# atneit/SCA-LDPC

Hardware: AMD Instinct MI355X
Metric: edge_message_updates_per_s (higher is better)
Workload: dtype f32; 1 GPU; hqc128 H=[Hin|I] N=17669 W=50 R=4000 E=204000, batch 4096/GPU, 50 fixed iters, min_sum; batch_per_gpu=4096, iters=50, tile_group=0

## Files before the change

### include/scaldpc.h

```cpp
#ifndef SCALDPC_H
#define SCALDPC_H

#include <stdint.h>

#ifdef __cplusplus
extern "C" {
#endif

#define SCALDPC_VERSION 104

#define SCALDPC_OK 0
#define SCALDPC_EINVAL 1
#define SCALDPC_EHIP 2
#define SCALDPC_ENOMEM 3
#define SCALDPC_EPMF 4
#define SCALDPC_ENOCONF 5
#define SCALDPC_EDEGREE 6

#define SCALDPC_BP_PRODUCT_SUM 0
#define SCALDPC_BP_MIN_SUM 1

#define SCALDPC_IN_SYNDROME 0
#define SCALDPC_IN_RECEIVED 1

#define SCALDPC_F_EARLY_EXIT 1u
#define SCALDPC_F_DEVICE_IO 2u
#define SCALDPC_F_ASYNC 4u

const char *scaldpc_last_error(void);
int scaldpc_version(void);
int scaldpc_device_count(int *count);
int scaldpc_set_device(int device);
int scaldpc_trim(void);
int scaldpc_debug_live_blocks(int64_t *out);
int scaldpc_debug_fail_alloc(int32_t countdown);
int scaldpc_measure_rmw_stream(int64_t bytes, int32_t rows_per_wave, int32_t reps, double *gbps);

typedef struct scaldpc_bp scaldpc_bp;

int scaldpc_bp_create(int32_t m, int32_t n, int64_t nnz, const int32_t *row_ptr,
                      const int32_t *col_idx, scaldpc_bp **out);
int scaldpc_bp_set_channel_probs(scaldpc_bp *h, const double *probs);
int scaldpc_bp_append_rows(scaldpc_bp *h, int32_t nrows, const int32_t *row_ptr, const int32_t *col_idx, int32_t new_n);
int scaldpc_bp_set_channel_probs_tail(scaldpc_bp *h, int32_t first, int32_t count, const double *probs);
int scaldpc_bp_decode_batch(scaldpc_bp *h, const uint8_t *in, int32_t input_kind, int32_t batch,
                            int32_t max_iter, int32_t method, float alpha, uint32_t flags,
                            void *stream, uint8_t *out_bits, float *out_llr, int32_t *out_iters,
                            uint8_t *out_conv);
int scaldpc_bp_decode_batch_soft(scaldpc_bp *h, const uint8_t *in, int32_t input_kind, int32_t batch,
                                 const float *probs, int32_t prob_cols,
                                 int32_t max_iter, int32_t method, float alpha, uint32_t flags, void *stream,
                                 uint8_t *out_bits, float *out_llr, int32_t *out_iters, uint8_t *out_conv);
int scaldpc_bp_decode_batch_f64(scaldpc_bp *h, const uint8_t *in, int32_t input_kind, int32_t batch,
                                const double *probs, int32_t prob_cols, int32_t max_iter, uint32_t flags, void *stream,
                                uint8_t *out_bits, double *out_llr, int32_t *out_iters, uint8_t *out_conv);
int scaldpc_bp_time_kernels(scaldpc_bp *h, int32_t iters, int32_t method, float alpha, void *stream,
                            float *ms, int32_t *launches);
int scaldpc_bp_set_tile_group(scaldpc_bp *h, int32_t tiles);
int scaldpc_bp_last_compacted(scaldpc_bp *h, int64_t *count);
int scaldpc_bp_last_stats(scaldpc_bp *h, int64_t *out);
#define SCALDPC_SCHEDULE_WORDS 24
int scaldpc_bp_last_schedule(scaldpc_bp *h, int64_t *out);
int scaldpc_bp_last_settle(scaldpc_bp *h, int32_t *frozen_at, int32_t cap, int64_t *info);
int scaldpc_bp_configure(scaldpc_bp *h, const char *key, const char *value);
int scaldpc_bp_device_of(scaldpc_bp *h, int32_t *out);
void scaldpc_bp_destroy(scaldpc_bp *h);

int scaldpc_mc_fer_run(scaldpc_bp *h, int64_t first_trial, int32_t batch, uint64_t seed, int32_t max_iter,
                       int32_t method, float alpha, uint32_t flags, void *stream, uint8_t *out_success,
                       int32_t *out_iters, uint8_t *out_error);
int scaldpc_mc_hqc_run(scaldpc_bp *h, int32_t omega, double eps, int64_t first_trial, int32_t batch, uint64_t seed,
                       int32_t max_iter, int32_t method, float alpha, uint32_t flags, void *stream,
                       uint8_t *out_success, int32_t *out_iters, uint8_t *out_msg, int32_t *out_y);

int scaldpc_mc_hqc_run_soft(scaldpc_bp *h, int32_t omega, const double *weights, const uint8_t *flips, const float *probs,
                            const int32_t *costs, int32_t K, int64_t first_trial, int32_t batch, uint64_t seed,
                            int32_t max_iter, int32_t method, float alpha, uint32_t flags, void *stream,
                            uint8_t *out_success, int32_t *out_iters, uint8_t *out_msg, int32_t *out_y, uint8_t *out_outcome,
                            int32_t *out_flips, int32_t *out_cost);

int scaldpc_mc_hqc_run_stats(scaldpc_bp *h, int32_t omega, const double *weights, const uint8_t *flips, const float *probs,
                             const int32_t *costs, int32_t K, int64_t first_trial, int32_t batch, uint64_t seed,
                             int32_t max_iter, int32_t method, float alpha, uint32_t flags, void *stream,
                             uint8_t *out_success, int32_t *out_iters, uint8_t *out_msg, int32_t *out_y, uint8_t *out_outcome,
                             int32_t *out_flips, int32_t *out_cost, int32_t *out_stats, uint8_t *out_bits);

int scaldpc_mc_fer_run_f64(scaldpc_bp *h, int64_t first_trial, int32_t batch, uint64_t seed, int32_t max_iter,
                           uint32_t flags, void *stream, uint8_t *out_success, int32_t *out_iters, uint8_t *out_error);
int scaldpc_mc_hqc_run_f64(scaldpc_bp *h, int32_t omega, double eps, int64_t first_trial, int32_t batch, uint64_t seed,
                           int32_t max_iter, uint32_t flags, void *stream, uint8_t *out_success, int32_t *out_iters,
                           uint8_t *out_msg, int32_t *out_y);
int scaldpc_mc_hqc_run_stats_f64(scaldpc_bp *h, int32_t omega, const double *weights, const uint8_t *flips,
                                 const double *probs, const int32_t *costs, int32_t K, int64_t first_trial,
                                 int32_t batch, uint64_t seed, int32_t max_iter, uint32_t flags, void *stream,
                                 uint8_t *out_success, int32_t *out_iters, uint8_t *out_msg, int32_t *out_y,
                                 uint8_t *out_outcome, int32_t *out_flips, int32_t *out_cost,
                                 int32_t *out_stats , uint8_t *out_bits);

int scaldpc_mc_fer_run_at(scaldpc_bp *h, const int64_t *trial_ids, int32_t batch, uint64_t seed, int32_t max_iter,
                          int32_t method, float alpha, uint32_t flags, void *stream, uint8_t *out_success,
                          int32_t *out_iters, uint8_t *out_error);
int scaldpc_mc_hqc_run_stats_at(scaldpc_bp *h, int32_t omega, const double *weights, const uint8_t *flips, const float *probs,
                                const int32_t *costs, int32_t K, const int64_t *trial_ids, int32_t batch, uint64_t seed,
                                int32_t max_iter, int32_t method, float alpha, uint32_t flags, void *stream,
                                uint8_t *out_success, int32_t *out_iters, uint8_t *out_msg, int32_t *out_y,
                                uint8_t *out_outcome, int32_t *out_flips, int32_t *out_cost,
                                int32_t *out_stats , uint8_t *out_bits);
int scaldpc_mc_fer_run_at_f64(scaldpc_bp *h, const int64_t *trial_ids, int32_t batch, uint64_t seed, int32_t max_iter,
                              uint32_t flags, void *stream, uint8_t *out_success, int32_t *out_iters, uint8_t *out_error);
int scaldpc_mc_hqc_run_stats_at_f64(scaldpc_bp *h, int32_t omega, const double *weights, const uint8_t *flips,
                                    const double *probs, const int32_t *costs, int32_t K, const int64_t *trial_ids,
                                    int32_t batch, uint64_t seed, int32_t max_iter, uint32_t flags, void *stream,
                                    uint8_t *out_success, int32_t *out_iters, uint8_t *out_msg, int32_t *out_y,
                                    uint8_t *out_outcome, int32_t *out_flips, int32_t *out_cost,
                                    int32_t *out_stats , uint8_t *out_bits);

typedef struct scaldpc_qary scaldpc_qary;

int scaldpc_qary_create(int32_t R, int32_t N, int32_t B, const int8_t *H, int32_t iterations,
                        scaldpc_qary **out);
int scaldpc_qary_min_sum_batch(scaldpc_qary *h, const float *pmf, int32_t batch, uint32_t flags,
                               void *stream, int8_t *out);
void scaldpc_qary_destroy(scaldpc_qary *h);
int scaldpc_qary_into_llr(const float *pmf, int64_t rows, int32_t Q, uint32_t flags, void *stream, float *llr);
int scaldpc_qary_configure(scaldpc_qary *h, const char *key, const char *value);
int scaldpc_qary_last_timing(scaldpc_qary *h, float *ms, int32_t *info);

int scaldpc_qary_special_create(int32_t R, int32_t N, int32_t B, int32_t BSUM, const int8_t *H,
                                int32_t iterations, scaldpc_qary **out);
int scaldpc_qary_special_min_sum_batch(scaldpc_qary *h, const float *pmf_b, const float *pmf_sum,
                                       int32_t batch, uint32_t flags, void *stream, int8_t *out);

int scaldpc_qary_min_sum_batch_soft(scaldpc_qary *h, const float *pmf, int32_t batch, uint32_t flags, void *stream,
                                    int8_t *out, float *out_cost, float *out_margin, int32_t *out_unmet);
int scaldpc_qary_special_min_sum_batch_soft(scaldpc_qary *h, const float *pmf_b, const float *pmf_sum, int32_t batch,
                                            uint32_t flags, void *stream, int8_t *out,
                                            float *out_cost_b, float *out_cost_sum, float *out_margin, int32_t *out_unmet);

int scaldpc_mc_qary_run(scaldpc_qary *h, const float *levels_b, const double *weights_b, int32_t k_b,
                        const float *levels_s, const double *weights_s, int32_t k_s,
                        int64_t first_trial, int32_t batch, uint64_t seed, uint32_t flags, void *stream,
                        uint8_t *out_success, int32_t *out_errs, int32_t *out_wrong, uint8_t *out_levels,
                        int8_t *out_symbols);

int scaldpc_mc_qary_run_secret(scaldpc_qary *h, const double *prior_b,
                               const float *levels_b, const double *weights_b, int32_t k_b,
                               const float *levels_s, const double *weights_s, int32_t k_s,
                               int64_t first_trial, int32_t batch, uint64_t seed, uint32_t flags, void *stream,
                               uint8_t *out_success, int32_t *out_wrong, int32_t *out_channel_wrong,
                               int8_t *out_secret, uint8_t *out_levels, int8_t *out_symbols);

int scaldpc_mc_qary_run_at(scaldpc_qary *h, const float *levels_b, const double *weights_b, int32_t k_b,
                           const float *levels_s, const double *weights_s, int32_t k_s,
                           const int64_t *trial_ids, int32_t batch, uint64_t seed, uint32_t flags, void *stream,
                           uint8_t *out_success, int32_t *out_errs, int32_t *out_wrong, uint8_t *out_levels,
                           int8_t *out_symbols);
int scaldpc_mc_qary_run_secret_at(scaldpc_qary *h, const double *prior_b,
                                  const float *levels_b, const double *weights_b, int32_t k_b,
                                  const float *levels_s, const double *weights_s, int32_t k_s,
                                  const int64_t *trial_ids, int32_t batch, uint64_t seed, uint32_t flags, void *stream,
                                  uint8_t *out_success, int32_t *out_wrong, int32_t *out_channel_wrong,
                                  int8_t *out_secret, uint8_t *out_levels, int8_t *out_symbols);

#ifdef __cplusplus
}
#endif
#endif
```

### sca-ldpc_amd/_lib.py

```python
from __future__ import annotations

import ctypes as C
import os
import subprocess
import sys

_HERE = os.path.dirname(os.path.abspath(__file__))
SO_PATH = os.environ.get("SCALDPC_SO") or os.path.join(_HERE, "libscaldpc.so")
CSRC = os.path.join(_HERE, "csrc")

OK, EINVAL, EHIP, ENOMEM, EPMF, ENOCONF, EDEGREE = range(7)
BP_PRODUCT_SUM, BP_MIN_SUM = 0, 1
IN_SYNDROME, IN_RECEIVED = 0, 1
F_EARLY_EXIT, F_DEVICE_IO, F_ASYNC = 1, 2, 4

_lib = None


class ScaldpcError(RuntimeError):
    pass


def build(verbose=False):
    out = None if verbose else subprocess.DEVNULL
    subprocess.check_call(["make", "-C", CSRC, "../libscaldpc.so"], stdout=out)
    return SO_PATH


def _declare(lib):
    p = C.POINTER
    vp = C.c_void_p
    lib.scaldpc_last_error.restype = C.c_char_p
    lib.scaldpc_last_error.argtypes = []
    lib.scaldpc_version.restype = C.c_int
    lib.scaldpc_device_count.argtypes = [p(C.c_int)]
    lib.scaldpc_set_device.argtypes = [C.c_int]
    lib.scaldpc_trim.argtypes = []
    lib.scaldpc_trim.restype = C.c_int
    lib.scaldpc_debug_live_blocks.argtypes = [p(C.c_int64)]
    lib.scaldpc_debug_live_blocks.restype = C.c_int
    lib.scaldpc_debug_fail_alloc.argtypes = [C.c_int32]
    lib.scaldpc_debug_fail_alloc.restype = C.c_int
    lib.scaldpc_measure_rmw_stream.argtypes = [C.c_int64, C.c_int32, C.c_int32, p(C.c_double)]
    lib.scaldpc_measure_rmw_stream.restype = C.c_int
    lib.scaldpc_bp_create.argtypes = [C.c_int32, C.c_int32, C.c_int64, vp, vp, p(vp)]
    lib.scaldpc_bp_set_channel_probs.argtypes = [vp, vp]
    lib.scaldpc_bp_decode_batch.argtypes = [
        vp, vp, C.c_int32, C.c_int32, C.c_int32, C.c_int32, C.c_float, C.c_uint32, vp, vp, vp, vp, vp,
    ]
    lib.scaldpc_bp_decode_batch_soft.argtypes = [
        vp, vp, C.c_int32, C.c_int32, vp, C.c_int32, C.c_int32, C.c_int32, C.c_float, C.c_uint32, vp, vp, vp, vp, vp,
    ]
    lib.scaldpc_bp_decode_batch_soft.restype = C.c_int
    lib.scaldpc_bp_decode_batch_f64.argtypes = [
        vp, vp, C.c_int32, C.c_int32, vp, C.c_int32, C.c_int32, C.c_uint32, vp, vp, vp, vp, vp,
    ]
    lib.scaldpc_bp_decode_batch_f64.restype = C.c_int
    lib.scaldpc_bp_time_kernels.argtypes = [vp, C.c_int32, C.c_int32, C.c_float, vp, p(C.c_float), p(C.c_int32)]
    lib.scaldpc_bp_set_tile_group.argtypes = [vp, C.c_int32]
    lib.scaldpc_bp_last_compacted.argtypes = [vp, p(C.c_int64)]
    lib.scaldpc_bp_last_compacted.restype = C.c_int
    lib.scaldpc_bp_last_stats.argtypes = [vp, p(C.c_int64)]
    lib.scaldpc_bp_last_stats.restype = C.c_int
    lib.scaldpc_bp_last_schedule.argtypes = [vp, p(C.c_int64)]
    lib.scaldpc_bp_last_schedule.restype = C.c_int
    if hasattr(lib, "scaldpc_bp_last_settle"):
        lib.scaldpc_bp_last_settle.argtypes = [vp, p(C.c_int32), C.c_int32, p(C.c_int64)]
        lib.scaldpc_bp_last_settle.restype = C.c_int
    lib.scaldpc_bp_append_rows.argtypes = [vp, C.c_int32, vp, vp, C.c_int32]
    lib.scaldpc_bp_append_rows.restype = C.c_int
    lib.scaldpc_bp_set_channel_probs_tail.argtypes = [vp, C.c_int32, C.c_int32, vp]
    lib.scaldpc_bp_set_channel_probs_tail.restype = C.c_int
    lib.scaldpc_bp_configure.argtypes = [vp, C.c_char_p, C.c_char_p]
    lib.scaldpc_bp_configure.restype = C.c_int
    lib.scaldpc_bp_device_of.argtypes = [vp, p(C.c_int32)]
    lib.scaldpc_bp_device_of.restype = C.c_int
    lib.scaldpc_bp_destroy.argtypes = [vp]
    lib.scaldpc_bp_destroy.restype = None
    lib.scaldpc_mc_fer_run.argtypes = [
        vp, C.c_int64, C.c_int32, C.c_uint64, C.c_int32, C.c_int32, C.c_float, C.c_uint32, vp, vp, vp, vp,
    ]
    lib.scaldpc_mc_hqc_run.argtypes = [
        vp, C.c_int32, C.c_double, C.c_int64, C.c_int32, C.c_uint64, C.c_int32, C.c_int32, C.c_float, C.c_uint32,
        vp, vp, vp, vp, vp,
    ]
    lib.scaldpc_mc_hqc_run_soft.argtypes = [
        vp, C.c_int32, vp, vp, vp, vp, C.c_int32, C.c_int64, C.c_int32, C.c_uint64, C.c_int32, C.c_int32, C.c_float, C.c_uint32,
        vp, vp, vp, vp, vp, vp, vp, vp,
    ]
    lib.scaldpc_mc_hqc_run_stats.argtypes = lib.scaldpc_mc_hqc_run_soft.argtypes + [vp, vp]
    lib.scaldpc_mc_fer_run_f64.argtypes = [vp, C.c_int64, C.c_int32, C.c_uint64, C.c_int32, C.c_uint32, vp, vp, vp, vp]
    lib.scaldpc_mc_hqc_run_f64.argtypes = [
        vp, C.c_int32, C.c_double, C.c_int64, C.c_int32, C.c_uint64, C.c_int32, C.c_uint32, vp, vp, vp, vp, vp,
    ]
    lib.scaldpc_mc_hqc_run_stats_f64.argtypes = [
        vp, C.c_int32, vp, vp, vp, vp, C.c_int32, C.c_int64, C.c_int32, C.c_uint64, C.c_int32, C.c_uint32,
        vp, vp, vp, vp, vp, vp, vp, vp, vp, vp,
    ]
    for name in ("scaldpc_mc_fer_run_f64", "scaldpc_mc_hqc_run_f64", "scaldpc_mc_hqc_run_stats_f64"):
        getattr(lib, name).restype = C.c_int
    for name, sibling, at in (("scaldpc_mc_fer_run_at", "scaldpc_mc_fer_run", 1),
                              ("scaldpc_mc_hqc_run_stats_at", "scaldpc_mc_hqc_run_stats", 7),
                              ("scaldpc_mc_fer_run_at_f64", "scaldpc_mc_fer_run_f64", 1),
                              ("scaldpc_mc_hqc_run_stats_at_f64", "scaldpc_mc_hqc_run_stats_f64", 7)):
        a = list(getattr(lib, sibling).argtypes)
        assert a[at] is C.c_int64
        a[at] = vp
        getattr(lib, name).argtypes = a
        getattr(lib, name).restype = C.c_int
    for name in (
        "scaldpc_device_count", "scaldpc_set_device", "scaldpc_bp_create", "scaldpc_bp_set_channel_probs",
        "scaldpc_bp_decode_batch", "scaldpc_bp_time_kernels", "scaldpc_bp_set_tile_group", "scaldpc_mc_fer_run",
        "scaldpc_mc_hqc_run", "scaldpc_mc_hqc_run_soft", "scaldpc_mc_hqc_run_stats",
    ):
        getattr(lib, name).restype = C.c_int
    lib.scaldpc_qary_create.argtypes = [C.c_int32, C.c_int32, C.c_int32, vp, C.c_int32, p(vp)]
    lib.scaldpc_qary_min_sum_batch.argtypes = [vp, vp, C.c_int32, C.c_uint32, vp, vp]
    lib.scaldpc_qary_configure.argtypes = [vp, C.c_char_p, C.c_char_p]
    lib.scaldpc_qary_configure.restype = C.c_int
    lib.scaldpc_qary_last_timing.argtypes = [vp, p(C.c_float), p(C.c_int32)]
    lib.scaldpc_qary_last_timing.restype = C.c_int
    lib.scaldpc_qary_into_llr.argtypes = [vp, C.c_int64, C.c_int32, C.c_uint32, vp, vp]
    lib.scaldpc_qary_into_llr.restype = C.c_int
    lib.scaldpc_qary_destroy.argtypes = [vp]
    lib.scaldpc_qary_destroy.restype = None
    lib.scaldpc_qary_special_create.argtypes = [C.c_int32, C.c_int32, C.c_int32, C.c_int32, vp, C.c_int32, p(vp)]
    lib.scaldpc_qary_special_min_sum_batch.argtypes = [vp, vp, vp, C.c_int32, C.c_uint32, vp, vp]
    lib.scaldpc_qary_min_sum_batch_soft.argtypes = [vp, vp, C.c_int32, C.c_uint32, vp, vp, vp, vp, vp]
    lib.scaldpc_qary_special_min_sum_batch_soft.argtypes = [vp, vp, vp, C.c_int32, C.c_uint32, vp, vp, vp, vp, vp, vp]
    lib.scaldpc_mc_qary_run.argtypes = [
        vp, vp, vp, C.c_int32, vp, vp, C.c_int32, C.c_int64, C.c_int32, C.c_uint64, C.c_uint32, vp, vp, vp, vp, vp, vp,
    ]
    lib.scaldpc_mc_qary_run_secret.argtypes = [
        vp, vp, vp, vp, C.c_int32, vp, vp, C.c_int32, C.c_int64, C.c_int32, C.c_uint64, C.c_uint32, vp, vp, vp, vp, vp, vp, vp,
    ]
    lib.scaldpc_mc_qary_run_at.argtypes = [
        vp, vp, vp, C.c_int32, vp, vp, C.c_int32, vp, C.c_int32, C.c_uint64, C.c_uint32, vp, vp, vp, vp, vp, vp,
    ]
    lib.scaldpc_mc_qary_run_secret_at.argtypes = [
        vp, vp, vp, vp, C.c_int32, vp, vp, C.c_int32, vp, C.c_int32, C.c_uint64, C.c_uint32, vp, vp, vp, vp, vp, vp, vp,
    ]
    lib.scaldpc_mc_qary_run_at.restype = lib.scaldpc_mc_qary_run_secret_at.restype = C.c_int
    for name in (
        "scaldpc_qary_create", "scaldpc_qary_min_sum_batch", "scaldpc_qary_special_create",
        "scaldpc_qary_special_min_sum_batch", "scaldpc_qary_min_sum_batch_soft", "scaldpc_qary_special_min_sum_batch_soft",
        "scaldpc_mc_qary_run", "scaldpc_mc_qary_run_secret",
    ):
        getattr(lib, name).restype = C.c_int


def load():
    global _lib
    if _lib is not None:
        return _lib
    if not os.path.exists(SO_PATH):
        raise ScaldpcError(
            f"{SO_PATH} is missing: build it with `make -C {CSRC}` (or __graft_entry__.build()). "
            "sca-ldpc_amd has no CPU fallback."
        )
    if "torch" not in sys.modules and os.environ.get("SCALDPC_NO_TORCH") != "1":
        try:
            import torch
        except Exception:
            pass
    lib = C.CDLL(SO_PATH, mode=C.RTLD_GLOBAL)
    _declare(lib)
    _lib = lib
    return lib


def check(rc):
    if rc == OK:
        return
    msg = load().scaldpc_last_error().decode(errors="replace")
    if rc == EINVAL:
        raise ValueError(msg)
    if rc == ENOMEM:
        raise MemoryError(msg)
    raise ScaldpcError(f"[{rc}] {msg}")


def trim():
    check(load().scaldpc_trim())


def live_blocks():
    out = (C.c_int64 * 6)()
    check(load().scaldpc_debug_live_blocks(out))
    keys = ("device_blocks", "device_bytes", "pinned_blocks", "pinned_bytes", "idle_blocks", "idle_bytes")
    return dict(zip(keys, (int(v) for v in out)))


def measure_rmw_stream(nbytes, rows_per_wave=51, reps=50):
    out = C.c_double(0.0)
    check(load().scaldpc_measure_rmw_stream(int(nbytes), int(rows_per_wave), int(reps), C.byref(out)))
    return float(out.value)


def trial_ids(ids):
    import numpy as np

    a = np.asarray(ids)
    if a.ndim != 1:
        raise ValueError(f"trial_ids must be one-dimensional, got shape {a.shape}")
    if a.size == 0:
        raise ValueError("trial_ids is empty")
    if a.dtype == object and all(isinstance(x, (int, np.integer)) and not isinstance(x, (bool, np.bool_)) for x in a):
        pass
    elif a.dtype.kind not in "iu":
        raise ValueError(f"trial_ids must be of integer dtype, got {a.dtype} (trial indices are not rounded)")
    for bad, why in ((a < 0, "is negative"), (a > 2**63 - 1, "does not fit int64")):
        if bad.any():
            i = int(np.argmax(bad))
            raise ValueError(f"trial_ids[{i}] = {a[i]} {why}")
    return np.ascontiguousarray(a, dtype=np.int64)


def ptr(a):
    if a is None:
        return None
    if isinstance(a, int):
# ... 3 lines not shown
```

### sca-ldpc_amd/bp.py

```python
from __future__ import annotations

import ctypes as C
import os

import numpy as np

from . import _lib
from .graph import TannerGraph

_PS = {"prod_sum", "product_sum", "ps", "0", "prod sum", "prod_sum_log", "product_sum_log", "ps_log", "2", "psl"}
_MS = {"min_sum", "minimum_sum", "ms", "1", "minimum sum", "min sum", "min_sum_log", "minimum_sum_log", "ms_log", "3",
       "minimum sum_log", "msl"}


def _method_id(bp_method):
    key = str(bp_method).lower()
    if key in _PS:
        return _lib.BP_PRODUCT_SUM
    if key in _MS:
        return _lib.BP_MIN_SUM
    raise ValueError(
        f"BP method '{bp_method}' is invalid. Please choose from the following methods: "
        "'product_sum', 'minimum_sum', 'product_sum_log' or 'minimum_sum_log'"
    )
# ... 172 lines not shown
            if cp.ndim != 2 or cp.shape[0] != batch:
                raise ValueError(f"channel_probs must be a 2-D array [batch = {batch}, k], got shape {cp.shape}")
            if not 1 <= cp.shape[1] <= self.n:
                raise ValueError(f"channel_probs covers {cp.shape[1]} columns: expected 1 to n = {self.n}")
        if f64:
            _lib.check(
                self._lib.scaldpc_bp_decode_batch_f64(
                    self._h, _lib.ptr(x), kind, batch, _lib.ptr(cp), 0 if cp is None else cp.shape[1],
                    self.max_iter if max_iter is None else int(max_iter), flags, None,
                    _lib.ptr(bits), _lib.ptr(llr), _lib.ptr(iters), _lib.ptr(conv),
                )
            )
            return {"bits": bits, "llr": llr, "iters": iters, "converged": conv}
        if cp is not None:
            _lib.check(
                self._lib.scaldpc_bp_decode_batch_soft(
                    self._h, _lib.ptr(x), kind, batch, _lib.ptr(cp), cp.shape[1],
                    self.max_iter if max_iter is None else int(max_iter), self._method, self.ms_scaling_factor, flags, None,
                    _lib.ptr(bits), _lib.ptr(llr), _lib.ptr(iters), _lib.ptr(conv),
                )
            )
            return {"bits": bits, "llr": llr, "iters": iters, "converged": conv}
        _lib.check(
            self._lib.scaldpc_bp_decode_batch(
                self._h, _lib.ptr(x), kind, batch, self.max_iter if max_iter is None else int(max_iter),
                self._method, self.ms_scaling_factor, flags, None, _lib.ptr(bits), _lib.ptr(llr),
                _lib.ptr(iters), _lib.ptr(conv),
            )
        )
        return {"bits": bits, "llr": llr, "iters": iters, "converged": conv}

    def decode_batch_device(self, d_in, kind, batch, d_out_bits, max_iter=None, early_exit=False, stream=0,
                            d_out_llr=0, d_out_iters=0, d_out_conv=0, asynchronous=False, d_channel_probs=0, prob_cols=0,
                            precision=None):
        flags = _lib.F_DEVICE_IO | (_lib.F_EARLY_EXIT if early_exit else 0) | (_lib.F_ASYNC if asynchronous else 0)
        if (self.precision if precision is None else _precision(precision, self._method)) == "float64":
            _lib.check(
                self._lib.scaldpc_bp_decode_batch_f64(
                    self._h, C.c_void_p(d_in), kind, batch, C.c_void_p(d_channel_probs or None), int(prob_cols),
                    self.max_iter if max_iter is None else int(max_iter), flags, C.c_void_p(stream or None),
                    C.c_void_p(d_out_bits), C.c_void_p(d_out_llr or None), C.c_void_p(d_out_iters or None),
                    C.c_void_p(d_out_conv or None),
                )
            )
            return
        if d_channel_probs or prob_cols:
            _lib.check(
                self._lib.scaldpc_bp_decode_batch_soft(
                    self._h, C.c_void_p(d_in), kind, batch, C.c_void_p(d_channel_probs or None), int(prob_cols),
                    self.max_iter if max_iter is None else int(max_iter), self._method, self.ms_scaling_factor, flags,
                    C.c_void_p(stream or None), C.c_void_p(d_out_bits), C.c_void_p(d_out_llr or None),
                    C.c_void_p(d_out_iters or None), C.c_void_p(d_out_conv or None),
                )
            )
            return
        _lib.check(
            self._lib.scaldpc_bp_decode_batch(
                self._h, C.c_void_p(d_in), kind, batch, self.max_iter if max_iter is None else int(max_iter),
                self._method, self.ms_scaling_factor, flags, C.c_void_p(stream or None), C.c_void_p(d_out_bits),
                C.c_void_p(d_out_llr or None), C.c_void_p(d_out_iters or None), C.c_void_p(d_out_conv or None),
            )
        )

    def time_kernels(self, iters, stream=0):
        ms = (C.c_float * 2)()
        ln = (C.c_int32 * 6)()
        _lib.check(
            self._lib.scaldpc_bp_time_kernels(
                self._h, iters, self._method, self.ms_scaling_factor, C.c_void_p(stream or None), ms, ln
            )
        )
        return {"ms_check": ms[0], "ms_var": ms[1], "launches_check": ln[0], "launches_var": ln[1], "codewords": ln[2],
                "lanes": ln[3], "codewords_var": ln[4], "record_form": bool(ln[5] & 1),
                "var_writes_out": bool(ln[5] & 2), "var_slim": bool(ln[5] & 4)}

    def mc_fer_run(self, runs, seed, first_trial=0, max_iter=None, early_exit=True, want_errors=False, precision="float32"):
        return _mc_fer(self, int(first_trial), int(runs), "", seed, max_iter, early_exit, want_errors, precision)

    def mc_fer_run_at(self, trial_ids, seed, max_iter=None, early_exit=True, want_errors=False, precision="float32"):
        ids = _lib.trial_ids(trial_ids)
        return _mc_fer(self, _lib.ptr(ids), len(ids), "_at", seed, max_iter, early_exit, want_errors, precision)

    def mc_hqc_run(self, runs, omega, eps, seed, first_trial=0, max_iter=None, early_exit=True, want_inputs=False,
                   want_stats=False, want_bits=False, precision="float32"):
        f64 = _precision(precision, self._method) == "float64"
        if want_stats or want_bits:
            eps = float(eps)
            table = dict(weights=np.array([[eps, 1.0 - eps]] * 2), flips=np.array([1, 0], dtype=np.uint8),
                         probs=np.array([eps, eps]), costs=None)
            r = self.mc_hqc_run_soft(runs, omega, table, seed, first_trial=first_trial, max_iter=max_iter, early_exit=early_exit,
                                     want_inputs=want_inputs, want_stats=want_stats, want_bits=want_bits, precision=precision)
            return {k: r[k] for k in ("success", "iters", "msg", "y", "stats", "bits")}
        succ = np.empty(runs, dtype=np.uint8)
        iters = np.empty(runs, dtype=np.int32)
        msg = np.empty((runs, self.n), dtype=np.uint8) if want_inputs else None
        y = np.empty((runs, omega), dtype=np.int32) if want_inputs else None
        args = (
            self._h, int(omega), float(eps), int(first_trial), int(runs), int(seed),
            self.max_iter if max_iter is None else int(max_iter),
            *(() if f64 else (self._method, self.ms_scaling_factor)),
            _lib.F_EARLY_EXIT if early_exit else 0, None, _lib.ptr(succ), _lib.ptr(iters), _lib.ptr(msg), _lib.ptr(y),
        )
        _lib.check(getattr(self._lib, "scaldpc_mc_hqc_run" + ("_f64" if f64 else ""))(*args))
        return {"success": succ, "iters": iters, "msg": msg, "y": y}

    def mc_hqc_run_at(self, trial_ids, omega, eps, seed, max_iter=None, early_exit=True, want_inputs=False, want_stats=False,
                      want_bits=False, precision="float32"):
        ids = _lib.trial_ids(trial_ids)
        _precision(precision, self._method)
        eps = float(eps)
        table = dict(weights=np.array([[eps, 1.0 - eps]] * 2), flips=np.array([1, 0], dtype=np.uint8),
                     probs=np.array([eps, eps]), costs=None)
        r = self.mc_hqc_run_soft_at(ids, omega, table, seed, max_iter=max_iter, early_exit=early_exit, want_inputs=want_inputs,
                                    want_stats=want_stats, want_bits=want_bits, precision=precision)
        return {k: r[k] for k in ("success", "iters", "msg", "y") + (("stats", "bits") if want_stats or want_bits else ())}

    def mc_hqc_run_soft_at(self, trial_ids, omega, table, seed, max_iter=None, early_exit=True, want_inputs=False,
                           want_stats=False, want_bits=False, precision="float32"):
        ids = _lib.trial_ids(trial_ids)
        return _mc_hqc_soft(self, _lib.ptr(ids), len(ids), True, omega, table, seed, max_iter, early_exit, want_inputs, want_stats,
                                 want_bits, precision)

    def mc_hqc_run_soft(self, runs, omega, table, seed, first_trial=0, max_iter=None, early_exit=True, want_inputs=False,
                        want_stats=False, want_bits=False, precision="float32"):
        return _mc_hqc_soft(self, int(first_trial), int(runs), False, omega, table, seed, max_iter, early_exit, want_inputs,
                                 want_stats, want_bits, precision)

    def last_compacted(self):
        c = C.c_int64()
        _lib.check(self._lib.scaldpc_bp_last_compacted(self._h, C.byref(c)))
        return int(c.value)

    def last_stats(self):
        out = (C.c_int64 * 4)()
        _lib.check(self._lib.scaldpc_bp_last_stats(self._h, out))
        return {"compacted": int(out[0]), "row_parallel": int(out[1]), "levels": int(out[2])}

    def last_schedule(self):
        out = (C.c_int64 * 24)()
        _lib.check(self._lib.scaldpc_bp_last_schedule(self._h, out))
        w = [int(x) for x in out]
        return {"groups": w[0:4], "handed_down": w[4:7], "polls": w[7], "unseen": w[8], "continued": w[9],
                "left_open": w[10], "fixed_chained": w[11], "clears": w[12], "open_at_clear": w[13], "ring_rows": w[14],
                "row_parallel_polls": w[15], "ring_takes": w[16]}

    def last_settle(self):
        info = (C.c_int64 * 4)()
        _lib.check(self._lib.scaldpc_bp_last_settle(self._h, None, 0, info))
        tiles = int(info[0])
        at = (C.c_int32 * max(tiles, 1))()
        _lib.check(self._lib.scaldpc_bp_last_settle(self._h, at, tiles, info))
        return {"frozen_at": [int(x) for x in at[:tiles]], "launches_saved": int(info[1]), "tiles_rerun": int(info[2]),
                "horizon": int(info[3])}

    def last_row_parallel(self):
        return self.last_stats()["row_parallel"]

    def configure(self, **knobs):
        for k, v in knobs.items():
            _lib.check(self._lib.scaldpc_bp_configure(self._h, k.encode(), str(v).encode()))

    def device_of(self):
        out = (C.c_int32 * 4)()
        _lib.check(self._lib.scaldpc_bp_device_of(self._h, out))
        return {"device": out[0], "graph": out[1], "messages": out[2], "state": out[3]}

    def set_tile_group(self, tiles):
        _lib.check(self._lib.scaldpc_bp_set_tile_group(self._h, int(tiles)))

    def close(self):
        if getattr(self, "_h", None):
            self._lib.scaldpc_bp_destroy(self._h)
            self._h = None

    def __enter__(self):
        return self

    def __exit__(self, *exc):
        self.close()
        return False

    def __del__(self):
        try:
            self.close()
        except Exception:
            pass


def _mc_fer(dec, trials, runs, at, seed, max_iter, early_exit, want_errors, precision):
    f64 = _precision(precision, dec._method) == "float64"
    succ = np.empty(runs, dtype=np.uint8)
    iters = np.empty(runs, dtype=np.int32)
    err = np.empty((runs, dec.n), dtype=np.uint8) if want_errors else None
    args = (
        dec._h, trials, runs, int(seed), dec.max_iter if max_iter is None else int(max_iter),
        *(() if f64 else (dec._method, dec.ms_scaling_factor)),
        _lib.F_EARLY_EXIT if early_exit else 0, None, _lib.ptr(succ), _lib.ptr(iters), _lib.ptr(err),
    )
    _lib.check(getattr(dec._lib, f"scaldpc_mc_fer_run{at}" + ("_f64" if f64 else ""))(*args))
    return {"success": succ, "iters": iters, "errors": err}


def _mc_hqc_soft(dec, trials, runs, listed, omega, table, seed, max_iter, early_exit, want_inputs, want_stats, want_bits,
                 precision):
    f64 = _precision(precision, dec._method) == "float64"
    w = np.ascontiguousarray(table["weights"], dtype=np.float64)
    if w.ndim != 2 or w.shape[0] != 2:
        raise ValueError(f"table['weights'] must be [2, K], got shape {w.shape}")
    K = w.shape[1]
    fl = np.asarray(table["flips"])
    pr = np.ascontiguousarray(table["probs"], dtype=np.float64 if f64 else np.float32)
    costs = table.get("costs")
    if fl.shape != (K,) or pr.shape != (K,) or (costs is not None and np.shape(costs) != (K,)):
        raise ValueError(f"table: flips, probs and costs must hold one entry per outcome (K = {K})")
    cs = None if costs is None else np.asarray(costs)
    for name, a, t in (("flips", fl, np.uint8), ("costs", cs, np.int32)):
        if a is not None and not np.array_equal(a.astype(t), a):
            raise ValueError(f"table['{name}'] = {a.tolist()} does not fit {np.dtype(t).name}")
    fl = np.ascontiguousarray(fl, dtype=np.uint8)
    cs = None if cs is None else np.ascontiguousarray(cs, dtype=np.int32)
    succ = np.empty(runs, dtype=np.uint8)
    iters = np.empty(runs, dtype=np.int32)
    flips = np.empty(runs, dtype=np.int32)
    cost = np.empty(runs, dtype=np.int32) if costs is not None else None
    msg = np.empty((runs, dec.n), dtype=np.uint8) if want_inputs else None
    y = np.empty((runs, omega), dtype=np.int32) if want_inputs else None
    outcome = np.empty((runs, dec.m), dtype=np.uint8) if want_inputs else None
    args = (
        dec._h, int(omega), _lib.ptr(w), _lib.ptr(fl), _lib.ptr(pr), _lib.ptr(cs), K,
        trials, runs, int(seed), dec.max_iter if max_iter is None else int(max_iter),
        *(() if f64 else (dec._method, dec.ms_scaling_factor)),
        _lib.F_EARLY_EXIT if early_exit else 0, None, _lib.ptr(succ), _lib.ptr(iters),
        _lib.ptr(msg), _lib.ptr(y), _lib.ptr(outcome), _lib.ptr(flips), _lib.ptr(cost),
    )
    res = {"success": succ, "iters": iters, "flips": flips, "cost": cost, "msg": msg, "y": y, "outcome": outcome}
    want = want_stats or want_bits
    with_stats = want or listed or f64
    entry = "scaldpc_mc_hqc_run_" + ("stats" if with_stats else "soft") + ("_at" if listed else "") + ("_f64" if f64 else "")
    stats = np.empty((runs, len(HQC_STATS_COLUMNS)), dtype=np.int32) if want else None
    bits = np.empty((runs, dec.n), dtype=np.uint8) if want_bits else None
    _lib.check(getattr(dec._lib, entry)(*args, *((_lib.ptr(stats), _lib.ptr(bits)) if with_stats else ())))
    return dict(res, stats=stats, bits=bits) if want else res


bp_decoder = BpDecoder
```

### sca-ldpc_amd/csrc/scaldpc_bp.hip

```cpp
#include "scaldpc_common.h"
#include "scaldpc_bp_sched.h"
#include "scaldpc_mc_law.h"
#include "scaldpc_trials.h"

#include <algorithm>
#include <cfloat>
#include <chrono>
#include <cmath>
#include <cstdlib>
#include <cstring>
#include <mutex>
#include <unordered_map>
#include <vector>

typedef unsigned long long u64;

using namespace scaldpc;

#include "scaldpc_bp_kernels.h"
#include "scaldpc_bp_ref64.h"

namespace scaldpc {
int launch_mc_hqc_outcome64(const McHqcLaw64 &law, unsigned long long *synd, double *plane, int R, int batch, int T, long first,
                            unsigned k0, unsigned k1, int *acc_flips, int *acc_cost, uint8_t *out_outcome, hipStream_t s);
int launch_gather_prior64(const double *src, int cols, const int *ids, double *dst, int T2, hipStream_t s);
int launch_mc_bernoulli_at(bool xor_into, unsigned long long *planes, int len, int batch, int T, const long long *ids, unsigned stream,
                           unsigned k0, unsigned k1, const unsigned long long *thr, unsigned long long thr0, hipStream_t s);
int launch_mc_hqc_secret_at(unsigned long long *planes, int n, int N, int omega, int batch, int T, const long long *ids, unsigned k0,
                            unsigned k1, int *out_y, hipStream_t s);
int launch_mc_hqc_outcome_at(const McHqcLaw &law, unsigned long long *synd, float *plane, int R, int batch, int T, const long long *ids,
                             unsigned k0, unsigned k1, int *acc_flips, int *acc_cost, uint8_t *out_outcome, hipStream_t s);
int launch_mc_hqc_outcome64_at(const McHqcLaw64 &law, unsigned long long *synd, double *plane, int R, int batch, int T,
                               const long long *ids, unsigned k0, unsigned k1, int *acc_flips, int *acc_cost, uint8_t *out_outcome,
                               hipStream_t s);
}

namespace {

struct Buckets {
    int nb;
    int maxd[MAXB];
    int off[MAXB];
    int cnt[MAXB];
    int blk[MAXB + 1];
};

struct HostBuckets {
    Buckets bk;
    pvec<int> list;
    bool has_generic = false;
};

}

struct Knobs {
    enum Path { AUTO = 0, STREAM = 1, EDGE = 2, LDS = 3 };
    int path = AUTO;
    int split = 2;
    double group_mb = 215.0;
    int el_max = -1;
    int compact_after = -1;
    int fuse_test = 1;
    int first_fused = 1;
    int minsum_rec = 1;
    int settle = -1;
    int settle_horizon = 0;
};

struct HandleStreams {
    int device = 0;
    hipStream_t own_stream = nullptr;
    hipStream_t aux_stream[4] = {};
    hipEvent_t ev_join[4] = {}, ev_phase[4] = {};
    HandleStreams() = default;
    HandleStreams(const HandleStreams &) = delete;
    HandleStreams &operator=(const HandleStreams &) = delete;
    ~HandleStreams()
    {
        if (own_stream) stream_release(own_stream, device);
        for (int k = 0; k < 4; k++) {
            if (aux_stream[k]) stream_release(aux_stream[k], device);
            if (ev_join[k]) (void)hipEventDestroy(ev_join[k]);
            if (ev_phase[k]) (void)hipEventDestroy(ev_phase[k]);
        }
    }
};

struct scaldpc_bp : HandleStreams {
    Knobs kn;
    int m = 0, n = 0;
    long E = 0;
    int max_row_deg = 0, max_col_deg = 0, min_row_deg = 0;
    int *d_row_ptr = nullptr, *d_col_idx = nullptr, *d_col_ptr = nullptr, *d_csc_edge = nullptr;
    int *d_var_list = nullptr, *d_row_list = nullptr;
    int *d_var_meta = nullptr, *d_csc_list = nullptr;
    Buckets var_bk{}, row_bk{};
    bool need_scratch = false;
    float *d_prior = nullptr;
    bool have_prior = false;
    int prior_n = 0;
    int cap_tiles = 0, cap_group = 0, tile_group = 0;
    Buf<float> d_msg, d_scratch, d_post;
    Buf<u64> d_synd, d_recv, d_hard, d_done, d_conv, d_unsat;
    Buf<int> d_iters, d_remaining;
    Buf<float> d_pprior, d_probs_in;
    Buf<u64> d_soft_bad;
    int cap_remaining = 0;
    RemRing rem;
    SchedCounters sched;
    Buf<uint8_t> d_in, d_out_bits, d_out_conv;
    Buf<float> d_out_llr;
    Buf<int> d_out_iters;
    PinnedBuf<int> h_remaining;
    PinnedBuf<uint8_t> h_io;
    Buf<uint8_t> d_out_all;
    pvec<double> h_probs;
    Buf<u64> d_thr, d_mc, d_diff;
    Buf<int> d_ylist;
    Buf<uint8_t> d_succ;
    bool thr_valid = false;
    Buf<int> d_mc_acc;
    Buf<int> d_mc_stats;
    Buf<uint8_t> d_mc_outcome;
    Buf<long long> d_trial_ids;
    struct Level {
        int cap_tiles = 0;
        Buf<u64> synd, hard, done, conv, unsat;
        Buf<int> iters, ids, slot_of;
        Buf<float> post, pprior;
        Buf<double> pratio64;
    };
    static constexpr int MAX_LEVELS = SCHED_MAX_LEVELS;
    Level lv[MAX_LEVELS + 1];
    long stat_levels = 0;
    long stat_deferred = 0;
    Buf<float> d_emsg;
    Buf<int> d_el_unsat;
    int *d_el_slots = nullptr, *d_el_slot_col = nullptr;
    int el_waves = 0;
    int el_cap_bins = 0;
    bool el_ok = false;
    pvec<int> h_el_slots, h_el_col;
    pvec<int> seg_slot;
    pvec<unsigned char> seg_cap;
    int el_open_used = 0;
    bool incremental = false, full_stale = false;
    pvec<int> hg_col_idx;
    Buf<int> d_csr_rp, d_csr_ci;
    Buf<float> d_prior_buf;
    int ws_m = 0, ws_n = 0;
    pvec<int> el_dirty_slot, el_dirty_col;
    Buf<int> d_pairs;
    PinnedBuf<int> h_pairs;
    Buf<int> d_graph;
    Buf<int> d_tile_tab;
    Buf<int2> d_first_tab;
    Buf<float> d_rec;
    Buf<u64> d_mask;
    int cap_rec_group = 0;
    int *d_csc_row = nullptr, *d_var_rows = nullptr, *d_csr_pos = nullptr;
    bool var_reversed = false;
    bool first_valid = false;
    int first_method = -1;
    float first_alpha = 0.0f;
    Buf<int> d_el_tab;
    pvec<int> hg_row_ptr, hg_cdeg, hg_col_ptr, hg_csc_edge;
    HostBuckets hg_var, hg_row;
    int stat_el = 0;
    int identity_from = -1;
    bool async_used = false;
    bool broken = false;
    Buf<double> d_ratio, d_x64, d_c64, d_post64, d_pratio, d_probs_in64, d_out_llr64;
    Buf<int> d_rem64;
    PinnedBuf<int> h_rem64;
    bool ratio_valid = false;
    Buf<unsigned> d_settle;
    PinnedBuf<unsigned> h_settle;
    int settle_next = 0;
    int settle_key_iter = 0, settle_key_soft = 0;
    float settle_key_alpha = -1.0f;
    std::vector<int> settle_frozen_at;
    long settle_saved = 0, settle_rerun = 0;
    int settle_K = 0;
    int last_group = 0;
    bool last_early = false;
    std::mutex mu;
};

namespace {

bool set_knob(Knobs &k, const char *key, const char *val)
{
    if (!key || !val) return false;
    if (!strcmp(key, "path")) {
        if (!strcmp(val, "auto") || !*val) k.path = Knobs::AUTO;
        else if (!strcmp(val, "stream")) k.path = Knobs::STREAM;
        else if (!strcmp(val, "edge")) k.path = Knobs::EDGE;
        else if (!strcmp(val, "lds")) k.path = Knobs::LDS;
        else return false;
        return true;
    }
    char *end = nullptr;
    const double x = strtod(val, &end);
    if (end == val) return false;
    if (!strcmp(key, "split")) k.split = (int)x;
    else if (!strcmp(key, "group_mb")) k.group_mb = x;
    else if (!strcmp(key, "el_max")) k.el_max = (int)x;
    else if (!strcmp(key, "compact_after")) k.compact_after = (int)x;
    else if (!strcmp(key, "first_fused")) k.first_fused = (int)x != 0;
    else if (!strcmp(key, "minsum_rec")) k.minsum_rec = x == 2.0 ? 2 : (int)x != 0;
    else if (!strcmp(key, "fuse_test")) k.fuse_test = (int)x != 0;
    else if (!strcmp(key, "settle") && x >= -1 && x <= 2) k.settle = (int)x;
    else if (!strcmp(key, "settle_horizon") && x >= 0) k.settle_horizon = (int)x;
    else return false;
    return true;
}

void knobs_from_env(Knobs &k)
{
    static const char *const names[][2] = {{"SCALDPC_PATH", "path"}, {"SCALDPC_SPLIT", "split"},
                                           {"SCALDPC_GROUP_MB", "group_mb"}, {"SCALDPC_EL_MAX", "el_max"},
                                           {"SCALDPC_COMPACT_AFTER", "compact_after"}, {"SCALDPC_FIRST_FUSED", "first_fused"},
                                           {"SCALDPC_FUSE_TEST", "fuse_test"}, {"SCALDPC_MINSUM_REC", "minsum_rec"},
                                           {"SCALDPC_SETTLE", "settle"}, {"SCALDPC_SETTLE_HORIZON", "settle_horizon"}};
    for (auto &nm : names)
        if (const char *e = getenv(nm[0])) (void)set_knob(k, nm[1], e);
}

void build_buckets(const pvec<int> &deg, const int *bounds, int nb, bool keep_isolated, HostBuckets &out)
{
    const int n = (int)deg.size();
    int maxdeg = 0;
    for (int d : deg) maxdeg = std::max(maxdeg, d);
    pvec<int> start(maxdeg + 2, 0);
    for (int d : deg) start[d + 1]++;
    for (int d = 0; d <= maxdeg; d++) start[d + 1] += start[d];
    pvec<int> order(n), cursor(start.begin(), start.end() - 1);
    for (int i = 0; i < n; i++) order[cursor[deg[i]]++] = i;
    out.list.clear();
    out.list.reserve(n);
    out.has_generic = false;
    Buckets &bk = out.bk;
    memset(&bk, 0, sizeof bk);
    int lo = keep_isolated ? 0 : 1;
    for (int b = 0; b <= nb && lo <= maxdeg; b++) {
        const int hi = b < nb ? std::min(bounds[b], maxdeg) : maxdeg;
        if (hi < lo) continue;
        const int first = start[lo], last = start[hi + 1];
        if (last > first) {
            const int i = bk.nb++;
            bk.maxd[i] = b < nb ? bounds[b] : 0;
            if (b == nb) out.has_generic = true;
            bk.off[i] = (int)out.list.size();
            bk.cnt[i] = last - first;
            bk.blk[i + 1] = bk.blk[i] + (bk.cnt[i] + 3) / 4;
            out.list.insert(out.list.end(), order.begin() + first, order.begin() + last);
        }
        lo = hi + 1;
    }
}

template <typename T, bool P>
int grow(Buf<T, P> &b, size_t need)
{
    return b.ensure(need, need + need / 8);
}

int auto_group(const scaldpc_bp *h, int T, int plane_cols = 0)
{
    const double budget = h->kn.group_mb * 1e6;
    const double per_tile = ((double)h->E + plane_cols) * TW * sizeof(float);
    const int g = per_tile > 0 ? (int)(budget / per_tile) : T;
    return std::max(1, std::min(g, T));
}

int parity_blocks(int m) { return (m + 4 * ROWS_PER_WAVE - 1) / (4 * ROWS_PER_WAVE); }
int parity_waves(const scaldpc_bp *h) { return 4 * parity_blocks(h->m); }

int ensure_workspace(scaldpc_bp *h, int T, int G, bool want_post, int max_iter, int prob_cols = 0)
{
    if (prob_cols) SC_TRY(grow(h->d_pprior, (size_t)T * prob_cols * TW));
    if (T > h->cap_tiles || h->m > h->ws_m || h->n > h->ws_n) {
        h->d_synd.reset(); h->d_recv.reset(); h->d_hard.reset(); h->d_done.reset();
        h->d_conv.reset(); h->d_unsat.reset(); h->d_iters.reset(); h->d_post.reset();
        T = std::max(T, h->cap_tiles);
        h->cap_tiles = 0;
        const int wm = h->incremental ? h->m + h->m / 2 + 64 : h->m, wn = h->incremental ? h->n + h->n / 2 + 64 : h->n;
        const size_t pw = (size_t)4 * parity_blocks(wm);
        SC_TRY(h->d_synd.ensure((size_t)T * wm));
        SC_TRY(h->d_recv.ensure((size_t)T * wn));
        SC_TRY(h->d_hard.ensure((size_t)T * wn));
        SC_TRY(h->d_done.ensure((size_t)T));
        SC_TRY(h->d_conv.ensure((size_t)T));
        SC_TRY(h->d_unsat.ensure((size_t)T * pw));
        SC_TRY(h->d_iters.ensure((size_t)T * TW));
        h->cap_tiles = T;
        h->ws_m = wm;
        h->ws_n = wn;
    }
    if (want_post) SC_TRY(h->d_post.ensure((size_t)h->cap_tiles * h->ws_n * TW));
    const int want_rows = ring_rows_wanted(T, G);
    if (max_iter + 2 > h->cap_remaining || want_rows > h->rem.rows) {
        h->d_remaining.reset();
        h->h_remaining.reset();
        h->cap_remaining = 0;
        h->rem.rows = 0;
        const int len = max_iter + 2;
        SC_TRY(h->d_remaining.ensure((size_t)want_rows * (size_t)len));
        SC_TRY(h->h_remaining.ensure((size_t)len));
        h->cap_remaining = len;
        h->rem.rows = want_rows;
    }
    h->rem.slot = h->rem.rows;
    h->sched.w[SCHED_RING_ROWS] = h->rem.rows;
    return 0;
}

int next_remaining_row(scaldpc_bp *h, hipStream_t s, int **row, bool lanes_open)
{
    bool clears = false;
    const int slot = ring_take(h->rem, &clears);
    h->sched.note_take(clears, lanes_open);
    if (clears) SC_HIP(hipMemsetAsync(h->d_remaining, 0, sizeof(int) * (size_t)h->rem.rows * h->cap_remaining, s));
    *row = h->d_remaining + (size_t)slot * h->cap_remaining;
    return 0;
}

int *stage_buffer(size_t ints)
{
    struct Staging {
        int *p = nullptr;
        size_t cap = 0;
        ~Staging() { free(p); }
    };
    static thread_local Staging stage;
    if (ints > stage.cap || stage.cap > ((size_t)64 << 20)) {
        free(stage.p);
        stage.cap = 0;
        stage.p = (int *)malloc(std::max<size_t>(ints, 1) * sizeof(int));
        if (!stage.p) return nullptr;
        stage.cap = ints;
    }
    return stage.p;
}

int upload_table(Buf<int> &dst, const int *host, size_t ints)
{
    SC_TRY(dst.ensure(ints));
    SC_HIP(hipMemcpy(dst, host, ints * sizeof(int), hipMemcpyHostToDevice));
    return 0;
}

int ensure_tile_tables(scaldpc_bp *h)
{
    if (h->d_tile_tab) return 0;
    const HostBuckets &hv = h->hg_var, &hr = h->hg_row;
    const int *row_ptr = h->hg_row_ptr.data(), *cdeg = h->hg_cdeg.data(), *col_ptr = h->hg_col_ptr.data(),
              *csc_edge = h->hg_csc_edge.data();
    size_t total = 0;
    auto reserve = [&](size_t cnt) {
        const size_t off = total;
        total += (cnt + 63) / 64 * 64;
        return off;
    };
    const size_t o_var_meta = reserve((size_t)4 * VAR_REC * hv.bk.blk[hv.bk.nb] + 4), o_csc_list = reserve((size_t)h->E + 1 + 64);
    const size_t o_row_list = reserve((size_t)16 * hr.bk.blk[hr.bk.nb] + 4);
    const size_t o_csc_row = reserve((size_t)h->E + 1 + 64);
    const size_t o_csr_pos = reserve((size_t)h->E + 64);
    const size_t o_var_rows = reserve((size_t)4 * VAR_INLINE * hv.bk.blk[hv.bk.nb] + 4);
    int *host = stage_buffer(total);
    if (!host) return fail(SCALDPC_ENOMEM, "out of host memory");
    pvec<int> const_last((size_t)h->m);
    rec_mark_const_last(h->m, h->n, row_ptr, col_ptr, csc_edge, const_last.data());
    for (int b = 0; b < hr.bk.nb; b++) {
        const int blocks = hr.bk.blk[b + 1] - hr.bk.blk[b];
        for (int sl = 0; sl < blocks * 4; sl++) {
            int *md = host + o_row_list + 4 * ((size_t)hr.bk.blk[b] * 4 + sl);
// ... 428 lines not shown
        with_first_prior(h, first, tv, [&](auto fst, auto P, auto prior) {
            hipLaunchKernelGGL((k_el_check<M, fst, decltype(P)>), dim3((h->m + 3) / 4, nb), dim3(256), 0, s, h->d_row_ptr,
                               h->d_col_idx, prior, h->d_emsg, tv.synd, tv.done, skip_done, h->m, h->E, alpha, hard_g, unsat_prev);
        });
    });
    LAUNCH_CHECK();
    return 0;
}
int launch_el_var(scaldpc_bp *h, const TileState &tv, int nb, int skip_done, int write_out, hipStream_t s, const int *unsat_prev,
                  int it_prev, int *remaining_prev)
{
    const unsigned gx = (unsigned)(((h->el_waves + 3) / 4 + 7) / 8 * 8);
    with_prior(h, tv.pprior, tv.first_col, [&](auto P, auto prior) {
        hipLaunchKernelGGL((k_el_var<decltype(P)>), dim3(gx, nb), dim3(256), 0, s, (const int2 *)h->d_el_slots, h->d_el_slot_col,
                           h->el_waves, prior, h->d_emsg, tv.post, tv.hard, tv.done, skip_done, h->E, write_out, unsat_prev, it_prev,
                           remaining_prev ? tv.conv : nullptr, remaining_prev ? tv.iters : nullptr, remaining_prev);
    });
    LAUNCH_CHECK();
    return 0;
}

int launch_syndrome(const scaldpc_bp *h, const u64 *x, u64 *synd, int T, hipStream_t s)
{
    hipLaunchKernelGGL(k_parity<false>, dim3(parity_blocks(h->m), T), dim3(256), 0, s, h->d_row_ptr, h->d_col_idx, x, h->m, h->n,
                       synd, (u64 *)nullptr, (const u64 *)nullptr);
    LAUNCH_CHECK();
    return 0;
}

size_t small_lds_bytes(const scaldpc_bp *h) { return (size_t)2 * h->E * sizeof(float) + (size_t)2 * h->n + h->m + 64; }
size_t small_lds(const scaldpc_bp *h)
{
    const size_t lds = small_lds_bytes(h);
    const bool fits = h->E > 0 && lds <= 60 * 1024;
    return fits && h->kn.path != Knobs::STREAM && h->kn.path != Knobs::EDGE ? lds : 0;
}

template <bool PLANES>
int launch_small(scaldpc_bp *h, size_t lds, int method, int batch, const void *in, int input_kind, int max_iter, float alpha,
                 bool early, void *bits, float *llr, int *iters, void *conv, hipStream_t s, const float *pprior = nullptr,
                 int first_col = 0)
{
    with_method(method, [&](auto M) {
        auto launch = [&](auto P, auto prior) {
            hipLaunchKernelGGL((k_bp_small<M, PLANES, decltype(P)>), dim3(batch), dim3(256), lds, s, h->d_row_ptr, h->d_col_idx,
                               h->d_col_ptr, h->d_csc_edge, prior, h->m, h->n, (int)h->E, in, input_kind, max_iter, alpha,
                               early ? 1 : 0, bits, llr, iters, conv);
        };
        with_prior(h, pprior, first_col, launch);
    });
    LAUNCH_CHECK();
    return 0;
}

float alpha_for(float alpha, int it)
{
    return alpha == 0.0f ? (float)(1.0 - std::pow(2.0, -1.0 * it)) : alpha;
}

int ensure_el_unsat(scaldpc_bp *h, int max_iter) { return h->d_el_unsat.ensure(((size_t)max_iter + 2) * TW); }

int iterate_el(scaldpc_bp *h, const DecodeCall &c, const TileState &st, int nb)
{
    const hipStream_t s = c.s;
    const bool early = c.early;
    const int max_iter = c.max_iter, skip = early ? 1 : 0;
    if (early) {
        SC_TRY(ensure_el_unsat(h, max_iter));
        if (!c.state_ready) {
            SC_HIP(hipMemsetAsync(h->d_el_unsat, 0, sizeof(int) * ((size_t)max_iter + 2) * TW, s));
            SC_HIP(hipMemsetAsync(h->d_remaining, 0, sizeof(int) * ((size_t)max_iter + 2), s));
        }
    }
    static_assert(ROW_CAP == TW, "el_ok (a row = at most one wave of edge lanes) must imply fused_init's rows <= ROW_CAP");
    for (int it = 1; it <= max_iter; it++) {
        const bool last = it == max_iter;
        int *const up = early && it > 1 ? h->d_el_unsat + (size_t)(it - 1) * TW : nullptr;
        int *const rem_prev = early ? h->d_remaining + it - 1 : nullptr;
        SC_TRY(launch_el_check(h, st, nb, c.method, alpha_for(c.alpha, it), skip, s, it == 1, early ? st.hard : nullptr, up));
        SC_TRY(launch_el_var(h, st, nb, skip, (early || last) ? 1 : 0, s, up, early ? it - 1 : 0, rem_prev));
        if (last) {
            hipLaunchKernelGGL(k_parity<true>, dim3(parity_blocks(h->m), 1), dim3(256), 0, s, h->d_row_ptr, h->d_col_idx, st.hard,
                               h->m, h->n, const_cast<u64 *>(st.synd), st.unsat, (const u64 *)st.done);
            LAUNCH_CHECK();
            hipLaunchKernelGGL(k_finalize, dim3(1), dim3(64), 0, s, it, early ? 1 : 0, st.done, st.conv, st.unsat, parity_waves(h),
                               st.iters, h->d_remaining + it);
            LAUNCH_CHECK();
            break;
        }
        const int ip = it - 1;
        if (early && el_poll_point(ip)) {
            h->sched.w[SCHED_EL_POLLS]++;
            SC_HIP(hipMemcpyAsync(h->h_remaining + ip, h->d_remaining + ip, sizeof(int), hipMemcpyDeviceToHost, s));
            SC_HIP(hipStreamSynchronize(s));
            if (h->h_remaining[ip] == 0) break;
        }
    }
    return 0;
}

constexpr int MAX_LANES = SCHED_MAX_LANES;
int fixed_lanes(const scaldpc_bp *h, int g)
{
    if (h->E == 0) return 1;
    return lanes_of(h->kn.split, g);
}
int ensure_lanes(scaldpc_bp *h, int nl)
{
    for (int k = 1; k < nl; k++)
        if (!h->aux_stream[k]) {
            int dev = 0;
            SC_TRY(stream_acquire(&h->aux_stream[k], &dev));
            SC_HIP(hipEventCreateWithFlags(&h->ev_join[k], hipEventDisableTiming));
            SC_HIP(hipEventCreateWithFlags(&h->ev_phase[k], hipEventDisableTiming));
        }
    if (nl > 1 && !h->ev_join[0]) SC_HIP(hipEventCreateWithFlags(&h->ev_join[0], hipEventDisableTiming));
    return 0;
}
struct Lanes {
    scaldpc_bp *h;
    hipStream_t s;
    int n = 1;
    bool open = false;
    Lanes(scaldpc_bp *h_, hipStream_t s_) : h(h_), s(s_) {}
    Lanes(const Lanes &) = delete;
    Lanes &operator=(const Lanes &) = delete;
    ~Lanes() { if (open) (void)join(); }
    hipStream_t operator[](int k) const { return k ? h->aux_stream[k] : s; }
    int fork(int nl)
    {
        n = nl;
        open = nl > 1;
        if (!open) return 0;
        SC_HIP(hipEventRecord(h->ev_join[0], s));
        for (int k = 1; k < n; k++) SC_HIP(hipStreamWaitEvent(h->aux_stream[k], h->ev_join[0], 0));
        return 0;
    }
    int join()
    {
        for (int k = 1; k < n; k++) {
            SC_HIP(hipEventRecord(h->ev_join[k], h->aux_stream[k]));
            SC_HIP(hipStreamWaitEvent(s, h->ev_join[k], 0));
        }
        open = false;
        return 0;
    }
};


struct SettlePlan {
    unsigned *words = nullptr;
    int first_test = 0, horizon = 0;
    unsigned *of(int tile) const { return words + (size_t)tile * SETTLE_WORDS; }
};
int iterate_tiles(scaldpc_bp *h, const DecodeCall &c, Lanes &lanes, const TileState &st, int g0, int g, int defer_after,
                  bool *deferred, PollState &ps, int chain, const SettlePlan &sl)
{
    const hipStream_t s = lanes.s;
    const bool early = c.early;
    const int max_iter = c.max_iter, method = c.method, skip = early ? 1 : 0;
    const int nl = fixed_lanes(h, g);
    SC_TRY(ensure_lanes(h, nl));
    int gs[MAX_LANES], t0[MAX_LANES];
    deal_tiles(g, nl, gs, t0);
    TileState tv[MAX_LANES];
    for (int k = 0; k < nl; k++) tv[k] = st.at(h, g0 + t0[k]);
    const int pw = parity_waves(h);
    const bool fused = fused_init(h, method);
    if (h->E && !fused) {
        with_prior(h, tv[0].pprior, st.first_col, [&](auto P, auto prior) {
            hipLaunchKernelGGL((k_init_msg<decltype(P)>), dim3((unsigned)((h->E + 3) / 4), g), dim3(256), 0, s, h->d_col_idx,
                               h->d_msg.get(), h->E, prior);
        });
        LAUNCH_CHECK();
    }
    int *rem = h->d_remaining;
    if (early) SC_TRY(next_remaining_row(h, s, &rem, lanes.open));
    if (!(chain & 1)) SC_TRY(lanes.fork(nl));
    const bool first_fuse = first_fusable(h, method) && !st.pprior;
    if (first_fuse) SC_TRY(ensure_first_table(h, method, alpha_for(c.alpha, 1), s));
    const bool ride = early && h->kn.fuse_test && check_can_test(h, method) && pw >= FT_WORDS;
    bool verdict_pending[MAX_LANES] = {};
    const bool recf = rec_form(h, method);
    bool rec_booted[MAX_LANES] = {};
    const bool tracked = sl.words && recf && !early;
    const int K = tracked ? sl.horizon : 0, last_test = K ? K : max_iter;
    bool set_phase = phase_reestablished(chain, K, max_iter);
    if (K) h->settle_saved += (long)nl * settle_launches_saved(K, max_iter);
    const bool keep_hard = tracked && st.post == nullptr;
    for (int it = 1; it <= max_iter; it++) {
        const bool last = it == max_iter;
        if (!settle_enqueued(it, K, max_iter)) continue;
        const bool no_check = (first_fuse && it == 1) || !settle_has_check(it, K, max_iter);
        const bool poll = poll_point(it, defer_after, ps);
        lanes.open = nl > 1;
        for (int k = 0; k < nl && !no_check; k++) {
            CheckPass cp;
            cp.alpha = alpha_for(c.alpha, it);
            cp.first = fused && it == 1;
            cp.tile0 = t0[k];
            if (verdict_pending[k]) {
                cp.test = fused_test(h, tv[k], rem + (it - 1), it - 1, true);
                verdict_pending[k] = false;
            }
            cp.boot = recf && !cp.first && !rec_booted[k];
            if (cp.boot) rec_booted[k] = true;
            if (tracked)
                cp.settle = Settle{sl.of(g0 + t0[k]), settle_check_done(it, sl.first_test),
                                   cp.boot ? 0 : settle_check_mark(it, sl.first_test, last_test)};
            SC_TRY(launch_check(h, tv[k], gs[k], method, skip, lanes[k], cp));
            if (set_phase && k + 1 < nl) {
                SC_HIP(hipEventRecord(h->ev_phase[k + 1], lanes[k]));
                SC_HIP(hipStreamWaitEvent(lanes[k + 1], h->ev_phase[k + 1], 0));
            }
        }
        if (!no_check) set_phase = false;
        if (!settle_has_var(it, K)) continue;
        for (int k = 0; k < nl; k++) {
            VarPass vp;
            vp.write_out = (early || last) ? 1 : 0;
            vp.tile0 = t0[k];
            vp.first_synd = first_fuse && it == 1;
            vp.rec = it > 1 && recf;
            vp.light = it > 1;
            vp.final_pass = last;
            vp.keep_hard = keep_hard && !last;
            if (tracked && !last)
                vp.settle = Settle{sl.of(g0 + t0[k]), settle_var_done(it, sl.first_test, last_test),
                                   settle_var_mark(it, sl.first_test, last_test)};
            else if (keep_hard)
                vp.settle = Settle{sl.of(g0 + t0[k]), last_test, 0};
            SC_TRY(launch_var(h, tv[k], gs[k], skip, lanes[k], vp));
            if (ride && !last && !poll) {
                verdict_pending[k] = true;
            } else if (early || last) {
                const dim3 grid(parity_blocks(h->m), gs[k]);
                const FusedTest pf = fused_test(h, tv[k], rem + it, it, early);
                if (pw >= FT_WORDS && h->kn.fuse_test)
                    hipLaunchKernelGGL(k_parity_fin_sharded, grid, dim3(256), 0, lanes[k], h->d_row_ptr, h->d_col_idx, h->m, tv[k].synd,
                                       pf);
                else
                    hipLaunchKernelGGL(k_parity_fin, grid, dim3(256), 0, lanes[k], h->d_row_ptr, h->d_col_idx, pf.hard, h->m, h->n,
                                       tv[k].synd, pf.unsat, pf.pw, pf.it_prev, pf.latch, pf.done, pf.conv, pf.iters, pf.remaining);
                LAUNCH_CHECK();
            }
        }
        if (!early || last || !poll) continue;
        if (it == defer_after && stops_unseen(defer_after, max_iter, ps)) {
            note_unseen(ps);
            h->sched.w[SCHED_UNSEEN]++;
            *deferred = true;
            if (chain & 2) return 0;
            return lanes.join();
        }
        SC_TRY(lanes.join());
        SC_HIP(hipMemcpyAsync(h->h_remaining + it, rem + it, sizeof(int), hipMemcpyDeviceToHost, s));
        SC_HIP(hipStreamSynchronize(s));
        set_phase = true;
        h->sched.w[SCHED_POLLS]++;
        const PollVerdict v = after_poll(ps, it, defer_after, max_iter, h->h_remaining[it], std::min(c.batch - g0 * TW, g * TW), g,
                                          el_limit(h, method));
        if (v == POLL_DONE) return 0;
        if (v == POLL_HAND_OVER) {
            *deferred = true;
            return 0;
        }
    }
    if (chain & 2) return 0;
    return lanes.join();
}

int ensure_level(scaldpc_bp *h, scaldpc_bp::Level &L, int T2)
{
    if (T2 <= L.cap_tiles) return 0;
    L.synd.reset(); L.hard.reset(); L.done.reset(); L.conv.reset(); L.unsat.reset();
    L.iters.reset(); L.ids.reset();
    L.cap_tiles = 0;
    SC_TRY(L.synd.ensure((size_t)T2 * h->m));
    SC_TRY(L.hard.ensure((size_t)T2 * h->n));
    SC_TRY(L.done.ensure((size_t)T2));
    SC_TRY(L.conv.ensure((size_t)T2));
    SC_TRY(L.unsat.ensure((size_t)T2 * parity_waves(h)));
    SC_TRY(L.iters.ensure((size_t)T2 * TW));
    SC_TRY(L.ids.ensure((size_t)T2 * TW));
    L.cap_tiles = T2;
    return 0;
}

int plan_settle(scaldpc_bp *h, const DecodeCall &c, int lvl, const TileState &st, SettlePlan *sl)
{
    const int settle = settle_mode(h->kn.settle, h->identity_from >= 0);
    if (lvl != 0 || c.early || settle <= 0 || !rec_form(h, c.method)) return 0;
    int alpha_from = 1;
    while (alpha_from < c.max_iter && alpha_for(c.alpha, alpha_from) != alpha_for(c.alpha, c.max_iter)) alpha_from++;
    sl->first_test = settle_first_test(alpha_from);
    const int soft = st.pprior ? 1 : 0;
    if (h->settle_key_iter != c.max_iter || h->settle_key_alpha != c.alpha || h->settle_key_soft != soft) {
        h->settle_next = 0;
        h->settle_key_iter = c.max_iter;
        h->settle_key_alpha = c.alpha;
        h->settle_key_soft = soft;
    }
    if (sl->first_test > c.max_iter) return 0;
    SC_TRY(h->d_settle.ensure((size_t)c.T * SETTLE_WORDS));
    SC_HIP(hipMemsetAsync(h->d_settle, 0, sizeof(unsigned) * (size_t)c.T * SETTLE_WORDS, c.s));
    sl->words = h->d_settle;
    if (settle >= 2 && !c.no_sync) {
        const int K = h->kn.settle_horizon > 0 ? h->kn.settle_horizon : h->settle_next;
        if (settle_horizon_usable(K, sl->first_test, c.max_iter)) sl->horizon = K;
    }
    return 0;
}

int collect_settle(scaldpc_bp *h, const DecodeCall &c, Lanes &lanes, const TileState &st, const SettlePlan &sl)
{
    const int T = c.T, Gl = std::min(c.G, T);
    SC_TRY(h->h_settle.ensure((size_t)T * SETTLE_WORDS));
    auto read_back = [&](int t0, int cnt, int last_test) -> int {
        SC_HIP(hipMemcpyAsync(h->h_settle + (size_t)t0 * SETTLE_WORDS, sl.of(t0), sizeof(unsigned) * (size_t)cnt * SETTLE_WORDS,
                              hipMemcpyDeviceToHost, c.s));
        SC_HIP(hipStreamSynchronize(c.s));
        for (int t = t0; t < t0 + cnt; t++) {
            unsigned latest = 0;
            for (int i = 0; i < SETTLE_SHARDS; i++) latest = std::max(latest, h->h_settle[(size_t)t * SETTLE_WORDS + i]);
            h->settle_frozen_at[t] = settle_frozen_at((int)latest, sl.first_test, last_test);
        }
        return 0;
    };
    h->settle_frozen_at.assign(T, 0);
    h->settle_K = sl.horizon;
    SC_TRY(read_back(0, T, sl.horizon ? sl.horizon : c.max_iter));
    if (sl.horizon) {
        SettlePlan again = sl;
        again.horizon = 0;
        PollState poll;
        for (int t = 0; t < T;) {
            if (h->settle_frozen_at[t]) { t++; continue; }
            int g = 1;
            while (g < Gl && t + g < T && !h->settle_frozen_at[t + g]) g++;
            SC_HIP(hipMemsetAsync(sl.of(t), 0, sizeof(unsigned) * (size_t)g * SETTLE_WORDS, c.s));
            bool d = false;
            SC_TRY(iterate_tiles(h, c, lanes, st, t, g, 0, &d, poll, 0, again));
            SC_TRY(read_back(t, g, c.max_iter));
            h->settle_rerun += g;
            t += g;
        }
    }
    int frozen = 0, max_at = 0;
    for (int t = 0; t < T; t++) {
        frozen += h->settle_frozen_at[t] > 0;
        max_at = std::max(max_at, h->settle_frozen_at[t]);
    }
    const bool learns = settle_mode(h->kn.settle, h->identity_from >= 0) >= 2;
    h->settle_next = learns ? settle_next_horizon(T, frozen, max_at, (int)h->settle_rerun, c.max_iter) : 0;
    return 0;
}

int hand_down(scaldpc_bp *h, const DecodeCall &c, int lvl, const TileState &st, const std::vector<char> &deferred_tile);

int decode_level(scaldpc_bp *h, const DecodeCall &c, int lvl, const TileState &st)
{
    const int T = c.T, Gl = std::min(c.G, T), max_iter = c.max_iter;
    const bool early = c.early;
    const int el = (T == 1 && c.batch <= el_limit(h, c.method)) ? c.batch : 0;
    if (el)
        SC_TRY(ensure_el(h, el));
    else
        SC_TRY(ensure_msg(h, Gl, c.method));
    if (lvl == 0) {
        h->last_group = el ? 0 : Gl;
        h->last_early = early;
    }
    h->stat_levels = lvl;
    if (el) {
        h->stat_el = el;
        return iterate_el(h, c, st, el);
    }

    const int defer_after = defer_after_of(early, lvl, h->kn.compact_after, max_iter);
    SC_HIP(hipMemsetAsync(st.unsat, 0, sizeof(u64) * (size_t)T * parity_waves(h), c.s));
    std::vector<char> deferred_tile(T, 0);
    bool any = false;
    PollState poll;
    const bool lanes2 = fused_init(h, c.method) && fixed_lanes(h, Gl) > 1;
    Lanes lanes(h, c.s);
    SettlePlan sl;
    SC_TRY(plan_settle(h, c, lvl, st, &sl));
    for (int g0 = 0; g0 < T; g0 += Gl) {
        const int g = std::min(Gl, T - g0);
        bool d = false;
        const bool next_full = g0 + Gl < T && std::min(Gl, T - (g0 + Gl)) == Gl;
        const int chain = chain_bits(early, lanes2, g == Gl, g0 == 0, next_full, lanes.open, defer_after, max_iter, poll, h->rem);
        h->sched.note_group(lvl, early, chain);
        SC_TRY(iterate_tiles(h, c, lanes, st, g0, g, defer_after, &d, poll, chain, sl));
        if (d) {
            any = true;
            for (int t = g0; t < g0 + g; t++) deferred_tile[t] = 1;
        }
    }
    if (sl.words && !c.no_sync) SC_TRY(collect_settle(h, c, lanes, st, sl));
    return any ? hand_down(h, c, lvl, st, deferred_tile) : 0;
}

int hand_down(scaldpc_bp *h, const DecodeCall &c, int lvl, const TileState &st, const std::vector<char> &deferred_tile)
{
    const hipStream_t s = c.s;
    const int T = c.T;
    std::vector<u64> done_h(T);
    SC_HIP(hipMemcpyAsync(done_h.data(), st.done, sizeof(u64) * T, hipMemcpyDeviceToHost, s));
    SC_HIP(hipStreamSynchronize(s));
    pvec<int> ids, slot_of((size_t)T * TW, -1);
    for (int t = 0; t < T; t++) {
        if (!deferred_tile[t]) continue;
        for (int w = 0; w < TW; w++) {
            const long b = (long)t * TW + w;
            if (b < c.batch && !((done_h[t] >> w) & 1)) {
                slot_of[b] = (int)ids.size();
                ids.push_back((int)b);
            }
        }
    }
    DecodeCall c2 = c;
    c2.batch = (int)ids.size();
    if (c2.batch == 0) return 0;
    if (lvl == 0) h->stat_deferred = c2.batch;
    h->sched.w[SCHED_HANDED + lvl] = c2.batch;
    const int T2 = c2.T = (c2.batch + TW - 1) / TW;
    ids.resize((size_t)T2 * TW, -1);
    scaldpc_bp::Level &L = h->lv[lvl + 1];
    SC_TRY(ensure_level(h, L, T2));
    SC_TRY(grow(L.slot_of, (size_t)T * TW));
    if (c.want_post) SC_TRY(grow(L.post, (size_t)T2 * h->n * TW));
    const int pcols = st.pprior ? h->n - st.first_col : 0;
    if (pcols) SC_TRY(grow(L.pprior, (size_t)T2 * pcols * TW));
    SC_HIP(hipMemcpyAsync(L.ids, ids.data(), sizeof(int) * ids.size(), hipMemcpyHostToDevice, s));
    SC_HIP(hipMemcpyAsync(L.slot_of, slot_of.data(), sizeof(int) * slot_of.size(), hipMemcpyHostToDevice, s));
    hipLaunchKernelGGL(k_gather_planes, dim3((h->m + 63) / 64, T2), dim3(256), 0, s, st.synd, h->m, L.ids, L.synd);
    LAUNCH_CHECK();
    if (pcols) {
        hipLaunchKernelGGL(k_gather_prior, dim3((pcols + 3) / 4, T2), dim3(256), 0, s, st.pprior, pcols, L.ids, L.pprior);
        LAUNCH_CHECK();
    }
    hipLaunchKernelGGL(k_init_state, dim3(T2), dim3(64), 0, s, c2.batch, c.max_iter, L.done, L.conv, L.iters);
    LAUNCH_CHECK();
    SC_HIP(hipMemsetAsync(L.hard, 0, sizeof(u64) * (size_t)T2 * h->n, s));
    SC_HIP(hipStreamSynchronize(s));
    const TileState st2{L.synd, L.hard, L.done, L.conv, L.unsat, L.iters, c.want_post ? L.post : nullptr,
                        pcols ? L.pprior.get() : nullptr, st.first_col};
    SC_TRY(decode_level(h, c2, lvl + 1, st2));
    hipLaunchKernelGGL(k_scatter_planes, dim3((h->n + 63) / 64, T), dim3(256), 0, s, st.hard, h->n, L.slot_of, L.hard);
    LAUNCH_CHECK();
    hipLaunchKernelGGL(k_scatter_state, dim3(T), dim3(64), 0, s, st.iters, st.conv, L.slot_of, L.iters, L.conv);
    LAUNCH_CHECK();
    if (c.want_post) {
        hipLaunchKernelGGL(k_scatter_post, dim3(h->n, T), dim3(64), 0, s, st.post, h->n, L.slot_of, L.post);
        LAUNCH_CHECK();
    }
    return 0;
}

int run_core(scaldpc_bp *h, const DecodeCall &c, const float *pprior = nullptr, int first_col = 0)
{
    if (!c.state_ready) {
        hipLaunchKernelGGL(k_init_state, dim3(c.T), dim3(64), 0, c.s, c.batch, c.max_iter, h->d_done, h->d_conv, h->d_iters);
        LAUNCH_CHECK();
        SC_HIP(hipMemsetAsync(h->d_hard, 0, sizeof(u64) * (size_t)c.T * h->n, c.s));
    }
    h->last_group = 0;
    h->stat_deferred = 0;
    h->stat_el = 0;
    h->stat_levels = 0;

    if (const size_t lds = small_lds(h)) {
        return launch_small<true>(h, lds, c.method, c.batch, h->d_synd, SCALDPC_IN_SYNDROME, c.max_iter, c.alpha, c.early, h->d_hard,
                                  c.want_post ? h->d_post.get() : nullptr, h->d_iters, h->d_conv, c.s, pprior, first_col);
    }
    const TileState st{h->d_synd, h->d_hard, h->d_done, h->d_conv, h->d_unsat, h->d_iters,
                       c.want_post ? h->d_post : nullptr, pprior, first_col};
    return decode_level(h, c, 0, st);
}

}

#define TMARK(name)                                                                                   \
    do {                                                                                              \
        static const bool on__ = getenv("SCALDPC_TIMING") != nullptr;                                 \
        if (on__) {                                                                                   \
            auto now__ = std::chrono::steady_clock::now();                                            \
            fprintf(stderr, "[create] %-10s %8.1f us\n", name,                                        \
                    std::chrono::duration<double, std::micro>(now__ - tmark_last()).count());         \
            tmark_last() = now__;                                                                     \
        }                                                                                             \
    } while (0)
static std::chrono::steady_clock::time_point &tmark_last()
{
    static thread_local std::chrono::steady_clock::time_point t = std::chrono::steady_clock::now();
    return t;
}

namespace {

int finish_graph(scaldpc_bp *h, const int *row_ptr, const int *col_idx, const pvec<int> &rdeg, pvec<int> &cdeg)
{
    const int m = h->m, n = h->n;
    const long nnz = h->E;
    h->max_row_deg = m ? *std::max_element(rdeg.begin(), rdeg.end()) : 0;
    h->min_row_deg = m ? *std::min_element(rdeg.begin(), rdeg.end()) : 0;
    h->max_col_deg = *std::max_element(cdeg.begin(), cdeg.end());
    static const int vb[] = {1, 2, 4, 8, 16, 32, 64};
    static const int rb[] = {2, 4, 8, 16, 32, 64};
    HostBuckets hv, hr;
    build_buckets(cdeg, vb, 7, true, hv);
    build_buckets(rdeg, rb, 6, false, hr);
    TMARK("buckets");
    h->var_bk = hv.bk;
    h->row_bk = hr.bk;
    h->need_scratch = hv.has_generic || hr.has_generic;
    h->identity_from = -1;
    if (n > m) {
        bool ident = true;
        for (int r = 0; r < m && ident; r++) {
            const int j = n - m + r;
            ident = cdeg[j] == 1 && row_ptr[r + 1] > row_ptr[r] && col_idx[row_ptr[r + 1] - 1] == j;
        }
        h->identity_from = ident ? n - m : -1;
    }
    h->el_ok = nnz > 0 && h->max_row_deg <= ROW_CAP && h->max_col_deg <= 64;
    const bool own_csr = h->incremental;
    size_t total = 0;
    auto reserve = [&](size_t cnt) {
        const size_t off = total;
        total += (cnt + 63) / 64 * 64;
        return off;
    };
    const size_t o_row_ptr = own_csr ? 0 : reserve((size_t)m + 1), o_col_idx = own_csr ? 0 : reserve((size_t)nnz);
    const size_t o_col_ptr = reserve((size_t)n + 1), o_csc_edge = reserve((size_t)nnz), o_var_list = reserve(hv.list.size());
    const size_t o_prior = own_csr ? 0 : reserve((size_t)n);
    int *const host = stage_buffer(total);
    if (!host) return fail(SCALDPC_ENOMEM, "out of host memory");
    TMARK("reserve");
    if (!own_csr) {
        std::copy(row_ptr, row_ptr + m + 1, host + o_row_ptr);
        std::copy(col_idx, col_idx + nnz, host + o_col_idx);
    }
    int *col_ptr = host + o_col_ptr, *csc_edge = host + o_csc_edge;
    {
        col_ptr[0] = 0;
        for (int j = 0; j < n; j++) col_ptr[j + 1] = col_ptr[j] + cdeg[j];
        pvec<int> cursor(col_ptr, col_ptr + n);
        for (int e = 0; e < (int)nnz; e++) csc_edge[cursor[col_idx[e]]++] = e;
    }
    std::copy(hv.list.begin(), hv.list.end(), host + o_var_list);
    TMARK("csc");
    SC_TRY(h->d_graph.ensure(total));
    if (hipMemcpy(h->d_graph, host, total * sizeof(int), hipMemcpyHostToDevice) != hipSuccess)
        return fail(SCALDPC_EHIP, "graph upload failed");
    TMARK("upload");
    if (!own_csr) h->hg_row_ptr.assign(row_ptr, row_ptr + m + 1);
    h->hg_col_ptr.assign(col_ptr, col_ptr + n + 1);
    h->hg_csc_edge.assign(csc_edge, csc_edge + nnz);
    h->hg_cdeg.swap(cdeg);
    h->hg_var = std::move(hv);
    h->hg_row = std::move(hr);
    TMARK("keep");
    if (!own_csr) {
        h->d_row_ptr = h->d_graph + o_row_ptr;
        h->d_col_idx = h->d_graph + o_col_idx;
        h->d_prior = (float *)(h->d_graph + o_prior);
    }
    h->d_col_ptr = h->d_graph + o_col_ptr;
    h->d_csc_edge = h->d_graph + o_csc_edge;
    h->d_var_list = h->d_graph + o_var_list;
    return 0;
}

int make_incremental(scaldpc_bp *h)
{
    if (h->incremental) return 0;
    const size_t rows = (size_t)h->m + 1, edges = (size_t)h->E, cols = (size_t)h->n;
    SC_TRY(h->d_csr_rp.ensure(rows + rows / 2 + 256));
    SC_TRY(h->d_csr_ci.ensure(edges + edges / 2 + 4096));
    SC_TRY(h->d_prior_buf.ensure(cols + cols / 2 + 256));
    SC_HIP(hipMemcpy(h->d_csr_rp, h->d_row_ptr, rows * sizeof(int), hipMemcpyDeviceToDevice));
    if (edges) SC_HIP(hipMemcpy(h->d_csr_ci, h->d_col_idx, edges * sizeof(int), hipMemcpyDeviceToDevice));
    SC_HIP(hipMemcpy(h->d_prior_buf, h->d_prior, cols * sizeof(float), hipMemcpyDeviceToDevice));
    h->d_row_ptr = h->d_csr_rp;
    h->d_col_idx = h->d_csr_ci;
    h->d_prior = h->d_prior_buf;
    h->hg_col_idx.resize(edges);
    for (int j = 0; j < h->n; j++)
        for (int k = h->hg_col_ptr[j]; k < h->hg_col_ptr[j + 1]; k++) h->hg_col_idx[h->hg_csc_edge[k]] = j;
    h->incremental = true;
    h->d_el_tab.reset();
    h->d_el_slots = h->d_el_slot_col = nullptr;
    return 0;
}

template <typename T>
int grow_graph(Buf<T> &b, size_t used, size_t need)
{
    return b.grow_keep(used, need, need + need / 2 + 256);
}

int refresh_full(scaldpc_bp *h)
{
    if (!h->full_stale) return 0;
    pvec<int> rdeg(h->m), cdeg(h->hg_cdeg);
    for (int r = 0; r < h->m; r++) rdeg[r] = h->hg_row_ptr[r + 1] - h->hg_row_ptr[r];
    h->d_graph.reset();
    h->d_tile_tab.reset();
    h->d_var_meta = h->d_csc_list = h->d_row_list = nullptr;
    SC_TRY(finish_graph(h, h->hg_row_ptr.data(), h->hg_col_idx.data(), rdeg, cdeg));
    h->full_stale = false;
    return 0;
}

int check_usable(const scaldpc_bp *h)
{
    if (!h->broken) return 0;
    return fail(SCALDPC_EHIP, "this decoder is unusable: an earlier scaldpc_bp_append_rows failed part-way; destroy it and build a new one");
}

int prior_llrs(const double *probs, int first, int count, pvec<float> &llr)
{
    float last_p = 0.0f, last_llr = 0.0f;
    for (int j = 0; j < count; j++) {
        if (!(probs[j] >= 0.0 && probs[j] <= 1.0))
            return fail(SCALDPC_EINVAL, "channel_probs[%d] = %g is not a probability", first + j, probs[j]);
        const float p = (float)probs[j];
        if (j == 0 || p != last_p) {
            last_p = p;
            last_llr = logf((1.0f - p) / p);
        }
        llr[j] = last_llr;
    }
    return 0;
}

void settle_report_reset(scaldpc_bp *h)
{
    h->settle_frozen_at.clear();
    h->settle_saved = h->settle_rerun = 0;
    h->settle_K = 0;
}
int begin_call(scaldpc_bp *h, int batch, int max_iter, void *stream, DecodeCall *c)
{
    if (!h->have_prior || h->prior_n < h->n)
        return fail(SCALDPC_EINVAL, "channel probabilities not set (columns [%d, %d))", h->have_prior ? h->prior_n : 0, h->n);
    h->sched.reset();
    settle_report_reset(h);
    c->batch = batch;
    c->max_iter = max_iter > 0 ? max_iter : h->n;
    c->s = stream ? (hipStream_t)stream : h->own_stream;
    c->T = (batch + TW - 1) / TW;
    if (c->T > 65535) return fail(SCALDPC_EINVAL, "batch %d too large for one call (max %d)", batch, 65535 * TW);
    c->G = (h->tile_group > 0) ? std::min(h->tile_group, c->T) : auto_group(h, c->T);
    return 0;
}

struct SyncOnError {
    hipStream_t s;
    bool ok = false;
    ~SyncOnError() { if (!ok) (void)hipStreamSynchronize(s); }
    int done() { ok = true; return 0; }
};

struct TimingEvents {
    std::vector<hipEvent_t> ev;
    TimingEvents() = default;
    TimingEvents(const TimingEvents &) = delete;
    TimingEvents &operator=(const TimingEvents &) = delete;
    ~TimingEvents() { for (hipEvent_t e : ev) if (e) (void)hipEventDestroy(e); }
    int create(size_t count)
    {
        ev.assign(count, nullptr);
        for (hipEvent_t &e : ev) SC_HIP(hipEventCreate(&e));
        return 0;
    }
    hipEvent_t &operator[](size_t i) { return ev[i]; }
};

int stage_input(scaldpc_bp *h, const uint8_t *in, size_t bytes, bool dev_io, hipStream_t s, const uint8_t **din)
{
    *din = in;
    if (dev_io) return 0;
    SC_TRY(grow(h->d_in, bytes));
    SC_HIP(hipMemcpyAsync(h->d_in, in, bytes, hipMemcpyHostToDevice, s));
    *din = h->d_in;
    return 0;
}

struct Outputs {
    uint8_t *bits = nullptr;
    float *llr = nullptr;
    int32_t *iters = nullptr;
    uint8_t *conv = nullptr;
};
int stage_outputs(scaldpc_bp *h, const Outputs &out, int batch, bool dev_io, bool with_state, Outputs *dev)
{
    *dev = out;
    if (dev_io) return 0;
    const size_t planes = (size_t)batch * h->n;
    if (out.bits) {
        SC_TRY(grow(h->d_out_bits, planes));
        dev->bits = h->d_out_bits;
    }
    if (out.llr) {
        SC_TRY(grow(h->d_out_llr, planes));
        dev->llr = h->d_out_llr;
    }
    if (with_state) {
        if ((size_t)batch > h->d_out_conv.cap()) {
            h->d_out_iters.reset();
            h->d_out_conv.reset();
            SC_TRY(h->d_out_iters.ensure((size_t)batch));
            SC_TRY(h->d_out_conv.ensure((size_t)batch));
        }
        dev->iters = out.iters ? h->d_out_iters.get() : nullptr;
        dev->conv = out.conv ? h->d_out_conv.get() : nullptr;
    }
    return 0;
}
int copy_outputs(const scaldpc_bp *h, const Outputs &out, const Outputs &dev, int batch, bool dev_io, hipStream_t s)
{
    if (dev_io) return 0;
    const size_t planes = (size_t)batch * h->n;
    if (out.bits) SC_HIP(hipMemcpyAsync(out.bits, dev.bits, planes, hipMemcpyDeviceToHost, s));
    if (out.llr) SC_HIP(hipMemcpyAsync(out.llr, dev.llr, sizeof(float) * planes, hipMemcpyDeviceToHost, s));
    if (out.iters) SC_HIP(hipMemcpyAsync(out.iters, dev.iters, sizeof(int) * (size_t)batch, hipMemcpyDeviceToHost, s));
    if (out.conv) SC_HIP(hipMemcpyAsync(out.conv, dev.conv, (size_t)batch, hipMemcpyDeviceToHost, s));
    return 0;
}

template <typename T, bool P>
int mc_stage(Buf<T, P> &block, T *out, size_t count, bool dev_io, T **dev)
{
    *dev = out;
    if (!out || dev_io) return 0;
    SC_TRY(grow(block, count));
    *dev = block.get();
    return 0;
}
template <typename T>
int mc_unstage(T *out, const T *dev, size_t count, bool dev_io, hipStream_t s)
{
    if (out && !dev_io) SC_HIP(hipMemcpyAsync(out, dev, sizeof(T) * count, hipMemcpyDeviceToHost, s));
    return 0;
}

}


extern "C" {

int scaldpc_bp_create(int32_t m, int32_t n, int64_t nnz, const int32_t *row_ptr, const int32_t *col_idx,
                      scaldpc_bp **out)
{
    if (!out) return fail(SCALDPC_EINVAL, "out is NULL");
    *out = nullptr;
    if (m <= 0 || n <= 0 || nnz < 0 || !row_ptr || (nnz && !col_idx))
        return fail(SCALDPC_EINVAL, "bad graph arguments (m=%d n=%d nnz=%lld)", m, n, (long long)nnz);
    if (nnz > 0x7fffffffLL) return fail(SCALDPC_EINVAL, "nnz too large");
    if (row_ptr[0] != 0 || row_ptr[m] != nnz) return fail(SCALDPC_EINVAL, "row_ptr does not span [0, nnz]");
    TMARK("start");
    pvec<int> rdeg(m), cdeg(n, 0);
    for (int r = 0; r < m; r++) {
        if (row_ptr[r + 1] < row_ptr[r]) return fail(SCALDPC_EINVAL, "row_ptr not monotone at row %d", r);
        rdeg[r] = row_ptr[r + 1] - row_ptr[r];
        for (int e = row_ptr[r]; e < row_ptr[r + 1]; e++) {
            if (col_idx[e] < 0 || col_idx[e] >= n) return fail(SCALDPC_EINVAL, "col_idx out of range at edge %d", e);
            if (e > row_ptr[r] && col_idx[e] <= col_idx[e - 1])
                return fail(SCALDPC_EINVAL, "col_idx not strictly ascending in row %d", r);
            cdeg[col_idx[e]]++;
        }
    }
    scaldpc_bp *h = new (std::nothrow) scaldpc_bp();
    if (!h) return fail(SCALDPC_ENOMEM, "out of host memory");
    knobs_from_env(h->kn);
    h->m = m;
    h->n = n;
    h->E = nnz;
    TMARK("validate");
    int rc = finish_graph(h, row_ptr, col_idx, rdeg, cdeg);
    if (!rc) rc = stream_acquire(&h->own_stream, &h->device);
    TMARK("stream");
    if (rc) {
        scaldpc_bp_destroy(h);
        return rc;
    }
    *out = h;
    return 0;
}

int scaldpc_bp_set_channel_probs(scaldpc_bp *h, const double *probs)
{
    if (!h || !probs) return fail(SCALDPC_EINVAL, "NULL argument");
    std::lock_guard<std::mutex> lk(h->mu);
    SC_TRY(check_usable(h));
    DeviceGuard dg(h->device);
    pvec<float> llr(h->n);
    SC_TRY(prior_llrs(probs, 0, h->n, llr));
    SC_HIP(hipMemcpy(h->d_prior, llr.data(), sizeof(float) * h->n, hipMemcpyHostToDevice));
    h->h_probs.assign(probs, probs + h->n);
    h->thr_valid = false;
    h->first_valid = false;
    h->settle_next = 0;
    h->ratio_valid = false;
    h->have_prior = true;
    h->prior_n = h->n;
    return 0;
}

int scaldpc_bp_set_channel_probs_tail(scaldpc_bp *h, int32_t first, int32_t count, const double *probs)
{
    if (!h || (count > 0 && !probs)) return fail(SCALDPC_EINVAL, "NULL argument");
    std::lock_guard<std::mutex> lk(h->mu);
    SC_TRY(check_usable(h));
    DeviceGuard dg(h->device);
    if (first < 0 || count < 0 || (long)first + count > h->n)
        return fail(SCALDPC_EINVAL, "columns [%d, %d) are outside the graph (n = %d)", first, first + count, h->n);
    if (first > h->prior_n) return fail(SCALDPC_EINVAL, "priors of columns [%d, %d) are still unset", h->prior_n, first);
    if (count == 0) return 0;
    if (h->async_used) SC_HIP(hipDeviceSynchronize());
    pvec<float> llr(count);
    SC_TRY(prior_llrs(probs, first, count, llr));
    SC_HIP(hipMemcpy(h->d_prior + first, llr.data(), sizeof(float) * count, hipMemcpyHostToDevice));
    h->h_probs.resize(h->n, 0.0);
    std::copy(probs, probs + count, h->h_probs.begin() + first);
    h->thr_valid = false;
    h->first_valid = false;
    h->settle_next = 0;
    h->ratio_valid = false;
    h->prior_n = std::max(h->prior_n, first + count);
    h->have_prior = true;
    return 0;
}

int scaldpc_bp_append_rows(scaldpc_bp *h, int32_t nrows, const int32_t *row_ptr, const int32_t *col_idx, int32_t new_n)
{
    if (!h || nrows < 0 || (nrows > 0 && !row_ptr)) return fail(SCALDPC_EINVAL, "bad arguments");
    std::lock_guard<std::mutex> lk(h->mu);
    SC_TRY(check_usable(h));
    DeviceGuard dg(h->device);
    CacheBypass guard(h->async_used);
    if (new_n < h->n) return fail(SCALDPC_EINVAL, "new_n = %d is smaller than the current block length %d", new_n, h->n);
    const long add = nrows ? row_ptr[nrows] : 0;
    if (nrows && (row_ptr[0] != 0 || add < 0 || (add && !col_idx))) return fail(SCALDPC_EINVAL, "row_ptr does not start at 0");
    if ((long)h->E + add > 0x7fffffffL) return fail(SCALDPC_EINVAL, "nnz too large");
    for (int r = 0; r < nrows; r++) {
        if (row_ptr[r + 1] < row_ptr[r]) return fail(SCALDPC_EINVAL, "row_ptr not monotone at appended row %d", r);
        for (int e = row_ptr[r]; e < row_ptr[r + 1]; e++) {
            if (col_idx[e] < 0 || col_idx[e] >= new_n) return fail(SCALDPC_EINVAL, "col_idx out of range at appended edge %d", e);
            if (e > row_ptr[r] && col_idx[e] <= col_idx[e - 1])
                return fail(SCALDPC_EINVAL, "col_idx not strictly ascending in appended row %d", r);
        }
    }
    if (nrows == 0 && new_n == h->n) return 0;
    if (h->async_used) SC_HIP(hipDeviceSynchronize());
    TMARK("app:start");
    struct Unfinished {
        scaldpc_bp *h;
        bool done = false;
        ~Unfinished() { if (!done) h->broken = true; }
    } unfinished{h};
    SC_TRY(make_incremental(h));
    hipStream_t s = h->own_stream;
    const int m0 = h->m, n0 = h->n;
    const long E0 = h->E;
    SC_TRY(grow_graph(h->d_csr_rp, (size_t)m0 + 1, (size_t)m0 + 1 + nrows));
    h->d_row_ptr = h->d_csr_rp;
    SC_TRY(grow_graph(h->d_csr_ci, (size_t)E0, (size_t)E0 + add));
    h->d_col_idx = h->d_csr_ci;
    SC_TRY(grow_graph(h->d_prior_buf, (size_t)n0, (size_t)new_n));
    h->d_prior = h->d_prior_buf;

    h->hg_row_ptr.reserve((size_t)m0 + 1 + nrows);
    for (int r = 0; r < nrows; r++) h->hg_row_ptr.push_back((int)(E0 + row_ptr[r + 1]));
    h->hg_col_idx.insert(h->hg_col_idx.end(), col_idx, col_idx + add);
    h->hg_cdeg.resize(new_n, 0);
    for (int r = 0; r < nrows; r++) h->max_row_deg = std::max(h->max_row_deg, row_ptr[r + 1] - row_ptr[r]);

    TMARK("app:mirror");
    const bool had_tables = h->d_el_tab;
    pvec<int> &dirty_slot = h->el_dirty_slot, &dirty_col = h->el_dirty_col;
    dirty_slot.clear();
    dirty_col.clear();
    bool el_alive = had_tables;
    if (had_tables) {
        h->seg_slot.resize(new_n, -1);
        h->seg_cap.resize(new_n, 0);
    }
    auto set_slot = [&](size_t i, int v) {
        h->h_el_slots[i] = v;
        dirty_slot.push_back((int)i);
    };
    auto new_segment = [&](int c, int cap, const int *edges, int d) {
        const int s0 = el_alloc_segment(h, cap), start = s0 & 63;
        for (int k = 0; k < cap; k++) {
            set_slot(2 * (size_t)(s0 + k), k < d ? edges[k] : -1);
            set_slot(2 * (size_t)(s0 + k) + 1, el_tag(start, k, cap, true));
        }
        h->h_el_col[s0] = c;
        dirty_col.push_back(s0);
        h->seg_slot[c] = s0;
        h->seg_cap[c] = (unsigned char)cap;
    };
    int edges_tmp[64];
    for (long i = 0; i < add; i++) {
        const int c = col_idx[i], e = (int)(E0 + i);
        const int d_old = h->hg_cdeg[c]++;
        h->max_col_deg = std::max(h->max_col_deg, d_old + 1);
        if (!el_alive) continue;
        if (d_old + 1 > 64) {
            el_alive = false;
            continue;
        }
        if (h->seg_slot[c] < 0) {
            edges_tmp[0] = e;
            new_segment(c, std::min(64, 1 + el_slack(h, c, 1)), edges_tmp, 1);
        } else if (d_old < h->seg_cap[c]) {
            set_slot(2 * (size_t)(h->seg_slot[c] + d_old), e);
        } else {
            const int s_old = h->seg_slot[c];
            for (int k = 0; k < d_old; k++) edges_tmp[k] = h->h_el_slots[2 * (size_t)(s_old + k)];
            edges_tmp[d_old] = e;
            for (int k = 0; k < d_old; k++) set_slot(2 * (size_t)(s_old + k), -1);
            set_slot(2 * (size_t)s_old + 1, 0);
            new_segment(c, std::min(64, d_old + 1 + std::max(el_slack(h, c, d_old + 1), (d_old + 1) / 2)), edges_tmp, d_old + 1);
        }
    }
    if (el_alive)
        for (int c = n0; c < new_n; c++)
            if (h->seg_slot[c] < 0) new_segment(c, 1, edges_tmp, 0);

    h->m = m0 + nrows;
    h->n = new_n;
    h->E = E0 + add;
    h->el_ok = h->E > 0 && h->max_row_deg <= ROW_CAP && h->max_col_deg <= 64;
    if (had_tables && (!el_alive || !h->el_ok)) {
        h->d_el_tab.reset();
        h->d_el_slots = h->d_el_slot_col = nullptr;
        el_alive = false;
    }

    TMARK("app:tables");
    const bool reupload = el_alive && h->el_waves > h->el_cap_bins;
    const size_t npairs = (el_alive && !reupload) ? dirty_slot.size() + dirty_col.size() : 0;
    const size_t stage_ints = (size_t)nrows + add + 2 * npairs;
    if (stage_ints > h->d_pairs.cap()) {
        h->h_pairs.reset();
        h->d_pairs.reset();
        const size_t want = stage_ints + stage_ints / 2 + 1024;
        SC_TRY(h->h_pairs.ensure(want));
        SC_TRY(h->d_pairs.ensure(want));
    }
    int *st = h->h_pairs;
    for (int r = 0; r < nrows; r++) st[r] = (int)(E0 + row_ptr[r + 1]);
    std::copy(col_idx, col_idx + add, st + nrows);
    if (nrows) SC_HIP(hipMemcpyAsync(h->d_row_ptr + m0 + 1, st, sizeof(int) * nrows, hipMemcpyHostToDevice, s));
    if (add) SC_HIP(hipMemcpyAsync(h->d_col_idx + E0, st + nrows, sizeof(int) * add, hipMemcpyHostToDevice, s));
    if (reupload) {
        SC_TRY(el_upload(h));
    } else if (npairs) {
        int *pp = st + nrows + add;
        const int col_base = (int)el_col_off(h);
        size_t q = 0;
        for (int i : dirty_slot) {
            pp[2 * q] = i;
            pp[2 * q + 1] = h->h_el_slots[i];
            q++;
        }
        for (int i : dirty_col) {
            pp[2 * q] = col_base + i;
            pp[2 * q + 1] = h->h_el_col[i];
            q++;
        }
        SC_HIP(hipMemcpyAsync(h->d_pairs, pp, sizeof(int) * 2 * npairs, hipMemcpyHostToDevice, s));
        hipLaunchKernelGGL(k_apply_pairs, dim3((unsigned)((npairs + 255) / 256)), dim3(256), 0, s, h->d_el_tab,
                           (const int2 *)h->d_pairs.get(), (int)npairs);
        LAUNCH_CHECK();
    }
    SC_HIP(hipStreamSynchronize(s));
    TMARK("app:device");

    h->full_stale = true;
    h->h_probs.resize(new_n, 0.0);
    h->thr_valid = false;
    h->first_valid = false;
    h->settle_next = 0;
    h->ratio_valid = false;
    h->d_x64.reset();
    h->d_c64.reset();
    h->d_post64.reset();
    h->d_thr.reset();
    h->d_msg.reset();
    h->d_scratch.reset();
    h->cap_group = 0;
    h->d_rec.reset();
    h->d_mask.reset();
    h->cap_rec_group = 0;
    for (auto &L : h->lv) {
        L.synd.reset(); L.hard.reset(); L.done.reset(); L.conv.reset(); L.unsat.reset();
        L.iters.reset(); L.ids.reset(); L.post.reset(); L.pprior.reset(); L.pratio64.reset();
        L.cap_tiles = 0;
    }
    h->last_group = 0;
    TMARK("app:tail");
    unfinished.done = true;
    return 0;
}

int scaldpc_bp_last_compacted(scaldpc_bp *h, int64_t *count)
{
    if (!h || !count) return fail(SCALDPC_EINVAL, "NULL argument");
    std::lock_guard<std::mutex> lk(h->mu);
    *count = h->stat_deferred;
    return 0;
}

int scaldpc_bp_last_stats(scaldpc_bp *h, int64_t *out)
{
    if (!h || !out) return fail(SCALDPC_EINVAL, "NULL argument");
    std::lock_guard<std::mutex> lk(h->mu);
    out[0] = h->stat_deferred;
    out[1] = h->stat_el;
    out[2] = h->stat_levels;
    out[3] = 0;
    return 0;
}

int scaldpc_bp_last_schedule(scaldpc_bp *h, int64_t *out)
{
    if (!h || !out) return fail(SCALDPC_EINVAL, "NULL argument");
    std::lock_guard<std::mutex> lk(h->mu);
    for (int i = 0; i < SCHED_WORDS; i++) out[i] = h->sched.w[i];
    for (int i = SCHED_WORDS; i < SCALDPC_SCHEDULE_WORDS; i++) out[i] = 0;
    return 0;
}

int scaldpc_bp_last_settle(scaldpc_bp *h, int32_t *frozen_at, int32_t cap, int64_t *info)
{
    if (!h || !info || cap < 0 || (cap > 0 && !frozen_at)) return fail(SCALDPC_EINVAL, "bad argument");
    std::lock_guard<std::mutex> lk(h->mu);
    const size_t T = h->settle_frozen_at.size();
    for (size_t t = 0; t < T && t < (size_t)cap; t++) frozen_at[t] = h->settle_frozen_at[t];
    info[0] = (int64_t)T;
    info[1] = h->settle_saved;
    info[2] = h->settle_rerun;
    info[3] = h->settle_K;
    return 0;
}

int scaldpc_bp_set_tile_group(scaldpc_bp *h, int32_t tiles)
{
    if (!h || tiles < 0) return fail(SCALDPC_EINVAL, "bad tile group");
    std::lock_guard<std::mutex> lk(h->mu);
    h->tile_group = tiles;
    return 0;
}

static int size_call(scaldpc_bp *h, DecodeCall &c, int prob_cols)
{
    if (prob_cols > 0 && h->tile_group <= 0) {
        int cols = prob_cols;
        if (!c.early && rec_form(h, c.method)) {
            cols = 0;
            for (int v = h->n - prob_cols; v < h->n; v++) cols += h->hg_cdeg[v] > 1;
        }
        c.G = auto_group(h, c.T, cols);
    }
    return ensure_workspace(h, c.T, c.G, c.want_post, c.max_iter, prob_cols);
}

static int decode_batch_impl(scaldpc_bp *h, const uint8_t *in, int32_t input_kind, int32_t batch, const float *probs,
                             int32_t prob_cols, int32_t max_iter_arg, int32_t method, float alpha, uint32_t flags, void *stream,
                             uint8_t *out_bits, float *out_llr, int32_t *out_iters, uint8_t *out_conv)
{
    if (!h || !in || !out_bits) return fail(SCALDPC_EINVAL, "NULL argument");
    if (batch <= 0) return fail(SCALDPC_EINVAL, "batch must be positive (got %d)", batch);
    if (input_kind != SCALDPC_IN_SYNDROME && input_kind != SCALDPC_IN_RECEIVED)
        return fail(SCALDPC_EINVAL, "unknown input kind %d", input_kind);
    if (method != SCALDPC_BP_PRODUCT_SUM && method != SCALDPC_BP_MIN_SUM)
        return fail(SCALDPC_EINVAL, "unknown bp method %d", method);
    if (!(alpha >= 0.0f)) return fail(SCALDPC_EINVAL, "ms_scaling_factor must be >= 0");
    std::lock_guard<std::mutex> lk(h->mu);
    SC_TRY(check_usable(h));
    if (prob_cols > h->n) return fail(SCALDPC_EINVAL, "prob_cols = %d exceeds the block length n = %d", prob_cols, h->n);
    DeviceGuard dg(h->device);
    DecodeCall c;
    SC_TRY(begin_call(h, batch, max_iter_arg, stream, &c));
    const bool dev_io = flags & SCALDPC_F_DEVICE_IO;
    const bool early = flags & SCALDPC_F_EARLY_EXIT;
    if ((flags & SCALDPC_F_ASYNC) && (!dev_io || early))
        return fail(SCALDPC_EINVAL, "SCALDPC_F_ASYNC needs DEVICE_IO and no EARLY_EXIT (early exit polls the device)");
    if (flags & SCALDPC_F_ASYNC) h->async_used = true;
    c.method = method;
    c.alpha = alpha;
    c.early = early;
    c.want_post = out_llr != nullptr;
    c.no_sync = (flags & SCALDPC_F_ASYNC) != 0;
    CacheBypass guard(h->async_used);
    const hipStream_t s = c.s;
    SyncOnError settle{s};
    const int T = c.T, max_iter = c.max_iter;
    const int len = input_kind == SCALDPC_IN_SYNDROME ? h->m : h->n;
    const Outputs out{out_bits, out_llr, out_iters, out_conv};
    Outputs dev;
    const bool soft = prob_cols > 0;
    const int first_col = h->n - prob_cols;
    if (soft && !dev_io)
        for (size_t i = 0, cnt = (size_t)batch * prob_cols; i < cnt; i++)
            if (!(probs[i] >= 0.0f && probs[i] <= 1.0f))
                return fail(SCALDPC_EINVAL, "channel_probs[%zu][%zu] = %g is not a probability (codeword %zu, column %zu)",
                            i / prob_cols, i % prob_cols, (double)probs[i], i / prob_cols, first_col + i % prob_cols);

    const size_t lds = small_lds(h);
    if (h->full_stale && (lds || !(T == 1 && batch <= el_limit(h, method))))
        SC_TRY(refresh_full(h));
    if (h->kn.path == Knobs::LDS && !lds)
        return fail(SCALDPC_EINVAL, "SCALDPC_PATH=lds but the graph needs %zu B of LDS", small_lds_bytes(h));
    auto soft_convert = [&]() -> int {
        const float *dp = probs;
        const size_t cnt = (size_t)batch * prob_cols;
        if (!dev_io) {
            SC_TRY(grow(h->d_probs_in, cnt));
            SC_HIP(hipMemcpyAsync(h->d_probs_in, probs, sizeof(float) * cnt, hipMemcpyHostToDevice, s));
            dp = h->d_probs_in;
        }
        SC_TRY(h->d_soft_bad.ensure(1));
        SC_HIP(hipMemsetAsync(h->d_soft_bad, 0xff, sizeof(u64), s));
        hipLaunchKernelGGL(k_soft_convert, dim3((prob_cols + 63) / 64, T), dim3(256), 0, s, dp, prob_cols, batch, h->d_pprior.get(),
                           h->d_soft_bad.get());
        LAUNCH_CHECK();
        return 0;
    };
    auto soft_verdict = [&]() -> int {
        u64 bad = ~0ull;
        SC_HIP(hipMemcpyAsync(&bad, h->d_soft_bad, sizeof(u64), hipMemcpyDeviceToHost, s));
        SC_HIP(hipStreamSynchronize(s));
        if (bad != ~0ull)
            return fail(SCALDPC_EINVAL, "channel_probs[%llu][%llu] is not a probability (codeword %llu, column %llu)", bad / prob_cols,
                        bad % prob_cols, bad / prob_cols, first_col + bad % prob_cols);
        return 0;
    };
    if (lds) {
        const uint8_t *din = in;
        SC_TRY(stage_input(h, in, (size_t)batch * len, dev_io, s, &din));
        SC_TRY(stage_outputs(h, out, batch, dev_io, true, &dev));
        if (soft) {
            SC_TRY(grow(h->d_pprior, (size_t)T * prob_cols * TW));
            SC_TRY(soft_convert());
        }
        SC_TRY(launch_small<false>(h, lds, method, batch, din, input_kind, max_iter, alpha, early, dev.bits, dev.llr, dev.iters,
                                   dev.conv, s, soft ? h->d_pprior.get() : nullptr, first_col));
        SC_TRY(copy_outputs(h, out, dev, batch, dev_io, s));
        h->stat_deferred = 0;
        if (soft && !(flags & SCALDPC_F_ASYNC)) SC_TRY(soft_verdict());
        if (!(flags & SCALDPC_F_ASYNC)) SC_HIP(hipStreamSynchronize(s));
        return settle.done();
    }
    SC_TRY(size_call(h, c, prob_cols));
    if (soft) SC_TRY(soft_convert());
    const float *const pprior = soft ? h->d_pprior.get() : nullptr;

    if (!dev_io && T == 1 && batch <= 8 && max_iter <= 1024) {
        const size_t bits_bytes = ((size_t)batch * h->n + 3) / 4 * 4;
        const size_t out_bytes = bits_bytes + (out_llr ? sizeof(float) * (size_t)batch * h->n : 0) + sizeof(int) * batch + batch;
        const size_t in_bytes = (size_t)batch * len, io_bytes = std::max(in_bytes, out_bytes);
        SC_TRY(h->h_io.ensure(io_bytes, io_bytes + io_bytes / 2));
        SC_TRY(grow(h->d_in, in_bytes));
        SC_TRY(grow(h->d_out_all, out_bytes));
        SC_TRY(ensure_el_unsat(h, max_iter));
        memcpy(h->h_io, in, in_bytes);
        SC_HIP(hipMemcpyAsync(h->d_in, h->h_io, in_bytes, hipMemcpyHostToDevice, s));
        const bool recvd = input_kind == SCALDPC_IN_RECEIVED;
        hipLaunchKernelGGL(k_small_prepare, dim3((std::max(len, h->n) + 63) / 64), dim3(256), 0, s, h->d_in, len, batch,
                           recvd ? h->d_recv : h->d_synd, h->n, h->d_hard, max_iter, h->d_done, h->d_conv, h->d_iters,
                           h->d_remaining, max_iter + 2, h->d_el_unsat, (max_iter + 2) * TW);
        LAUNCH_CHECK();
        if (recvd) SC_TRY(launch_syndrome(h, h->d_recv, h->d_synd, 1, s));
        c.state_ready = true;
        SC_TRY(run_core(h, c, pprior, first_col));
        hipLaunchKernelGGL(k_small_unpack, dim3((h->n + 255) / 256), dim3(256), 0, s, h->d_hard, recvd ? h->d_recv : (const u64 *)nullptr,
                           out_llr ? h->d_post : (const float *)nullptr, h->d_conv, h->d_iters, h->n, batch, h->d_out_all);
        LAUNCH_CHECK();
        SC_HIP(hipMemcpyAsync(h->h_io, h->d_out_all, out_bytes, hipMemcpyDeviceToHost, s));
        SC_HIP(hipStreamSynchronize(s));
        const uint8_t *o = h->h_io;
        memcpy(out_bits, o, (size_t)batch * h->n);
        o += bits_bytes;
        if (out_llr) {
            memcpy(out_llr, o, sizeof(float) * (size_t)batch * h->n);
            o += sizeof(float) * (size_t)batch * h->n;
        }
        if (out_iters) memcpy(out_iters, o, sizeof(int) * batch);
        if (out_conv) memcpy(out_conv, o + sizeof(int) * batch, batch);
        return settle.done();
    }

    const uint8_t *din = in;
    SC_TRY(stage_input(h, in, (size_t)batch * len, dev_io, s, &din));
    if (input_kind == SCALDPC_IN_SYNDROME) {
// ... 838 lines not shown
```

### sca-ldpc_amd/csrc/scaldpc_bp_kernels.h

```cpp
#pragma once
#include "scaldpc_logf.h"
#include "scaldpc_mc_law.h"
#include "scaldpc_philox.h"
#include "scaldpc_mc_draw.h"
#include "scaldpc_rec_pack.h"
#include "scaldpc_rec_trim.h"
#include <type_traits>

extern "C" __device__ int scaldpc_llvm_writelane(int src, int lane, int old) __asm("llvm.amdgcn.writelane.i32");

namespace {

__device__ __forceinline__ unsigned writelane(unsigned src, int lane, unsigned old)
{
    return (unsigned)scaldpc_llvm_writelane((int)src, lane, (int)old);
}

constexpr int TW = 64;
constexpr int MAXB = 8;
constexpr int ROW_CAP = 64;
#ifndef REC_CHUNK
#define REC_CHUNK 8
#endif

// ... 435 lines not shown
    const u64 *bt = ft.hard + (size_t)t * ft.n;
    u64 bad = 0;
    constexpr int IL = 4;
    const int rend = min(r0 + ROWS_PER_WAVE, m);
    for (int rb = r0; rb < rend; rb += IL) {
        u64 a[IL];
        int ea[IL], eb[IL];
#pragma unroll
        for (int i = 0; i < IL; i++) {
            const int r = min(rb + i, rend - 1);
            ea[i] = rfl(row_ptr[r]) + lane;
            eb[i] = rb + i < rend ? rfl(row_ptr[r + 1]) : 0;
        }
#pragma unroll
        for (int i = 0; i < IL; i++) a[i] = ea[i] < eb[i] ? bt[col_idx[ea[i]]] : 0ull;
#pragma unroll
        for (int i = 0; i < IL; i++)
            for (int e = ea[i] + 64; e < eb[i]; e += 64) a[i] ^= bt[col_idx[e]];
#pragma unroll
        for (int i = 0; i < IL; i++) {
            const int r = rb + i;
            if (r >= rend) break;
            u64 x = a[i];
#pragma unroll
            for (int off = 32; off >= 1; off >>= 1) x ^= __shfl_xor(x, off);
            bad |= x ^ synd[(size_t)t * m + r];
        }
    }
    fused_commit(ft, t, bad, dw);
}

template <class P>
__device__ __forceinline__ void init_msg_body(const int *__restrict__ col_idx, P pr, float *__restrict__ msg, long E)
{
    const int lane = threadIdx.x & 63;
    const long e = (long)blockIdx.x * 4 + (threadIdx.x >> 6);
    if (e >= E) return;
    msg[((size_t)blockIdx.y * E + e) * TW + lane] = pr(col_idx[e], blockIdx.y, lane);
}
template <class P>
__global__ __launch_bounds__(256) void k_init_msg(const int *__restrict__ col_idx, float *__restrict__ msg, long E,
                                                  typename P::Arg prior_arg)
{
    init_msg_body(col_idx, P{prior_arg}, msg, E);
}

template <bool FIRST, class P>
__device__ __forceinline__ void check_minsum_body(const int *__restrict__ row_ptr, float *msg,
                                                  const u64 *__restrict__ synd, const u64 *__restrict__ done,
                                                  int skip_done, int m, long E, float alpha,
                                                  const int *__restrict__ col_idx, P prior)
{
    const int lane = threadIdx.x & 63;
    const int r = rfl((int)blockIdx.x * 4 + (int)(threadIdx.x >> 6));
    if (r >= m) return;
    const int tl = blockIdx.y;
    if (skip_done && done[tl] == ~0ull) return;
    const int e0 = row_ptr[r];
    const int deg = row_ptr[r + 1] - e0;
    float *p = msg + ((size_t)tl * E + e0) * TW + lane;
    unsigned par = (unsigned)(synd[(size_t)tl * m + r] >> lane) & 1u;
    float m1 = FLT_MAX, m2 = FLT_MAX;
    int ix = 0;
#pragma unroll 16
    for (int k = 0; k < deg; k++) {
        const float x = FIRST ? prior(rfl(col_idx[e0 + k]), tl, lane) : p[(size_t)k * TW];
        const float a = fabsf(x);
        const unsigned n_ = x <= 0.0f;
        par ^= n_;
        const bool lt = a < m1;
        m2 = lt ? m1 : ((a < m2) ? a : m2);
        ix = lt ? k : ix;
        m1 = lt ? a : m1;
    }
    const float nalpha = -alpha;
#pragma unroll 8
    for (int k = 0; k < deg; k++) {
        const unsigned b = (unsigned)((FIRST ? prior(rfl(col_idx[e0 + k]), tl, lane) : p[(size_t)k * TW]) <= 0.0f);
        p[(size_t)k * TW] = ((k == ix) ? m2 : m1) * ((par ^ b) ? nalpha : alpha);
    }
}
template <bool FIRST, class P>
__global__ __launch_bounds__(256) void k_check_minsum(const int *__restrict__ row_ptr, float *msg,
                                                      const u64 *__restrict__ synd, const u64 *__restrict__ done,
                                                      int skip_done, int m, long E, float alpha,
                                                      const int *__restrict__ col_idx, typename P::Arg prior_arg)
{
    check_minsum_body<FIRST>(row_ptr, msg, synd, done, skip_done, m, E, alpha, col_idx, P{prior_arg});
}

template <int DEG, bool FIRST, class P>
__device__ __forceinline__ void check_minsum_row(float *p, unsigned par, float alpha, P prior, const int *__restrict__ cidx,
                                                 int tl, int lane)
{
    float x[DEG];
#pragma unroll
    for (int k = 0; k < DEG; k++) x[k] = FIRST ? prior(rfl(cidx[k]), tl, lane) : p[(size_t)k * TW];
    float m1 = FLT_MAX, m2 = FLT_MAX;
    int ix = 0;
#pragma unroll
    for (int k = 0; k < DEG; k++) {
        const float a = fabsf(x[k]);
        par ^= (unsigned)(x[k] <= 0.0f);
        const bool lt = a < m1;
        m2 = lt ? m1 : ((a < m2) ? a : m2);
        ix = lt ? k : ix;
        m1 = lt ? a : m1;
    }
    const float nalpha = -alpha;
#pragma unroll
    for (int k = 0; k < DEG; k++)
        p[(size_t)k * TW] = ((k == ix) ? m2 : m1) * ((par ^ (unsigned)(x[k] <= 0.0f)) ? nalpha : alpha);
}

template <int CAP, bool FIRST, bool PAR, class P>
__global__ __launch_bounds__(256) void k_check_minsum_x(const int *__restrict__ list, float *msg,
                                                        const u64 *__restrict__ synd, const u64 *done,
                                                        int skip_done, int m, long E, float alpha,
                                                        const int *__restrict__ col_idx, typename P::Arg prior_arg,
                                                        FusedTest ft)
{
    const P prior{prior_arg};
    const int lane = threadIdx.x & 63;
    const int tl = blockIdx.y;
    const int *md = list + (size_t)rfl((int)blockIdx.x * 4 + (int)(threadIdx.x >> 6)) * 4;
    u64 dw = 0;
    if constexpr (PAR) {
        dw = done[tl];
        if (skip_done && dw == ~0ull) return;
    } else {
        if (skip_done && done[tl] == ~0ull) return;
    }
    const int r = md[0];
    u64 bad = 0;
    if constexpr (PAR) bad = fused_row_parity(ft, tl, r, md[1], md[2], col_idx, synd, m);
    if (!PAR && r < 0) return;
    if (r >= 0) {
        const int e0 = md[1];
        const int deg = md[2];
        float *p = msg + ((size_t)tl * E + e0) * TW + lane;
        const unsigned sbit = (unsigned)(synd[(size_t)tl * m + r] >> lane) & 1u;
        for_exact_degree<CAP>(deg, [&](auto d) { check_minsum_row<d, FIRST>(p, sbit, alpha, prior, col_idx + e0, tl, lane); });
    }
    if constexpr (PAR) fused_commit(ft, tl, bad, dw);
}

constexpr unsigned REC_NO_ARG = 255;
static_assert(REC_TW == TW, "the record layout of scaldpc_rec_pack.h is laid out for the kernels' tile width");

constexpr int SETTLE_WORDS = 32, SETTLE_SHARDS = 8;
struct Settle {
    unsigned *words = nullptr;
    int done = 0, mark = 0;
};
__device__ __forceinline__ bool settle_frozen(const unsigned *__restrict__ w, int done)
{
    unsigned mx = 0;
#pragma unroll
    for (int i = 0; i < SETTLE_SHARDS; i++) mx = w[i] > mx ? w[i] : mx;
    return (int)mx < done;
}

template <int DEG, bool BOOT>
__device__ __forceinline__ void check_minsum_row_rec(const float *p, u64 synd_mask, float alpha, float *__restrict__ rec,
                                                     float *__restrict__ rec2, unsigned char *__restrict__ arg,
                                                     u64 *__restrict__ sgn, int lane, const int *__restrict__ pos,
                                                     bool const_last = false, float x_last = 0.0f,
                                                     unsigned *mark_word = nullptr, unsigned mark = 0, u64 real = 0)
{
    int mp = 0;
    if constexpr (BOOT)
        if (lane < DEG) mp = pos[lane];
    float x[DEG];
#pragma unroll
    for (int k = 0; k < DEG - 1; k++) x[k] = p[(size_t)k * TW];
    if (const_last)
        x[DEG - 1] = x_last;
    else
        x[DEG - 1] = p[(size_t)(DEG - 1) * TW];
    constexpr bool EARLY = DEG <= 32;
    bool tracked = false;
    if constexpr (!BOOT) tracked = mark_word != nullptr;
    unsigned o1 = 0, o2 = 0, oa = 0;
    if constexpr (!BOOT && EARLY)
        if (tracked) {
            o1 = __float_as_uint(rec[lane]);
            o2 = __float_as_uint(rec2[lane]);
            oa = arg[lane];
        }
    float m1 = FLT_MAX, m2 = FLT_MAX;
    const float fmax = FLT_MAX;
    u64 par = ((u64)(unsigned)rfl((int)(synd_mask >> 32)) << 32) | (unsigned)rfl((int)synd_mask);
#pragma unroll
    for (int k = 0; k < DEG; k++) {
        if (k % REC_CHUNK == 0 && k > 0) {
            asm volatile("" : "+s"(par));
#pragma unroll
            for (int j = k; j < DEG && j < k + REC_CHUNK; j++) asm volatile("" : "+v"(x[j]));
        }
        par ^= __ballot(x[k] <= 0.0f);
        float a;
        asm("v_min_f32 %0, |%1|, %2" : "=v"(a) : "v"(x[k]), "v"(fmax));
        asm("v_med3_f32 %0, %1, %2, %0" : "+v"(m2) : "v"(a), "v"(m1));
        asm("v_min_f32 %0, %0, %1" : "+v"(m1) : "v"(a));
    }
    float s1, s2;
    {
        const bool odd = __builtin_amdgcn_inverse_ballot_w64(par);
        const float r1 = m1 * alpha, r2 = m2 * alpha;
        s1 = odd ? -r1 : r1;
        s2 = odd ? -r2 : r2;
    }
    if (!tracked || EARLY) {
        rec[lane] = s1;
        rec2[lane] = s2;
    }
    constexpr int AT = DEG - 8;
    unsigned idx = REC_NO_ARG;
#pragma unroll
    for (int k = DEG - 1; k >= 0; k--) {
        asm("" : "+v"(x[k]) : "v"(idx));
        idx = (fabsf(x[k]) == m1) ? (unsigned)k : idx;
        if constexpr (!BOOT && !EARLY)
            if (k == AT && tracked) {
                int lo = lane;
                asm volatile("" : "+v"(lo) : "v"(idx));
                o1 = __float_as_uint(rec[lo]);
                o2 = __float_as_uint(rec2[lo]);
                rec[lo] = s1;
                rec2[lo] = s2;
            }
    }
    if constexpr (!BOOT) {
        if (tracked) {
            if constexpr (!EARLY) oa = arg[lane];
            arg[lane] = (unsigned char)idx;
            const bool changed = o1 != __float_as_uint(s1) || o2 != __float_as_uint(s2) || oa != idx;
            if ((__ballot(changed) & real) != 0 && lane == 0) *mark_word = mark;
        } else
            arg[lane] = (unsigned char)idx;
    } else
        arg[lane] = (unsigned char)idx;
    if constexpr (BOOT) {
        unsigned nlo = 0, nhi = 0;
#pragma unroll
        for (int k = 0; k < DEG; k++) {
            if (k % REC_CHUNK == 0) {
                asm volatile("" ::"v"(nlo), "v"(nhi));
#pragma unroll
                for (int j = k; j < DEG && j < k + REC_CHUNK; j++) asm volatile("" : "+v"(x[j]));
            }
            const u64 ng = __ballot(x[k] <= 0.0f);
            nlo = writelane((unsigned)ng, k, nlo);
            nhi = writelane((unsigned)(ng >> 32), k, nhi);
        }
        if (lane < DEG) sgn[mp] = ((u64)nhi << 32) | nlo;
    }
}

template <int CAP, bool BOOT, bool PAR = false>
__global__ __launch_bounds__(256) void k_check_minsum_rec(const int *__restrict__ list, const float *msg,
                                                          const u64 *__restrict__ synd, const u64 *done,
                                                          int skip_done, int m, long E, float alpha,
                                                          const int *__restrict__ col_idx,
                                                          float *__restrict__ rec, u64 *__restrict__ sgn,
                                                          const int *__restrict__ csr_pos,
                                                          const float *__restrict__ const_prior, FusedTest ft = FusedTest{},
                                                          Settle st = Settle{})
{
    const int lane = threadIdx.x & 63;
    const int tl = blockIdx.y;
    const int *md = list + (size_t)rfl((int)blockIdx.x * 4 + (int)(threadIdx.x >> 6)) * 4;
    u64 dw = 0;
    unsigned *mark_word = nullptr;
    if constexpr (PAR) {
        dw = done[tl];
        if (skip_done && dw == ~0ull) return;
    } else {
        if (skip_done && done[tl] == ~0ull) return;
        if (st.words) {
            unsigned *w = st.words + (size_t)tl * SETTLE_WORDS;
            if (settle_frozen(w, st.done)) return;
            if (!BOOT && st.mark) {
                mark_word = w + (blockIdx.x & (SETTLE_SHARDS - 1));
                dw = done[tl];
            }
        }
    }
    const int r = md[0];
    u64 bad = 0;
    if constexpr (PAR) bad = fused_row_parity(ft, tl, r, md[1], md[2], col_idx, synd, m);
    if (!PAR && r < 0) return;
    if (r >= 0) {
        const int e0 = md[1];
        const int deg = md[2];
        const float *p = msg + ((size_t)tl * E + e0) * TW + lane;
        float *rt = rec + (size_t)tl * rec_tile_floats(m);
        float *rc = rt + rec_row_off(r), *rc2 = rc + rec_m2_off(m);
        unsigned char *ar = (unsigned char *)(rt + rec_arg_off(m)) + (size_t)r * TW;
        u64 *sg = sgn + (size_t)tl * E;
        const int *ps = csr_pos + e0;
        const u64 sw = synd[(size_t)tl * m + r];
        const bool cl = const_prior != nullptr && (md[3] & REC_CONST_LAST) != 0;
        float xl = 0.0f;
        if (cl) xl = const_prior[rec_desc_col(md[3])];
#define MR(D)                                                                                                   \
    case D:                                                                                                     \
        if constexpr (D <= CAP)                                                                                 \
            check_minsum_row_rec<D, BOOT>(p, sw, alpha, rc, rc2, ar, sg, lane, ps, cl, xl, mark_word, (unsigned)st.mark, ~dw); \
        break;
#define MR8(D) MR(D) MR(D + 1) MR(D + 2) MR(D + 3) MR(D + 4) MR(D + 5) MR(D + 6) MR(D + 7)
        switch (deg) {
            MR(1) MR(2) MR(3) MR(4) MR(5) MR(6) MR(7)
            MR8(8) MR8(16) MR8(24) MR8(32) MR8(40) MR8(48) MR8(56)
            MR(64)
            default: break;
        }
#undef MR8
#undef MR
    }
    if constexpr (PAR) fused_commit(ft, tl, bad, dw);
}

__device__ __forceinline__ float tanh_compl(float a)
{
    return 2.0f * __builtin_amdgcn_rcpf(__builtin_amdgcn_exp2f(a * 1.44269504088896340736f) + 1.0f);
}
__device__ __forceinline__ float llr_from_compl(float U)
{
    return __builtin_amdgcn_logf(fmaf(2.0f, __builtin_amdgcn_rcpf(U), -1.0f)) * 0.69314718055994530942f;
}
__device__ __forceinline__ float compl_step(float U, float u) { return fmaf(u, 1.0f - U, U); }

template <int DEG, bool FIRST, class P>
__device__ __forceinline__ void check_tanh_row(float *p, unsigned sbit, P prior, const int *__restrict__ cidx, int tl, int lane)
{
    float uu[DEG], pre[DEG];
#pragma unroll
    for (int k = 0; k < DEG; k++) uu[k] = FIRST ? prior(rfl(cidx[k]), tl, lane) : p[(size_t)k * TW];
    unsigned acc = sbit << 31;
    float U = 0.0f;
#pragma unroll
    for (int k = 0; k < DEG; k++) {
        const unsigned xb = __float_as_uint(uu[k]);
        acc ^= xb;
        const float u = tanh_compl(fabsf(uu[k]));
        uu[k] = __uint_as_float(__float_as_uint(u) | (xb & 0x80000000u));
        pre[k] = U;
        U = compl_step(U, u);
    }
    U = 0.0f;
#pragma unroll
    for (int k = DEG - 1; k >= 0; k--) {
        const float Ut = compl_step(pre[k], U);
        const float Lm = llr_from_compl(Ut);
        const unsigned sg = (acc ^ __float_as_uint(uu[k])) & 0x80000000u;
        U = compl_step(U, fabsf(uu[k]));
        p[(size_t)k * TW] = __uint_as_float(__float_as_uint(Lm) ^ sg);
    }
}

__device__ __forceinline__ void check_tanh_row_generic(float *p, float *sc, int deg, unsigned sbit)
{
    float U = 0.0f;
    unsigned par = sbit;
    for (int k = 0; k < deg; k++) {
        const float x = p[(size_t)k * TW];
        sc[(size_t)k * TW] = U;
        par ^= (unsigned)(x < 0.0f);
        const float u = tanh_compl(fabsf(x));
        U = compl_step(U, u);
    }
    U = 0.0f;
    for (int k = deg - 1; k >= 0; k--) {
        const float x = p[(size_t)k * TW];
        const float pk = sc[(size_t)k * TW];
        const float Ut = compl_step(pk, U);
        const float Lm = llr_from_compl(Ut);
        p[(size_t)k * TW] = ((par ^ (unsigned)(x < 0.0f)) & 1u) ? -Lm : Lm;
        const float u = tanh_compl(fabsf(x));
        U = compl_step(U, u);
    }
}

template <int CAP, bool FIRST, bool PAR, class P>
__global__ __launch_bounds__(256) void k_check_tanh(const int *__restrict__ list, float *msg, float *scratch,
                                                    const u64 *__restrict__ synd, const u64 *done,
                                                    int skip_done, int m, long E, const int *__restrict__ col_idx,
                                                    typename P::Arg prior_arg, FusedTest ft)
{
    const P prior{prior_arg};
    const int lane = threadIdx.x & 63;
    const int tl = blockIdx.y;
    const int *md = list + (size_t)rfl((int)blockIdx.x * 4 + (int)(threadIdx.x >> 6)) * 4;
    u64 dw = 0;
    if constexpr (PAR) {
        dw = done[tl];
        if (skip_done && dw == ~0ull) return;
    } else {
        if (skip_done && done[tl] == ~0ull) return;
    }
    const int r = md[0];
    u64 bad = 0;
    if constexpr (PAR) bad = fused_row_parity(ft, tl, r, md[1], md[2], col_idx, synd, m);
    if (!PAR && r < 0) return;
    if (r >= 0) {
        const int e0 = md[1];
        const int deg = md[2];
        const size_t base = ((size_t)tl * E + e0) * TW + lane;
        float *p = msg + base;
        const unsigned sbit = (unsigned)(synd[(size_t)tl * m + r] >> lane) & 1u;
        if (md[3] == 0)
            check_tanh_row_generic(p, scratch + base, deg, sbit);
        else
            for_exact_degree<CAP>(deg, [&](auto d) { check_tanh_row<d, FIRST>(p, sbit, prior, col_idx + e0, tl, lane); });
    }
    if constexpr (PAR) fused_commit(ft, tl, bad, dw);
}

template <int METHOD, bool PLANES, class P>
__device__ __forceinline__ void bp_small_body(const int *__restrict__ row_ptr, const int *__restrict__ col_idx,
                                              const int *__restrict__ col_ptr, const int *__restrict__ csc_edge,
                                              P prior, int m, int n, int E,
                                              const void *__restrict__ in_, int kind, int max_iter, float alpha0,
                                              int early, void *__restrict__ out_bits_,
                                              float *__restrict__ out_llr, int *__restrict__ out_iters,
                                              void *__restrict__ out_conv_)
{
    const uint8_t *in = (const uint8_t *)in_;
    uint8_t *out_bits = (uint8_t *)out_bits_;
    uint8_t *out_conv = (uint8_t *)out_conv_;
    const u64 *in_planes = (const u64 *)in_;
    u64 *hard_planes = (u64 *)out_bits_;
    u64 *conv_planes = (u64 *)out_conv_;
    extern __shared__ float sm[];
    float *msg = sm, *scr = sm + E;
    uint8_t *hard = (uint8_t *)(scr + E);
    uint8_t *synd = hard + n;
    uint8_t *recv = synd + m;
    __shared__ int flag;
    const int b = blockIdx.x, tid = threadIdx.x, nt = blockDim.x;
    const int pt = b >> 6, pc = b & 63;

    if (PLANES) {
        for (int r = tid; r < m; r += nt) synd[r] = (uint8_t)((in_planes[(size_t)pt * m + r] >> pc) & 1);
    } else if (kind == SCALDPC_IN_SYNDROME) {
        for (int r = tid; r < m; r += nt) synd[r] = in[(size_t)b * m + r] & 1;
    } else {
        for (int v = tid; v < n; v += nt) recv[v] = in[(size_t)b * n + v] & 1;
        __syncthreads();
        for (int r = tid; r < m; r += nt) {
            uint8_t p = 0;
            for (int e = row_ptr[r]; e < row_ptr[r + 1]; e++) p ^= recv[col_idx[e]];
            synd[r] = p;
        }
    }
    for (int e = tid; e < E; e += nt) msg[e] = prior(col_idx[e], pt, pc);
    for (int v = tid; v < n; v += nt) hard[v] = 0;
    __syncthreads();

    int it_done = max_iter, conv = 0;
    for (int it = 1; it <= max_iter; it++) {
// ... 217 lines not shown
        temp += mt[o];
    }
    float suf = 0.0f;
    for (int k = d - 1; k >= 0; k--) {
        const size_t o = (size_t)ce[k] * TW;
        const float mk = mt[o];
        mt[o] = st[o] + suf;
        suf += mk;
    }
    return temp;
}

struct RecWide {
    const int *var_rows = nullptr, *csc_row = nullptr;
    const float *rec = nullptr;
    u64 *sgn = nullptr;
    int m = 0, blk0 = 0, xmap = 0;
    int last = 0;
    Settle stl = Settle{};
};
template <class P>
__device__ __forceinline__ void var_rec_wide_wave(const int *__restrict__ list, const int *__restrict__ csc_edge, const P &prior,
                                                  float *msg, float *__restrict__ post, u64 *__restrict__ hard,
                                                  const u64 *__restrict__ done, int skip_done, int n, long E, int write_out,
                                                  const RecWide &rw);

template <int CAP, class P>
__global__ __launch_bounds__(256) void k_var(const int *__restrict__ list, const int *__restrict__ csc_edge,
                                             typename P::Arg prior_arg, float *msg, float *scratch,
                                             float *__restrict__ post, u64 *__restrict__ hard,
                                             const u64 *__restrict__ done, int skip_done, int n, long E,
                                             int write_out, RecWide rw = RecWide{})
{
    const P prior{prior_arg};
    if constexpr (CAP >= 64)
        if (rw.rec) {
            var_rec_wide_wave(list, csc_edge, prior, msg, post, hard, done, skip_done, n, E, write_out, rw);
            return;
        }
    const int lane = threadIdx.x & 63;
    const int tl = blockIdx.y;
    const int *rec = list + (size_t)rfl((int)blockIdx.x * 4 + (int)(threadIdx.x >> 6)) * VAR_REC;
    const u64 dn = done[tl];
    if (skip_done && dn == ~0ull) return;
    const int v = rec[0];
    if (v < 0) return;
    const int cb = rec[1];
    const int d = rec[2];
    float *mt = msg + (size_t)tl * E * TW + lane;
    const int *ce = csc_edge + cb;
    const float pr = prior(v, tl, lane);
    float L = pr;
    {
        float *tb = msg + (size_t)tl * E * TW;
        const unsigned ul = threadIdx.x & 63u;
        const int4 *r4 = (const int4 *)rec;
        switch (rec[3]) {
            case 1: L = var_col_s<1>(tb, ul, r4, ce, d, pr); break;
            case 2: L = var_col_s<2>(tb, ul, r4, ce, d, pr); break;
            case 4: L = var_col_s<4>(tb, ul, r4, ce, d, pr); break;
            case 8: L = var_col_s<8>(tb, ul, r4, ce, d, pr); break;
            case 16: L = var_col_s<16>(tb, ul, r4, ce, d, pr); break;
            case 32:
                if constexpr (CAP >= 32) L = var_col_s<32>(tb, ul, r4, ce, d, pr);
                break;
            case 64:
                if constexpr (CAP >= 64) L = var_col_s<64>(tb, ul, r4, ce, d, pr);
                break;
            default: L = var_col_generic(mt, scratch + (size_t)tl * E * TW + lane, ce, d, pr);
        }
    }
    if (write_out) {
        const u64 hb = __ballot(L <= 0.0f);
        const size_t hi = (size_t)tl * n + v;
        if (lane == 0) hard[hi] = (hard[hi] & dn) | (hb & ~dn);
        if (post && !((dn >> lane) & 1)) post[hi * TW + lane] = L;
    }
}
template <int CAP>
__global__ __launch_bounds__(256) void k_var_first(const int *__restrict__ list, const int *__restrict__ csc_edge,
                                                   const float *__restrict__ prior, float *msg, float *__restrict__ post,
                                                   u64 *__restrict__ hard, const u64 *__restrict__ done, int skip_done, int n,
                                                   long E, int write_out, const int2 *__restrict__ first_tab,
                                                   const u64 *__restrict__ synd, int m, int nrec)
{
    const unsigned lane = threadIdx.x & 63u;
    const int tl = blockIdx.y;
    const int r0 = 2 * rfl((int)blockIdx.x * 4 + (int)(threadIdx.x >> 6));
    if (r0 >= nrec) return;
    const u64 dn = done[tl];
    if (skip_done && dn == ~0ull) return;
    float *tb = msg + (size_t)tl * E * TW;
    const u64 *st = synd + (size_t)tl * m;
    const int *rec[2] = {list + (size_t)r0 * VAR_REC, list + (size_t)(r0 + 1) * VAR_REC};
    int v[2], cb[2], d[2];
    int2 f[2];
    u64 wv[2];
    float pr[2];
#pragma unroll
    for (int j = 0; j < 2; j++) {
        v[j] = rec[j][0];
        cb[j] = rec[j][1];
        d[j] = v[j] < 0 ? 0 : rec[j][2];
        f[j] = make_int2(0, 0);
        if ((int)lane < d[j]) f[j] = first_tab[(size_t)cb[j] + lane];
    }
#pragma unroll
    for (int j = 0; j < 2; j++) {
        wv[j] = st[f[j].y];
        pr[j] = prior[v[j] < 0 ? 0 : v[j]];
    }
#pragma unroll
    for (int j = 0; j < 2; j++) {
        if (v[j] < 0) continue;
        const int4 *r4 = (const int4 *)rec[j];
        const int *ce = csc_edge + cb[j];
        float L = pr[j];
        switch (rec[j][3]) {
            case 1: L = var_col_first<1>(tb, lane, r4, ce, f[j], wv[j], d[j], pr[j]); break;
            case 2: L = var_col_first<2>(tb, lane, r4, ce, f[j], wv[j], d[j], pr[j]); break;
            case 4: L = var_col_first<4>(tb, lane, r4, ce, f[j], wv[j], d[j], pr[j]); break;
            case 8: L = var_col_first<8>(tb, lane, r4, ce, f[j], wv[j], d[j], pr[j]); break;
            case 16: L = var_col_first<16>(tb, lane, r4, ce, f[j], wv[j], d[j], pr[j]); break;
            case 32:
                if constexpr (CAP >= 32) L = var_col_first<32>(tb, lane, r4, ce, f[j], wv[j], d[j], pr[j]);
                break;
            case 64:
                if constexpr (CAP >= 64) L = var_col_first<64>(tb, lane, r4, ce, f[j], wv[j], d[j], pr[j]);
                break;
            default: break;
        }
        if (write_out) {
            const u64 hb = __ballot(L <= 0.0f);
            const size_t hi = (size_t)tl * n + v[j];
            if (lane == 0) hard[hi] = (hard[hi] & dn) | (hb & ~dn);
            if (post && !((dn >> lane) & 1)) post[hi * TW + lane] = L;
        }
    }
}

typedef __attribute__((address_space(1))) unsigned char gbyte;
__device__ __forceinline__ gbyte *sbase_b(const unsigned char *p)
{
    gbyte *g = (gbyte *)p;
    asm("" : "+s"(g));
    return g;
}

template <int D, bool LAST>
__device__ __forceinline__ float var_col_rec(float *tile_base, const float *__restrict__ rec_base, unsigned rec2_off,
                                             const unsigned char *__restrict__ arg_base, u64 *sgn_col, unsigned lane,
                                             const int *__restrict__ rc, const int4 *__restrict__ row4,
                                             const int *__restrict__ ce1, const int *__restrict__ cr1, float pr,
                                             unsigned *mark_word = nullptr, unsigned mark = 0, u64 real = 0)
{
    int eid[D], rw[D];
    {
        const int4 ra = row4[0], rb = row4[1], rc4 = row4[2], re = row4[3];
        const int rw16[16] = {ra.x, ra.y, ra.z, ra.w, rb.x, rb.y, rb.z, rb.w, rc4.x, rc4.y, rc4.z, rc4.w, re.x, re.y, re.z, re.w};
#pragma unroll
        for (int k = 0; k < D && k < VAR_INLINE; k++) rw[k] = rw16[k];
#pragma unroll
        for (int k = VAR_INLINE; k < D; k++) rw[k] = cr1[k];
    }
    u64 sg = 0;
    if ((int)lane < D) sg = sgn_col[lane];
    const int slo = (int)(unsigned)sg, shi = (int)(unsigned)(sg >> 32);
    float mm[D], pp[D];
    unsigned ab[D];
#pragma unroll
    for (int k = 0; k < D; k++) ab[k] = sbase_b(arg_base + (size_t)rec_row_of(rfl(rw[k])) * TW)[lane];
    const unsigned off1 = lane * 4u, off2 = off1 + rec2_off;
#pragma unroll
    for (int k = 0; k < D; k++) {
        const unsigned off = ab[k] == (unsigned)rec_index_of(rfl(rw[k])) ? off2 : off1;
        mm[k] = *(const gfloat *)((const gbyte *)sbase(rec_base + (size_t)rec_row_of(rfl(rw[k])) * TW) + off);
    }
#pragma unroll
    for (int k = 0; k < D; k++) {
        const u64 ng = ((u64)(unsigned)__builtin_amdgcn_readlane(shi, k) << 32) | (unsigned)__builtin_amdgcn_readlane(slo, k);
        mm[k] = __builtin_amdgcn_inverse_ballot_w64(ng) ? -mm[k] : mm[k];
    }
    if constexpr (LAST) {
        float sum = pr;
#pragma unroll
        for (int k = 0; k < D; k++) sum += mm[k];
        return sum;
    }
    {
        const int4 *rec4 = (const int4 *)rc;
        const int4 a = rec4[1], b = rec4[2], c = rec4[3], e = rec4[4];
        const int in16[16] = {a.x, a.y, a.z, a.w, b.x, b.y, b.z, b.w, c.x, c.y, c.z, c.w, e.x, e.y, e.z, e.w};
#pragma unroll
        for (int k = 0; k < D && k < VAR_INLINE; k++) eid[k] = in16[k];
    }
    float temp = pr;
#pragma unroll
    for (int k = 0; k < D; k++) {
        pp[k] = temp;
        temp += mm[k];
    }
#pragma unroll
    for (int k = VAR_INLINE; k < D; k++) eid[k] = ce1[k];
    float suf = 0.0f;
    unsigned nlo = 0, nhi = 0;
#pragma unroll
    for (int k = D - 1; k >= 0; k--) {
        gfloat *q = sbase(tile_base + (size_t)rfl(eid[k]) * TW) + lane;
        const float out = pp[k] + suf;
        __hip_atomic_store(q, out, __ATOMIC_RELAXED, __HIP_MEMORY_SCOPE_AGENT);
        const u64 nm = __ballot(out <= 0.0f);
        nlo = writelane((unsigned)nm, k, nlo);
        nhi = writelane((unsigned)(nm >> 32), k, nhi);
        suf += mm[k];
    }
    if ((int)lane < D) sgn_col[lane] = ((u64)nhi << 32) | nlo;
    if (mark_word) {
        const unsigned dlo = (nlo ^ (unsigned)slo) & (unsigned)real, dhi = (nhi ^ (unsigned)shi) & (unsigned)(real >> 32);
        if (__ballot((int)lane < D && (dlo | dhi) != 0) != 0 && lane == 0) *mark_word = mark;
    }
    return temp;
}

template <bool LAST>
__device__ __forceinline__ float var_col_rec_wide(float *tile_base, const float *__restrict__ rec_base, unsigned rec2_off,
                                                  const unsigned char *__restrict__ arg_base, u64 *sgn_col, unsigned lane,
                                                  const int *__restrict__ rc, const int4 *__restrict__ row4,
                                                  const int *__restrict__ ce1, const int *__restrict__ cr1, int d, float pr,
                                                  unsigned *mark_word = nullptr, unsigned mark = 0, u64 real = 0)
{
    constexpr int W = 64, CH = 16, SURE = 32;
    u64 sg = 0;
    if ((int)lane < d) sg = sgn_col[lane];
    const int slo = (int)(unsigned)sg, shi = (int)(unsigned)(sg >> 32);
    const unsigned off1 = lane * 4u, off2 = off1 + rec2_off;
    float mm[W];
    float sum = pr;
#pragma unroll
    for (int c = 0; c < W / CH; c++) {
        if (c * CH >= SURE && c * CH >= d) break;
        int rw[CH];
        if (c == 0) {
            const int4 ra = row4[0], rb = row4[1], rc4 = row4[2], re = row4[3];
            const int rw16[16] = {ra.x, ra.y, ra.z, ra.w, rb.x, rb.y, rb.z, rb.w, rc4.x, rc4.y, rc4.z, rc4.w, re.x, re.y, re.z, re.w};
#pragma unroll
            for (int k = 0; k < CH; k++) rw[k] = rw16[k];
        } else {
#pragma unroll
            for (int k = 0; k < CH; k++) rw[k] = cr1[c * CH + k];
        }
        unsigned ab[CH];
#pragma unroll
        for (int k = 0; k < CH; k++)
            if (c * CH + k < SURE || c * CH + k < d) ab[k] = sbase_b(arg_base + (size_t)rec_row_of(rfl(rw[k])) * TW)[lane];
#pragma unroll
        for (int k = 0; k < CH; k++)
            if (c * CH + k < SURE || c * CH + k < d) {
                const unsigned off = ab[k] == (unsigned)rec_index_of(rfl(rw[k])) ? off2 : off1;
                mm[c * CH + k] = *(const gfloat *)((const gbyte *)sbase(rec_base + (size_t)rec_row_of(rfl(rw[k])) * TW) + off);
            }
#pragma unroll
        for (int k = 0; k < CH; k++)
            if (c * CH + k < SURE || c * CH + k < d) {
                const int e = c * CH + k;
                const u64 ng = ((u64)(unsigned)__builtin_amdgcn_readlane(shi, e) << 32) | (unsigned)__builtin_amdgcn_readlane(slo, e);
                mm[e] = __builtin_amdgcn_inverse_ballot_w64(ng) ? -mm[e] : mm[e];
                if constexpr (LAST) sum += mm[e];
            }
    }
    if constexpr (LAST) return sum;
    float pp[W];
    float temp = pr;
#pragma unroll
    for (int k = 0; k < W; k++)
        if (k < SURE || k < d) {
            pp[k] = temp;
            temp += mm[k];
        }
    float suf = 0.0f;
    unsigned nlo = 0, nhi = 0;
#pragma unroll
    for (int c = W / CH - 1; c >= 0; c--) {
        if (c * CH >= SURE && c * CH >= d) continue;
        int eid[CH];
        if (c == 0) {
            const int4 *rec4 = (const int4 *)rc;
            const int4 a = rec4[1], b = rec4[2], c4 = rec4[3], e4 = rec4[4];
            const int in16[16] = {a.x, a.y, a.z, a.w, b.x, b.y, b.z, b.w, c4.x, c4.y, c4.z, c4.w, e4.x, e4.y, e4.z, e4.w};
#pragma unroll
            for (int k = 0; k < CH; k++) eid[k] = in16[k];
        } else {
#pragma unroll
            for (int k = 0; k < CH; k++) eid[k] = ce1[c * CH + k];
        }
#pragma unroll
        for (int k = CH - 1; k >= 0; k--)
            if (c * CH + k < SURE || c * CH + k < d) {
                const int e = c * CH + k;
                gfloat *q = sbase(tile_base + (size_t)rfl(eid[k]) * TW) + lane;
                const float out = pp[e] + suf;
                __hip_atomic_store(q, out, __ATOMIC_RELAXED, __HIP_MEMORY_SCOPE_AGENT);
                const u64 nm = __ballot(out <= 0.0f);
                nlo = writelane((unsigned)nm, e, nlo);
                nhi = writelane((unsigned)(nm >> 32), e, nhi);
                suf += mm[e];
            }
    }
    if ((int)lane < d) sgn_col[lane] = ((u64)nhi << 32) | nlo;
    if (mark_word) {
        const unsigned dlo = (nlo ^ (unsigned)slo) & (unsigned)real, dhi = (nhi ^ (unsigned)shi) & (unsigned)(real >> 32);
        if (__ballot((int)lane < d && (dlo | dhi) != 0) != 0 && lane == 0) *mark_word = mark;
    }
    return temp;
}

template <class P>
__device__ __forceinline__ void var_rec_wide_wave(const int *__restrict__ list, const int *__restrict__ csc_edge, const P &prior,
                                                  float *msg, float *__restrict__ post, u64 *__restrict__ hard,
                                                  const u64 *__restrict__ done, int skip_done, int n, long E, int write_out,
                                                  const RecWide &rw)
{
    const unsigned lane = threadIdx.x & 63u;
    int tl = blockIdx.y, bx = blockIdx.x;
    if (rw.xmap) {
        const unsigned G = gridDim.y, L = blockIdx.y * gridDim.x + blockIdx.x, xcd = L & 7u, slot = L >> 3;
        tl = (int)(xcd % G);
        bx = (int)(slot * (8u / G) + xcd / G);
        if (bx >= rw.xmap) return;
    }
    const int ri = rfl((bx + rw.blk0) * 4 + (int)(threadIdx.x >> 6));
    const int *rc = list + (size_t)ri * VAR_REC;
    const u64 dn = done[tl];
    if (skip_done && dn == ~0ull) return;
    const bool last = rw.last != 0;
    unsigned *mark_word = nullptr;
    bool decided = false;
    if (rw.stl.words) {
        unsigned *w = rw.stl.words + (size_t)tl * SETTLE_WORDS;
        const bool frozen = settle_frozen(w, rw.stl.done);
        if (last)
            decided = frozen;
        else {
            if (frozen) return;
            if (rw.stl.mark) mark_word = w + ((unsigned)bx & (SETTLE_SHARDS - 1));
        }
    }
    const int v = rc[0];
    if (v < 0) return;
    const int cb = rc[1];
    const int d = rc[2];
    if (d <= 32 || d > 64) return;
    if (last && decided) return;
    float *tb = msg + (size_t)tl * E * TW;
    const float *rb = rw.rec + (size_t)tl * rec_tile_floats(rw.m);
    const unsigned char *ab = (const unsigned char *)(rb + rec_arg_off(rw.m));
    u64 *st = rw.sgn + (size_t)tl * E;
    const int *ce = csc_edge + cb, *cr = rw.csc_row + cb;
    const int4 *w4 = (const int4 *)(rw.var_rows + (size_t)ri * VAR_INLINE);
    const float pr = prior(v, tl, (int)lane);
    const unsigned r2 = (unsigned)rw.m * (TW * (unsigned)sizeof(float));
    const float L = last ? var_col_rec_wide<true>(tb, rb, r2, ab, st + cb, lane, rc, w4, ce, cr, d, pr)
                         : var_col_rec_wide<false>(tb, rb, r2, ab, st + cb, lane, rc, w4, ce, cr, d, pr, mark_word,
                                                   (unsigned)rw.stl.mark, ~dn);
    if (write_out) {
        const u64 hb = __ballot(L <= 0.0f);
        const size_t hi = (size_t)tl * n + v;
        if (dn == 0) {
            if (lane == 0) hard[hi] = hb;
        } else if (lane == 0)
            hard[hi] = (hard[hi] & dn) | (hb & ~dn);
        if (post && !((dn >> lane) & 1)) post[hi * TW + lane] = L;
    }
}

template <int CAP, class P, bool LAST = false>
__global__ __launch_bounds__(256) void k_var_rec(const int *__restrict__ list, const int *__restrict__ var_rows,
                                                 const int *__restrict__ csc_edge, const int *__restrict__ csc_row,
                                                 typename P::Arg prior_arg, float *msg, const float *__restrict__ rec,
                                                 u64 *sgn, float *__restrict__ post,
                                                 u64 *__restrict__ hard, const u64 *__restrict__ done, int skip_done, int n, int m,
                                                 long E, int write_out, int blk0, int xmap, Settle stl = Settle{})
{
    const P prior{prior_arg};
    const unsigned lane = threadIdx.x & 63u;
    int tl = blockIdx.y, bx = blockIdx.x;
    if (xmap) {
        const unsigned G = gridDim.y, L = blockIdx.y * gridDim.x + blockIdx.x, xcd = L & 7u, slot = L >> 3;
        tl = (int)(xcd % G);
        bx = (int)(slot * (8u / G) + xcd / G);
        if (bx >= xmap) return;
    }
    const int ri = rfl((bx + blk0) * 4 + (int)(threadIdx.x >> 6));
    const int *rc = list + (size_t)ri * VAR_REC;
    const u64 dn = done[tl];
    if (skip_done && dn == ~0ull) return;
    unsigned *mark_word = nullptr;
    bool decided = false;
    if (stl.words) {
        unsigned *w = stl.words + (size_t)tl * SETTLE_WORDS;
        const bool frozen = settle_frozen(w, stl.done);
        if constexpr (LAST)
            decided = frozen;
        else {
            if (frozen) return;
            if (stl.mark) mark_word = w + ((unsigned)bx & (SETTLE_SHARDS - 1));
        }
    }
    const int v = rc[0];
    if (v < 0) return;
    const int cb = rc[1];
    const int d = rc[2];
    if (LAST && decided && d > 1) return;
    float *tb = msg + (size_t)tl * E * TW;
    const float *rb = rec + (size_t)tl * rec_tile_floats(m);
    const unsigned char *ab = (const unsigned char *)(rb + rec_arg_off(m));
    u64 *st = sgn + (size_t)tl * E;
    const int *ce = csc_edge + cb, *cr = csc_row + cb;
    const int4 *w4 = (const int4 *)(var_rows + (size_t)ri * VAR_INLINE);
    const float pr = prior(v, tl, (int)lane);
    float L = pr;
    const unsigned r2 = (unsigned)m * (TW * (unsigned)sizeof(float));
#define VR(D)                                                                                                \
    case D:                                                                                                  \
        if constexpr (D <= CAP)                                                                              \
            L = var_col_rec<D, LAST>(tb, rb, r2, ab, st + cb, lane, rc, w4, ce, cr, pr, mark_word, (unsigned)stl.mark, ~dn); \
        break;
#define VR8(D) VR(D) VR(D + 1) VR(D + 2) VR(D + 3) VR(D + 4) VR(D + 5) VR(D + 6) VR(D + 7)
    switch (d) {
        VR(1) VR(2) VR(3) VR(4) VR(5) VR(6) VR(7)
        VR8(8) VR8(16) VR8(24) VR(32)
        default: break;
    }
#undef VR8
#undef VR
    if (write_out) {
        const u64 hb = __ballot(L <= 0.0f);
        const size_t hi = (size_t)tl * n + v;
        if (dn == 0) {
            if (lane == 0) hard[hi] = hb;
        } else if (lane == 0)
            hard[hi] = (hard[hi] & dn) | (hb & ~dn);
        if (post && !((dn >> lane) & 1)) post[hi * TW + lane] = L;
    }
}
__device__ __forceinline__ float wave_min_f(float v)
{
#pragma unroll
    for (int off = 32; off >= 1; off >>= 1) v = fminf(v, __shfl_xor(v, off));
    return v;
}
__device__ __forceinline__ float readlane_f(float v, int l)
{
    return __int_as_float(__builtin_amdgcn_readlane(__float_as_int(v), l));
}

template <int METHOD, bool FIRST, class P>
__global__ __launch_bounds__(256) void k_el_check(const int *__restrict__ row_ptr, const int *__restrict__ col_idx,
                                                  typename P::Arg prior_arg, float *emsg,
                                                  const u64 *__restrict__ synd, const u64 *__restrict__ done,
                                                  int skip_done, int m, long E, float alpha,
                                                  const u64 *__restrict__ hard, int *__restrict__ unsat_prev)
{
    const P prior{prior_arg};
    const int lane = threadIdx.x & 63;
    int r = blockIdx.x * 4 + (threadIdx.x >> 6);
    if (r >= m) return;
    r = rfl(r);
    const int c = blockIdx.y;
    if (skip_done && ((done[0] >> c) & 1)) return;
    const int e0 = rfl(row_ptr[r]);
    const int deg = rfl(row_ptr[r + 1]) - e0;
    const bool act = lane < deg;
    const unsigned sbit = (unsigned)(synd[r] >> c) & 1u;
    if (unsat_prev) {
        const unsigned hb = act ? (unsigned)(hard[col_idx[e0 + lane]] >> c) & 1u : 0u;
        if ((((unsigned)__popcll(__ballot(hb != 0u)) & 1u) ^ sbit) && lane == 0) unsat_prev[c] = 1;
    }
    if (deg == 0) return;
    float *p = emsg + (size_t)c * E + e0 + lane;
    float x = 0.0f;
    if (act) x = FIRST ? prior(col_idx[e0 + lane], 0, c) : *p;
    if (METHOD == SCALDPC_BP_MIN_SUM) {
        const float a = act ? fminf(fabsf(x), FLT_MAX) : FLT_MAX;
        const bool ng = act && x <= 0.0f;
        const unsigned par = sbit ^ ((unsigned)__popcll(__ballot(ng)) & 1u);
        const float m1 = wave_min_f(a);
        const int ix = __ffsll((long long)__ballot(act && a == m1)) - 1;
        const float m2 = wave_min_f(lane == ix ? FLT_MAX : a);
        if (act) *p = ((lane == ix) ? m2 : m1) * ((par ^ (unsigned)ng) ? -alpha : alpha);
    } else {
        const unsigned xb = act ? __float_as_uint(x) : 0u;
        const float u = act ? tanh_compl(fabsf(x)) : 0.0f;
        const unsigned par = sbit ^ ((unsigned)__popcll(__ballot((xb >> 31) != 0u)) & 1u);
        float pre = 0.0f, suf = 0.0f;
#pragma unroll 4
        for (int t = 0; t < deg; t++) {
            const float nv = compl_step(pre, readlane_f(u, t));
            pre = (t < lane) ? nv : pre;
        }
#pragma unroll 4
        for (int t = deg - 1; t >= 0; t--) {
            const float nv = compl_step(suf, readlane_f(u, t));
            suf = (t > lane) ? nv : suf;
        }
        const float Lm = llr_from_compl(compl_step(pre, suf));
        const unsigned sg = ((par << 31) ^ xb) & 0x80000000u;
        if (act) *p = __uint_as_float(__float_as_uint(Lm) ^ sg);
    }
}
template <class P>
__device__ __forceinline__ void el_var_body(const int2 *__restrict__ slots, const int *__restrict__ slot_col,
                                            int nwaves, P prior, float *emsg,
                                            float *__restrict__ post, u64 *__restrict__ hard,
                                            u64 *done, int skip_done, long E, int write_out,
                                            const int *__restrict__ unsat_prev, int it_prev, u64 *conv,
                                            int *__restrict__ iters, int *__restrict__ remaining_prev)
{
    const int lane = threadIdx.x & 63;
    int w = blockIdx.x * 4 + (threadIdx.x >> 6);
    if (w >= nwaves) return;
    w = rfl(w);
    const int c = blockIdx.y;
    const bool frozen = (done[0] >> c) & 1;
    if (skip_done && frozen) return;
    if (unsat_prev) {
        const bool newly = !frozen && unsat_prev[c] == 0;
        if (newly) {
            if (w == 0 && lane == 0) {
                atomicOr(done, 1ull << c);
                atomicOr(conv, 1ull << c);
                iters[c] = it_prev;
            }
            return;
        }
        if (w == 0 && lane == 0 && !frozen) atomicAdd(remaining_prev, 1);
    }
    const int2 sl = slots[(size_t)w * 64 + lane];
    const int e = sl.x, start = sl.y & 63, pos = (sl.y >> 6) & 63, cap = ((sl.y >> 12) & 63) + 1;
    const bool live = (sl.y >> 18) & 1;
    const bool head = live && pos == 0;
    const u64 has = __ballot(e >= 0);
    const u64 segmask = (cap == 64 ? ~0ull : ((1ull << cap) - 1ull)) << start;
    const int deg = live ? __popcll(has & segmask) : 0;
    int dmax = deg;
#pragma unroll
    for (int off = 32; off >= 1; off >>= 1) dmax = max(dmax, __shfl_xor(dmax, off));
    dmax = rfl(dmax);
    float *mt = emsg + (size_t)c * E;
    const float mk = e >= 0 ? mt[e] : 0.0f;
    int v = 0;
    float pr = 0.0f;
    if (head) {
        v = slot_col[(size_t)w * 64 + lane];
        pr = prior(v, 0, c);
    }
    pr = __shfl(pr, start);
    float pre = pr, tot = pr, suf = 0.0f;
    for (int t = 0; t < dmax; t++) {
        const float val = __shfl(mk, (start + t) & 63);
        pre = (t < pos) ? pre + val : pre;
        tot = (t < deg) ? tot + val : tot;
    }
    for (int t = dmax - 1; t >= 0; t--) {
        const float val = __shfl(mk, (start + t) & 63);
        suf = (t > pos && t < deg) ? suf + val : suf;
    }
    if (e >= 0) mt[e] = pre + suf;
    if (write_out && head) {
        if (tot <= 0.0f)
            atomicOr(hard + v, 1ull << c);
        else
            atomicAnd(hard + v, ~(1ull << c));
        if (post) post[(size_t)v * TW + c] = tot;
    }
}
template <class P>
__global__ __launch_bounds__(256) void k_el_var(const int2 *__restrict__ slots, const int *__restrict__ slot_col,
                                                int nwaves, typename P::Arg prior_arg, float *emsg,
// ... 167 lines not shown
```

### sca-ldpc_amd/csrc/scaldpc_bp_sched.h

```cpp
#pragma once

#include <cstdint>

namespace scaldpc {

constexpr int SCHED_TW = 64;
constexpr int SCHED_MAX_LANES = 4;
constexpr int SCHED_MAX_LEVELS = 3;
constexpr int REM_SLOTS = 512;

constexpr int SPEC_PERIOD = 16;
constexpr int POLL_EVERY = 4;
struct PollState {
    int hint = 1, streak = 0, since_poll = 0;
};
inline bool poll_point(int it, int defer_after, const PollState &ps)
{
    return (it % POLL_EVERY == 0 || it == 1 || it == defer_after) && it >= ps.hint;
}
inline bool stops_unseen(int defer_after, int max_iter, const PollState &ps)
{
    return defer_after > 0 && 2 * defer_after < max_iter && ps.streak >= 2 && ps.since_poll < SPEC_PERIOD - 1 &&
           poll_point(defer_after, defer_after, ps);
}
// ... 8 lines not shown

inline int lanes_of(int split, int g)
{
    const int nl = split < g ? split : g;
    return nl < 1 ? 1 : nl > SCHED_MAX_LANES ? SCHED_MAX_LANES : nl;
}
inline void deal_tiles(int g, int nl, int *gs, int *t0)
{
    for (int k = 0, t = 0; k < nl; k++) {
        gs[k] = g / nl + (k < g % nl ? 1 : 0);
        t0[k] = t;
        t += gs[k];
    }
}

inline int defer_after_of(bool early, int lvl, int compact_after, int max_iter)
{
    int defer_after = 0;
    if (early && lvl < SCHED_MAX_LEVELS) {
        defer_after = 4;
        if (compact_after >= 0) defer_after = compact_after;
        if (max_iter <= 2 * defer_after) defer_after = 0;
    }
    return defer_after;
}

enum PollVerdict { POLL_DONE = 0, POLL_HAND_OVER = 1, POLL_GO_ON = 2 };
inline PollVerdict after_poll(PollState &ps, int it, int defer_after, int max_iter, int left, int real, int g, int el_lim)
{
    if (left == 0) return POLL_DONE;
    if (left >= real) ps.hint = ps.hint > it + 1 ? ps.hint : it + 1;
    const bool shrinks = (left + SCHED_TW - 1) / SCHED_TW < g || left <= el_lim;
    if (defer_after > 0 && it >= defer_after && 2 * it < max_iter && 2 * left <= real && shrinks) {
        ps.streak = (it == defer_after && 8 * left <= real) ? ps.streak + 1 : 0;
        ps.since_poll = 0;
        return POLL_HAND_OVER;
    }
    if (it >= defer_after) ps.streak = 0;
    return POLL_GO_ON;
}

inline int ring_rows_wanted(int T, int G)
{
    const int gg = G > 1 ? G : 1;
    const int groups = (T + gg - 1) / gg;
    const int want = 2 * groups + 8;
    return want < REM_SLOTS ? want : REM_SLOTS;
}
struct RemRing {
    int slot = 0, rows = 0;
};
inline int ring_take(RemRing &r, bool *clears)
{
    *clears = r.slot >= r.rows;
    if (*clears) r.slot = 1;
    return r.slot++;
}

inline int chain_bits(bool early, bool lanes2, bool full, bool first, bool next_full, bool lanes_open, int defer_after,
                      int max_iter, const PollState &ps, const RemRing &ring)
{
    int chain = 0;
    if (!lanes2 || !full) return 0;
    if (!early) {
        if (!first) chain |= 1;
        if (next_full) chain |= 2;
    } else if (runs_unseen(defer_after, max_iter, ps)) {
        PollState nxt = ps;
        note_unseen(nxt);
        if (lanes_open) chain |= 1;
        if (next_full && runs_unseen(defer_after, max_iter, nxt) && ring.slot + 2 < ring.rows) chain |= 2;
    }
    return chain;
}

inline bool phase_reestablished(int chain, int horizon, int max_iter)
{
    (void)chain;
    (void)horizon;
    (void)max_iter;
    return true;
}

enum SchedWord {
    SCHED_GROUPS = 0,
    SCHED_HANDED = 4,
    SCHED_POLLS = 7,
    SCHED_UNSEEN = 8,
    SCHED_CONTINUED = 9,
    SCHED_LEFT_OPEN = 10,
    SCHED_FIXED_CHAINED = 11,
    SCHED_CLEARS = 12,
    SCHED_OPEN_AT_CLEAR = 13,
    SCHED_RING_ROWS = 14,
    SCHED_EL_POLLS = 15,
    SCHED_RING_TAKES = 16,
    SCHED_WORDS = 17
};
struct SchedCounters {
    int64_t w[SCHED_WORDS] = {};
    bool ring_cleared = false;
    void reset() { *this = SchedCounters{}; }
    void note_take(bool clears, bool lanes_open)
    {
        w[SCHED_RING_TAKES]++;
        if (!clears) return;
        if (ring_cleared) w[SCHED_CLEARS]++;
        if (lanes_open) w[SCHED_OPEN_AT_CLEAR]++;
        ring_cleared = true;
    }
    void note_group(int lvl, bool early, int chain)
    {
        w[SCHED_GROUPS + lvl]++;
        if (early) {
            if (chain & 1) w[SCHED_CONTINUED]++;
            if (chain & 2) w[SCHED_LEFT_OPEN]++;
        } else if (chain & 1)
            w[SCHED_FIXED_CHAINED]++;
    }
};

constexpr int SETTLE_FIRST = 3;
inline int settle_first_test(int alpha_from)
{
    const int t = alpha_from + 1;
    return t < SETTLE_FIRST ? SETTLE_FIRST : t;
}
inline int settle_check_done(int it, int first_test) { return it - 1 >= first_test ? it - 1 : 0; }
inline int settle_check_mark(int it, int first_test, int last_test) { return it >= first_test && it <= last_test ? it : 0; }
inline int settle_var_done(int it, int first_test, int last_test) { return it >= first_test && it <= last_test ? it : 0; }
inline int settle_var_mark(int it, int first_test, int last_test) { return settle_check_mark(it + 1, first_test, last_test); }
inline int settle_frozen_at(int latest, int first_test, int last_test)
{
    if (last_test < first_test || latest >= last_test) return 0;
    return latest + 1 > first_test ? latest + 1 : first_test;
}
inline bool settle_horizon_usable(int K, int first_test, int max_iter) { return K >= first_test && K + 1 < max_iter; }
inline bool settle_enqueued(int it, int K, int max_iter) { return !(K && it > K && it < max_iter); }
inline bool settle_has_check(int it, int K, int max_iter) { return !(K && it == max_iter); }
inline bool settle_has_var(int it, int K) { return !(K && it == K); }
inline int settle_launches_saved(int K, int max_iter) { return 2 * (max_iter - K); }
inline int settle_next_horizon(int tiles, int frozen, int max_frozen_at, int rerun, int max_iter)
{
    if (tiles <= 0 || max_frozen_at <= 0) return 0;
    if (8 * rerun > tiles) return 0;
    const int K = max_frozen_at + 2;
    if (8 * frozen < 7 * tiles) return 0;
    if (2 * K >= max_iter) return 0;
    return K;
}

inline int settle_mode(int knob, bool identity_block) { return knob >= 0 ? knob : identity_block ? 2 : 0; }

struct RecVarSlices {
    int narrow0 = 0, narrow_n = 0, narrow_deg = 0, narrow_grid = 0;
    int wide0 = 0, wide_n = 0, wide_grid = 0;
    bool xmap = false;
};
inline RecVarSlices rec_var_slices(int nb, const int *maxd, const int *blk, bool var_reversed, bool light, bool write_out, int G,
                                   int max_col_deg)
{
    RecVarSlices r;
    const int nblk = blk[nb];
    const int n1 = (nb > 0 && maxd[0] == 1) ? blk[1] : 0;
    const bool slim = light && !write_out && n1 > 0 && n1 < nblk;
    r.wide_n = (nb > 0 && maxd[nb - 1] > 32) ? nblk - blk[nb - 1] : 0;
    r.narrow_deg = r.wide_n ? (nb > 1 ? maxd[nb - 2] : 0) : max_col_deg;
    r.narrow_n = (slim ? nblk - n1 : nblk) - r.wide_n;
    r.narrow0 = var_reversed ? r.wide_n : (slim ? n1 : 0);
    r.wide0 = var_reversed ? 0 : nblk - r.wide_n;
    r.xmap = G == 2 || G == 4 || G == 8;
    r.narrow_grid = r.xmap ? (r.narrow_n + 7) / 8 * 8 : r.narrow_n;
    r.wide_grid = r.xmap ? (r.wide_n + 7) / 8 * 8 : r.wide_n;
    return r;
}

inline bool el_poll_point(int ip) { return (ip >= 3 && ip <= 6) || (ip > 6 && ip <= 16 && ip % 2 == 0) || (ip > 16 && ip % 16 == 0); }

}
```

Before: 8378 billion directed edge-message updates/s.

## Skip unchanged check rows and variable columns via per-tile sparse dirty flags

Adds per-tile row and column change flags during the settle-tracking passes. A check row records which of its min/argmin outputs changed, and a variable column records whether its sign bits changed. On later passes, a check row whose neighbouring columns are all unchanged exits early, and so does a variable column whose rows did not change the relevant entries. The gating start iteration is learned from the earliest frozen iteration of the previous call. This removes redundant min-sum work once most of the graph has settled, at the cost of extra flag reads and writes and memsets. It is on by default when settle mode 2 is used with an identity block, which applies to this H=[Hin|I] workload.

```diff
diff --git a/include/scaldpc.h b/include/scaldpc.h
--- a/include/scaldpc.h
+++ b/include/scaldpc.h
@@ -62,6 +62,8 @@
 #define SCALDPC_SCHEDULE_WORDS 24
 int scaldpc_bp_last_schedule(scaldpc_bp *h, int64_t *out);
 int scaldpc_bp_last_settle(scaldpc_bp *h, int32_t *frozen_at, int32_t cap, int64_t *info);
+int scaldpc_bp_debug_sparse_flags(scaldpc_bp *h, int32_t tile, uint32_t *row_stamp, uint64_t *row_dirty, uint32_t *col_flag,
+                                  int64_t *info);
 int scaldpc_bp_configure(scaldpc_bp *h, const char *key, const char *value);
 int scaldpc_bp_device_of(scaldpc_bp *h, int32_t *out);
 void scaldpc_bp_destroy(scaldpc_bp *h);
diff --git a/profiles/settle_sparse/pass_means.py b/profiles/settle_sparse/pass_means.py
--- /dev/null
+++ b/profiles/settle_sparse/pass_means.py
@@ -0,0 +1,34 @@
+import collections
+import csv
+import re
+import sys
+
+
+def kind(name):
+    m = re.search(r"(k_\w+)(<[^>]*>)?", name)
+    if not m:
+        return name
+    k, t = m.group(1), m.group(2) or ""
+    if k == "k_var_rec":
+        return "var_last" if t.rstrip(">").endswith("true") else "var"
+    if k == "k_check_minsum_rec":
+        return "boot" if t.split(",")[1].strip() == "true" else "check"
+    return k
+
+
+rows = list(csv.DictReader(open(sys.argv[1])))
+ev = sorted((int(r["Start_Timestamp"]), int(r["End_Timestamp"]), r["Stream_Id"], kind(r["Kernel_Name"])) for r in rows)
+first = max(i for i, e in enumerate(ev) if e[3] == "k_pack_bits")
+ev = ev[first:]
+per = collections.defaultdict(list)
+count = {}
+for s, e, stream, k in ev:
+    if k == "k_var_first":
+        count[stream] = {"check": 0, "var": 0}
+    elif k in ("check", "var") and stream in count:
+        p = count[stream][k] + (3 if k == "check" else 2)
+        count[stream][k] += 1
+        per[(k, p)].append((e - s) / 1e3)
+print(sys.argv[1])
+for (k, p), v in sorted(per.items(), key=lambda kv: (kv[0][1], kv[0][0] == "var")):
+    print(f"  {k:5s} pass {p:2d}: {len(v):4d} launches, mean {sum(v) / len(v):6.2f} us, min {min(v):6.2f}, max {max(v):6.2f}")
diff --git a/sca-ldpc_amd/_lib.py b/sca-ldpc_amd/_lib.py
--- a/sca-ldpc_amd/_lib.py
+++ b/sca-ldpc_amd/_lib.py
@@ -67,6 +67,9 @@
     if hasattr(lib, "scaldpc_bp_last_settle"):
         lib.scaldpc_bp_last_settle.argtypes = [vp, p(C.c_int32), C.c_int32, p(C.c_int64)]
         lib.scaldpc_bp_last_settle.restype = C.c_int
+    if hasattr(lib, "scaldpc_bp_debug_sparse_flags"):
+        lib.scaldpc_bp_debug_sparse_flags.argtypes = [vp, C.c_int32, p(C.c_uint32), p(C.c_uint64), p(C.c_uint32), p(C.c_int64)]
+        lib.scaldpc_bp_debug_sparse_flags.restype = C.c_int
     lib.scaldpc_bp_append_rows.argtypes = [vp, C.c_int32, vp, vp, C.c_int32]
     lib.scaldpc_bp_append_rows.restype = C.c_int
     lib.scaldpc_bp_set_channel_probs_tail.argtypes = [vp, C.c_int32, C.c_int32, vp]
diff --git a/sca-ldpc_amd/bp.py b/sca-ldpc_amd/bp.py
--- a/sca-ldpc_amd/bp.py
+++ b/sca-ldpc_amd/bp.py
@@ -348,6 +348,24 @@
         _lib.check(self._lib.scaldpc_bp_last_settle(self._h, at, tiles, info))
         return {"frozen_at": [int(x) for x in at[:tiles]], "launches_saved": int(info[1]), "tiles_rerun": int(info[2]),
                 "horizon": int(info[3])}
+
+    def debug_sparse_flags(self):
+        info = (C.c_int64 * 4)()
+        _lib.check(self._lib.scaldpc_bp_debug_sparse_flags(self._h, 0, None, None, None, info))
+        tiles, m, n = (int(x) for x in info[:3])
+        out = []
+        for t in range(tiles):
+            rs, rd, cf = np.zeros(m, dtype=np.uint32), np.zeros(m, dtype=np.uint64), np.zeros(n, dtype=np.uint32)
+            _lib.check(self._lib.scaldpc_bp_debug_sparse_flags(
+                self._h, t, rs.ctypes.data_as(C.POINTER(C.c_uint32)), rd.ctypes.data_as(C.POINTER(C.c_uint64)),
+                cf.ctypes.data_as(C.POINTER(C.c_uint32)), info))
+            out.append({"row_stamp": rs, "row_dirty": rd, "col_flag": cf})
+        return out
+
+    def debug_sparse_start(self):
+        info = (C.c_int64 * 4)()
+        _lib.check(self._lib.scaldpc_bp_debug_sparse_flags(self._h, 0, None, None, None, info))
+        return int(info[3])
 
     def last_row_parallel(self):
         return self.last_stats()["row_parallel"]
diff --git a/sca-ldpc_amd/csrc/scaldpc_bp.hip b/sca-ldpc_amd/csrc/scaldpc_bp.hip
--- a/sca-ldpc_amd/csrc/scaldpc_bp.hip
+++ b/sca-ldpc_amd/csrc/scaldpc_bp.hip
@@ -65,6 +65,7 @@
     int minsum_rec = 1;
     int settle = -1;
     int settle_horizon = 0;
+    int settle_sparse = -1;
 };
 
 struct HandleStreams {
@@ -175,6 +176,10 @@
     PinnedBuf<int> h_rem64;
     bool ratio_valid = false;
     Buf<unsigned> d_settle;
+    Buf<uint4> d_rowf;
+    Buf<unsigned> d_colf;
+    int sparse_m = 0, sparse_n = 0, sparse_T = 0;
+    int sparse_start_next = 0, sparse_start = 0;
     PinnedBuf<unsigned> h_settle;
     int settle_next = 0;
     int settle_key_iter = 0, settle_key_soft = 0;
@@ -212,6 +217,7 @@
     else if (!strcmp(key, "fuse_test")) k.fuse_test = (int)x != 0;
     else if (!strcmp(key, "settle") && x >= -1 && x <= 2) k.settle = (int)x;
     else if (!strcmp(key, "settle_horizon") && x >= 0) k.settle_horizon = (int)x;
+    else if (!strcmp(key, "settle_sparse") && x >= -1 && x <= 1) k.settle_sparse = (int)x;
     else return false;
     return true;
 }
@@ -222,7 +228,8 @@
                                            {"SCALDPC_GROUP_MB", "group_mb"}, {"SCALDPC_EL_MAX", "el_max"},
                                            {"SCALDPC_COMPACT_AFTER", "compact_after"}, {"SCALDPC_FIRST_FUSED", "first_fused"},
                                            {"SCALDPC_FUSE_TEST", "fuse_test"}, {"SCALDPC_MINSUM_REC", "minsum_rec"},
-                                           {"SCALDPC_SETTLE", "settle"}, {"SCALDPC_SETTLE_HORIZON", "settle_horizon"}};
+                                           {"SCALDPC_SETTLE", "settle"}, {"SCALDPC_SETTLE_HORIZON", "settle_horizon"},
+                                           {"SCALDPC_SETTLE_SPARSE", "settle_sparse"}};
     for (auto &nm : names)
         if (const char *e = getenv(nm[0])) (void)set_knob(k, nm[1], e);
 }
@@ -957,6 +964,21 @@
     unsigned *words = nullptr;
     int first_test = 0, horizon = 0;
     unsigned *of(int tile) const { return words + (size_t)tile * SETTLE_WORDS; }
+    uint4 *rowf = nullptr;
+    unsigned *colf = nullptr;
+    int m = 0, n = 0;
+    int gate_start = 0;
+    Settle pass(int tile, int done, int mark, int gate) const
+    {
+        Settle s{of(tile), done, mark};
+        if (rowf && mark) {
+            s.rowf = rowf + (size_t)tile * m;
+            s.colf = colf + (size_t)tile * n;
+            s.ncol = n;
+            s.gate = gate;
+        }
+        return s;
+    }
 };
 int iterate_tiles(scaldpc_bp *h, const DecodeCall &c, Lanes &lanes, const TileState &st, int g0, int g, int defer_after,
                   bool *deferred, PollState &ps, int chain, const SettlePlan &sl)
@@ -988,6 +1010,7 @@
     bool verdict_pending[MAX_LANES] = {};
     const bool recf = rec_form(h, method);
     bool rec_booted[MAX_LANES] = {};
+    int boot_it[MAX_LANES] = {};
     const bool tracked = sl.words && recf && !early;
     const int K = tracked ? sl.horizon : 0, last_test = K ? K : max_iter;
     bool set_phase = phase_reestablished(chain, K, max_iter);
@@ -1010,9 +1033,11 @@
             }
             cp.boot = recf && !cp.first && !rec_booted[k];
             if (cp.boot) rec_booted[k] = true;
+            boot_it[k] = cp.boot ? it : boot_it[k];
             if (tracked)
-                cp.settle = Settle{sl.of(g0 + t0[k]), settle_check_done(it, sl.first_test),
-                                   cp.boot ? 0 : settle_check_mark(it, sl.first_test, last_test)};
+                cp.settle = sl.pass(g0 + t0[k], settle_check_done(it, sl.first_test),
+                                    cp.boot ? 0 : settle_check_mark(it, sl.first_test, last_test),
+                                    cp.boot ? 0 : settle_sparse_check_gate(it, sl.first_test, last_test, sl.gate_start));
             SC_TRY(launch_check(h, tv[k], gs[k], method, skip, lanes[k], cp));
             if (set_phase && k + 1 < nl) {
                 SC_HIP(hipEventRecord(h->ev_phase[k + 1], lanes[k]));
@@ -1031,8 +1056,9 @@
             vp.final_pass = last;
             vp.keep_hard = keep_hard && !last;
             if (tracked && !last)
-                vp.settle = Settle{sl.of(g0 + t0[k]), settle_var_done(it, sl.first_test, last_test),
-                                   settle_var_mark(it, sl.first_test, last_test)};
+                vp.settle = sl.pass(g0 + t0[k], settle_var_done(it, sl.first_test, last_test),
+                                    settle_var_mark(it, sl.first_test, last_test),
+                                    boot_it[k] == it ? 0 : settle_sparse_var_gate(it, sl.first_test, last_test, sl.gate_start));
             else if (keep_hard)
                 vp.settle = Settle{sl.of(g0 + t0[k]), last_test, 0};
             SC_TRY(launch_var(h, tv[k], gs[k], skip, lanes[k], vp));
@@ -1102,6 +1128,7 @@
     const int soft = st.pprior ? 1 : 0;
     if (h->settle_key_iter != c.max_iter || h->settle_key_alpha != c.alpha || h->settle_key_soft != soft) {
         h->settle_next = 0;
+        h->sparse_start_next = 0;
         h->settle_key_iter = c.max_iter;
         h->settle_key_alpha = c.alpha;
         h->settle_key_soft = soft;
@@ -1110,6 +1137,21 @@
     SC_TRY(h->d_settle.ensure((size_t)c.T * SETTLE_WORDS));
     SC_HIP(hipMemsetAsync(h->d_settle, 0, sizeof(unsigned) * (size_t)c.T * SETTLE_WORDS, c.s));
     sl->words = h->d_settle;
+    if (settle_sparse_mode(h->kn.settle_sparse, settle, h->identity_from >= 0)) {
+        SC_TRY(h->d_rowf.ensure((size_t)c.T * h->m));
+        SC_TRY(h->d_colf.ensure((size_t)c.T * h->n));
+        SC_HIP(hipMemsetAsync(h->d_rowf, 0, sizeof(uint4) * (size_t)c.T * h->m, c.s));
+        SC_HIP(hipMemsetAsync(h->d_colf, 0, sizeof(unsigned) * (size_t)c.T * h->n, c.s));
+        sl->rowf = h->d_rowf;
+        sl->colf = h->d_colf;
+        sl->m = h->m;
+        sl->n = h->n;
+        h->sparse_m = h->m;
+        h->sparse_n = h->n;
+        h->sparse_T = c.T;
+        sl->gate_start = h->sparse_start_next > sl->first_test ? h->sparse_start_next : sl->first_test;
+        h->sparse_start = sl->gate_start;
+    }
     if (settle >= 2 && !c.no_sync) {
         const int K = h->kn.settle_horizon > 0 ? h->kn.settle_horizon : h->settle_next;
         if (settle_horizon_usable(K, sl->first_test, c.max_iter)) sl->horizon = K;
@@ -1144,6 +1186,10 @@
             int g = 1;
             while (g < Gl && t + g < T && !h->settle_frozen_at[t + g]) g++;
             SC_HIP(hipMemsetAsync(sl.of(t), 0, sizeof(unsigned) * (size_t)g * SETTLE_WORDS, c.s));
+            if (sl.rowf) {
+                SC_HIP(hipMemsetAsync(sl.rowf + (size_t)t * sl.m, 0, sizeof(uint4) * (size_t)g * sl.m, c.s));
+                SC_HIP(hipMemsetAsync(sl.colf + (size_t)t * sl.n, 0, sizeof(unsigned) * (size_t)g * sl.n, c.s));
+            }
             bool d = false;
             SC_TRY(iterate_tiles(h, c, lanes, st, t, g, 0, &d, poll, 0, again));
             SC_TRY(read_back(t, g, c.max_iter));
@@ -1158,6 +1204,10 @@
     }
     const bool learns = settle_mode(h->kn.settle, h->identity_from >= 0) >= 2;
     h->settle_next = learns ? settle_next_horizon(T, frozen, max_at, (int)h->settle_rerun, c.max_iter) : 0;
+    int min_at = 0;
+    for (int t = 0; t < T; t++)
+        if (h->settle_frozen_at[t] > 0 && (min_at == 0 || h->settle_frozen_at[t] < min_at)) min_at = h->settle_frozen_at[t];
+    h->sparse_start_next = settle_sparse_next_start(min_at, sl.first_test);
     return 0;
 }
 
@@ -1447,6 +1497,8 @@
     h->settle_frozen_at.clear();
     h->settle_saved = h->settle_rerun = 0;
     h->settle_K = 0;
+    h->sparse_m = h->sparse_n = h->sparse_T = 0;
+    h->sparse_start = 0;
 }
 int begin_call(scaldpc_bp *h, int batch, int max_iter, void *stream, DecodeCall *c)
 {
@@ -1610,6 +1662,7 @@
     h->thr_valid = false;
     h->first_valid = false;
     h->settle_next = 0;
+    h->sparse_start_next = 0;
     h->ratio_valid = false;
     h->have_prior = true;
     h->prior_n = h->n;
@@ -1635,6 +1688,7 @@
     h->thr_valid = false;
     h->first_valid = false;
     h->settle_next = 0;
+    h->sparse_start_next = 0;
     h->ratio_valid = false;
     h->prior_n = std::max(h->prior_n, first + count);
     h->have_prior = true;
@@ -1793,6 +1847,7 @@
     h->thr_valid = false;
     h->first_valid = false;
     h->settle_next = 0;
+    h->sparse_start_next = 0;
     h->ratio_valid = false;
     h->d_x64.reset();
     h->d_c64.reset();
@@ -1853,6 +1908,28 @@
     info[1] = h->settle_saved;
     info[2] = h->settle_rerun;
     info[3] = h->settle_K;
+    return 0;
+}
+
+int scaldpc_bp_debug_sparse_flags(scaldpc_bp *h, int32_t tile, uint32_t *row_stamp, uint64_t *row_dirty, uint32_t *col_flag, int64_t *info)
+{
+    if (!h || !info || tile < 0) return fail(SCALDPC_EINVAL, "bad argument");
+    std::lock_guard<std::mutex> lk(h->mu);
+    info[0] = h->sparse_T;
+    info[1] = h->sparse_m;
+    info[2] = h->sparse_n;
+    info[3] = h->sparse_start;
+    if (!row_stamp && !row_dirty && !col_flag) return 0;
+    if (tile >= h->sparse_T || !row_stamp || !row_dirty || !col_flag) return fail(SCALDPC_EINVAL, "no sparse flags for that tile");
+    DeviceGuard dev(h->device);
+    const int m = h->sparse_m, n = h->sparse_n;
+    std::vector<uint4> rows((size_t)m);
+    if (m) SC_HIP(hipMemcpy(rows.data(), h->d_rowf + (size_t)tile * m, sizeof(uint4) * (size_t)m, hipMemcpyDeviceToHost));
+    if (n) SC_HIP(hipMemcpy(col_flag, h->d_colf + (size_t)tile * n, sizeof(unsigned) * (size_t)n, hipMemcpyDeviceToHost));
+    for (int r = 0; r < m; r++) {
+        row_stamp[r] = rows[(size_t)r].x;
+        row_dirty[r] = ((uint64_t)rows[(size_t)r].w << 32) | rows[(size_t)r].z;
+    }
     return 0;
 }
 
diff --git a/sca-ldpc_amd/csrc/scaldpc_bp_kernels.h b/sca-ldpc_amd/csrc/scaldpc_bp_kernels.h
--- a/sca-ldpc_amd/csrc/scaldpc_bp_kernels.h
+++ b/sca-ldpc_amd/csrc/scaldpc_bp_kernels.h
@@ -611,6 +611,9 @@
 struct Settle {
     unsigned *words = nullptr;
     int done = 0, mark = 0;
+    uint4 *rowf = nullptr;
+    unsigned *colf = nullptr;
+    int ncol = 0, gate = 0;
 };
 __device__ __forceinline__ bool settle_frozen(const unsigned *__restrict__ w, int done)
 {
@@ -625,7 +628,8 @@
                                                      float *__restrict__ rec2, unsigned char *__restrict__ arg,
                                                      u64 *__restrict__ sgn, int lane, const int *__restrict__ pos,
                                                      bool const_last = false, float x_last = 0.0f,
-                                                     unsigned *mark_word = nullptr, unsigned mark = 0, u64 real = 0)
+                                                     unsigned *mark_word = nullptr, unsigned mark = 0, u64 real = 0,
+                                                     uint4 *row_flag = nullptr)
 {
     int mp = 0;
     if constexpr (BOOT)
@@ -694,8 +698,28 @@
         if (tracked) {
             if constexpr (!EARLY) oa = arg[lane];
             arg[lane] = (unsigned char)idx;
-            const bool changed = o1 != __float_as_uint(s1) || o2 != __float_as_uint(s2) || oa != idx;
-            if ((__ballot(changed) & real) != 0 && lane == 0) *mark_word = mark;
+            const u64 c1 = __ballot(o1 != __float_as_uint(s1)) & real;
+            const u64 c2 = __ballot(o2 != __float_as_uint(s2) || oa != idx) & real;
+            if ((c1 | c2) != 0 && lane == 0) *mark_word = mark;
+            if (row_flag) {
+                u64 dirty = 0;
+                if (c1 != 0)
+                    dirty = ~0ull;
+                else if (c2 != 0) {
+#pragma unroll 1
+                    for (int half = 0; half < 2; half++) {
+                        const unsigned av = half ? idx : oa;
+                        u64 rem = c2;
+#pragma unroll 1
+                        while (rem != 0) {
+                            const unsigned a = (unsigned)__builtin_amdgcn_readlane((int)av, rfl(__builtin_ctzll(rem)));
+                            if (a < 64u) dirty |= 1ull << a;
+                            rem &= ~__ballot(av == a);
+                        }
+                    }
+                }
+                if (lane == 0) *row_flag = make_uint4(mark, 0u, (unsigned)dirty, (unsigned)(dirty >> 32));
+            }
         } else
             arg[lane] = (unsigned char)idx;
     } else
@@ -732,6 +756,7 @@
     const int *md = list + (size_t)rfl((int)blockIdx.x * 4 + (int)(threadIdx.x >> 6)) * 4;
     u64 dw = 0;
     unsigned *mark_word = nullptr;
+    bool sparse = false;
     if constexpr (PAR) {
         dw = done[tl];
         if (skip_done && dw == ~0ull) return;
@@ -743,6 +768,7 @@
             if (!BOOT && st.mark) {
                 mark_word = w + (blockIdx.x & (SETTLE_SHARDS - 1));
                 dw = done[tl];
+                sparse = st.rowf != nullptr;
             }
         }
     }
@@ -753,6 +779,16 @@
     if (r >= 0) {
         const int e0 = md[1];
         const int deg = md[2];
+        uint4 *rf = nullptr;
+        if constexpr (!BOOT && !PAR)
+            if (sparse) {
+                if (st.gate) {
+                    unsigned cf = 0;
+                    if (lane < deg) cf = st.colf[(size_t)tl * st.ncol + col_idx[e0 + lane]];
+                    if (__ballot(lane < deg && (cf >> 1) == (unsigned)(st.mark - 1)) == 0) return;
+                }
+                rf = st.rowf + (size_t)tl * m + r;
+            }
         const float *p = msg + ((size_t)tl * E + e0) * TW + lane;
         float *rt = rec + (size_t)tl * rec_tile_floats(m);
         float *rc = rt + rec_row_off(r), *rc2 = rc + rec_m2_off(m);
@@ -766,7 +802,7 @@
 #define MR(D)                                                                                                   \
     case D:                                                                                                     \
         if constexpr (D <= CAP)                                                                                 \
-            check_minsum_row_rec<D, BOOT>(p, sw, alpha, rc, rc2, ar, sg, lane, ps, cl, xl, mark_word, (unsigned)st.mark, ~dw); \
+            check_minsum_row_rec<D, BOOT>(p, sw, alpha, rc, rc2, ar, sg, lane, ps, cl, xl, mark_word, (unsigned)st.mark, ~dw, rf); \
         break;
 #define MR8(D) MR(D) MR(D + 1) MR(D + 2) MR(D + 3) MR(D + 4) MR(D + 5) MR(D + 6) MR(D + 7)
         switch (deg) {
@@ -1290,7 +1326,8 @@
                                              const unsigned char *__restrict__ arg_base, u64 *sgn_col, unsigned lane,
                                              const int *__restrict__ rc, const int4 *__restrict__ row4,
                                              const int *__restrict__ ce1, const int *__restrict__ cr1, float pr,
-                                             unsigned *mark_word = nullptr, unsigned mark = 0, u64 real = 0)
+                                             unsigned *mark_word = nullptr, unsigned mark = 0, u64 real = 0,
+                                             unsigned *col_flag = nullptr)
 {
     int eid[D], rw[D];
     {
@@ -1355,7 +1392,9 @@
     if ((int)lane < D) sgn_col[lane] = ((u64)nhi << 32) | nlo;
     if (mark_word) {
         const unsigned dlo = (nlo ^ (unsigned)slo) & (unsigned)real, dhi = (nhi ^ (unsigned)shi) & (unsigned)(real >> 32);
-        if (__ballot((int)lane < D && (dlo | dhi) != 0) != 0 && lane == 0) *mark_word = mark;
+        const bool sc = __ballot((int)lane < D && (dlo | dhi) != 0) != 0;
+        if (sc && lane == 0) *mark_word = mark;
+        if (col_flag && lane == 0) *col_flag = ((mark - 1u) << 1) | (sc ? 1u : 0u);
     }
     return temp;
 }
@@ -1497,6 +1536,7 @@
     const int4 *w4 = (const int4 *)(rw.var_rows + (size_t)ri * VAR_INLINE);
     const float pr = prior(v, tl, (int)lane);
     const unsigned r2 = (unsigned)rw.m * (TW * (unsigned)sizeof(float));
+    if (mark_word && rw.stl.colf && lane == 0) rw.stl.colf[(size_t)tl * rw.stl.ncol + v] = ((unsigned)rw.stl.mark - 1u) << 1;
     const float L = last ? var_col_rec_wide<true>(tb, rb, r2, ab, st + cb, lane, rc, w4, ce, cr, d, pr)
                          : var_col_rec_wide<false>(tb, rb, r2, ab, st + cb, lane, rc, w4, ce, cr, d, pr, mark_word,
                                                    (unsigned)rw.stl.mark, ~dn);
@@ -1549,11 +1589,28 @@
     const int cb = rc[1];
     const int d = rc[2];
     if (LAST && decided && d > 1) return;
+    const int *ce = csc_edge + cb, *cr = csc_row + cb;
+    unsigned *cf = nullptr;
+    if constexpr (!LAST)
+        if (mark_word && stl.colf && d > 1) {
+            cf = stl.colf + (size_t)tl * n + v;
+            if (stl.gate) {
+                const unsigned t = (unsigned)stl.mark - 1u;
+                bool hit = false;
+                if ((int)lane < d) {
+                    const int w = cr[lane];
+                    const uint4 f = stl.rowf[(size_t)tl * m + rec_row_of(w)];
+                    const unsigned ix = (unsigned)rec_index_of(w);
+                    hit = f.x == t && (((ix < 32u ? f.z : f.w) >> (ix & 31u)) & 1u) != 0;
+                }
+                const unsigned own = *cf;
+                if (__ballot(hit) == 0 && own != (((t - 1u) << 1) | 1u)) return;
+            }
+        }
     float *tb = msg + (size_t)tl * E * TW;
     const float *rb = rec + (size_t)tl * rec_tile_floats(m);
     const unsigned char *ab = (const unsigned char *)(rb + rec_arg_off(m));
     u64 *st = sgn + (size_t)tl * E;
-    const int *ce = csc_edge + cb, *cr = csc_row + cb;
     const int4 *w4 = (const int4 *)(var_rows + (size_t)ri * VAR_INLINE);
     const float pr = prior(v, tl, (int)lane);
     float L = pr;
@@ -1561,7 +1618,7 @@
 #define VR(D)                                                                                                \
     case D:                                                                                                  \
         if constexpr (D <= CAP)                                                                              \
-            L = var_col_rec<D, LAST>(tb, rb, r2, ab, st + cb, lane, rc, w4, ce, cr, pr, mark_word, (unsigned)stl.mark, ~dn); \
+            L = var_col_rec<D, LAST>(tb, rb, r2, ab, st + cb, lane, rc, w4, ce, cr, pr, mark_word, (unsigned)stl.mark, ~dn, cf); \
         break;
 #define VR8(D) VR(D) VR(D + 1) VR(D + 2) VR(D + 3) VR(D + 4) VR(D + 5) VR(D + 6) VR(D + 7)
     switch (d) {
diff --git a/sca-ldpc_amd/csrc/scaldpc_bp_sched.h b/sca-ldpc_amd/csrc/scaldpc_bp_sched.h
--- a/sca-ldpc_amd/csrc/scaldpc_bp_sched.h
+++ b/sca-ldpc_amd/csrc/scaldpc_bp_sched.h
@@ -184,6 +184,28 @@
 
 inline int settle_mode(int knob, bool identity_block) { return knob >= 0 ? knob : identity_block ? 2 : 0; }
 
+inline int settle_sparse_check_gate(int it, int first_test, int last_test, int start)
+{
+    const int from = start > first_test ? start : first_test;
+    return settle_check_mark(it, first_test, last_test) != 0 && settle_var_mark(it - 1, first_test, last_test) != 0 && it > from;
+}
+inline int settle_sparse_var_gate(int it, int first_test, int last_test, int start)
+{
+    const int from = start > first_test ? start : first_test;
+    return settle_var_mark(it, first_test, last_test) != 0 && settle_check_mark(it, first_test, last_test) != 0 && it >= from;
+}
+constexpr int SETTLE_SPARSE_LEAD = 2;
+inline int settle_sparse_next_start(int min_frozen_at, int first_test)
+{
+    if (min_frozen_at <= 0) return 0;
+    const int s = min_frozen_at - SETTLE_SPARSE_LEAD;
+    return s > first_test ? s : first_test;
+}
+inline int settle_sparse_mode(int knob, int settle, bool identity_block)
+{
+    return settle <= 0 ? 0 : knob >= 0 ? knob : (settle >= 2 && identity_block) ? 1 : 0;
+}
+
 struct RecVarSlices {
     int narrow0 = 0, narrow_n = 0, narrow_deg = 0, narrow_grid = 0;
     int wide0 = 0, wide_n = 0, wide_grid = 0;
```

Measured after the change: 9264 billion directed edge-message updates/s (median of 6 runs). +10.6%, better.
